# Francesco215/autoregressive_diffusion

Measured on AMD Instinct MI355X. Metric: denoiser-step frames/sec at 1/2/4/8 MI355X; 64-frame Lunar-Lander seq, higher is better.
Workload: dtype bf16; 1 GPU; Lunar-Lander 64-frame seq, gym EDM2 UNet 46.2M (gym_train.py:37-47), 8 seq/GPU (gym_train.py:55 micro_batch_size), step = EDM2Loss fwd + bwd + grad all-reduce + [grad-norm clip +] AdamW + 2 EMA profiles, 3:1 mix of 3-D/2-D steps; global_batch=8, seq_len=64, parallelism=dp1, hip_graph=False

## Files before the change

autoregressive_diffusion_amd/_lib.py:

```python
import ctypes as C
import os

import torch

_HERE = os.path.dirname(os.path.abspath(__file__))
LIB_PATH = os.path.join(_HERE, os.environ.get("ONIRIS_LIB_NAME", "liboniris_hip.so"))

if not os.path.exists(LIB_PATH):
    raise ImportError(f"{LIB_PATH} not found: build the HIP extension first (make -j8 at the repo root); "
                      "there is no CPU/PyTorch fallback for the denoiser kernels")

lib = C.CDLL(LIB_PATH)

c_void_p, c_int, c_float, c_int32, c_int64, c_size_t = C.c_void_p, C.c_int, C.c_float, C.c_int32, C.c_int64, C.c_size_t


class WeightDesc(C.Structure):
    _fields_ = [("w", c_void_p), ("grad", c_void_p), ("wf", c_void_p), ("wb", c_void_p), ("dwp", c_void_p), ("dws", c_void_p),
                ("cout", c_int32), ("cin", c_int32), ("taps", c_int32), ("kt", c_int32),
                ("CoutP", c_int32), ("CinP", c_int32), ("CoutPb", c_int32), ("CinPb", c_int32),
                ("row_start", c_int32), ("perm3", c_int32), ("gain", c_float), ("nsplit_cap", c_int32),
                ("nsplit", c_void_p), ("tile_start", c_int32), ("pad_", c_int32)]


class ConvArgs(C.Structure):
    _fields_ = [("x", c_void_p), ("ctx", c_void_p), ("w_own", c_void_p), ("w_ctx", c_void_p), ("out", c_void_p),
                ("coef_own", c_void_p), ("coef_ctx", c_void_p),
                ("B", c_int32), ("S", c_int32), ("T", c_int32), ("H", c_int32), ("W", c_int32),
                ("Cin", c_int32), ("CinP", c_int32), ("Cout", c_int32), ("CoutP", c_int32), ("taps", c_int32),
                ("ctx_bstride", c_int32), ("ctx_T", c_int32), ("coff0", c_int32), ("coff1", c_int32),
                ("ctx_fill", c_float), ("epi", c_int32),
                ("res", c_void_p), ("escale", c_void_p), ("emb_gain", c_void_p), ("out2", c_void_p),
                ("ta", c_float), ("tb", c_float), ("clip", c_float), ("ctx_out", c_void_p),
                ("big_tile", c_int32), ("escale_pitch", c_int32),
                ("splitk_ws", c_void_p), ("splitk_ws_bytes", C.c_size_t), ("clip_flag", c_void_p),
                ("ctx_prod", c_void_p), ("ctx_prod_mode", c_int32), ("x_split", c_int32), ("x2", c_void_p), ("act_out", c_void_p),
                ("cat_w1", c_float), ("cat_w2", c_float), ("ctx_rows", c_int32),
                ("ab_c1", c_int32), ("ab_da", c_void_p), ("ab_xo", c_void_p), ("ab_dskip", c_void_p), ("ab_dadd", c_void_p),
                ("ab_w1", c_float), ("ab_w2", c_float), ("ab_dxo_scale", c_float)]


class WgradArgs(C.Structure):
    _fields_ = [("x", c_void_p), ("dy", c_void_p), ("dwp", c_void_p), ("scale", c_void_p),
                ("B", c_int32), ("T", c_int32), ("H", c_int32), ("W", c_int32), ("Cin", c_int32), ("CinP", c_int32),
                ("Cout", c_int32), ("CoutP", c_int32), ("taps", c_int32),
                ("xb_stride", c_int32), ("x_T", c_int32), ("coff", c_int32), ("fill", c_float),
                ("nsplit_cap", c_int32), ("taps_total", c_int32), ("tap0", c_int32), ("pad_", c_int32),
                ("nsplit_out", c_void_p)]


class AttnArgs(C.Structure):
    _fields_ = [("q", c_void_p), ("k", c_void_p), ("v", c_void_p), ("qt", c_void_p), ("kt", c_void_p),
                ("vt", c_void_p), ("out", c_void_p), ("lse", c_void_p),
                ("kv_num", c_void_p), ("kv_idx", c_void_p), ("q_num", c_void_p), ("q_idx", c_void_p),
                ("tab_cols", c_int32), ("qtab_cols", c_int32),
                ("B", c_int32), ("heads", c_int32), ("Lq", c_int32), ("Lk", c_int32), ("C", c_int32),
                ("mask_mode", c_int32), ("P", c_int32), ("T", c_int32), ("tab_block", c_int32),
                ("dout", c_void_p), ("doutt", c_void_p), ("delta", c_void_p),
                ("dq", c_void_p), ("dk", c_void_p), ("dv", c_void_p),
                ("dkv_part", c_void_p), ("dkv_chunks", c_int32), ("dkv_item_keys", c_int32),
                ("sched", c_void_p), ("sched_wgs", c_int32), ("sched_slots", c_int32), ("v_bstride", c_int64),
                ("k_bstride", c_int64), ("split_ws", c_void_p), ("kv_splits", c_int32), ("frame_kernel", c_int32)]


class AttnF32Args(C.Structure):
    _fields_ = [("q", c_void_p), ("k", c_void_p), ("v", c_void_p), ("out", c_void_p), ("lse", c_void_p),
                ("dout", c_void_p), ("delta", c_void_p), ("dq", c_void_p), ("dk", c_void_p), ("dv", c_void_p),
                ("BH", c_int32), ("Lq", c_int32), ("Lk", c_int32), ("D", c_int32), ("mask_mode", c_int32), ("P", c_int32),
                ("T", c_int32), ("q_frame_off", c_int32), ("scale", c_float), ("pad_", c_int32)]


EPI_NONE, EPI_EMB_SILU, EPI_MPSUM, EPI_ACT_BWD = 0, 1, 2, 3

_SIGS = {
    "oniris_last_error": (C.c_char_p, []),
    "oniris_abi_version": (c_int, []),
    "oniris_struct_sizes": (c_int, [c_void_p]),
    "oniris_profile_arm": (c_int, [c_void_p, c_void_p]),
    "oniris_profile_disarm": (c_int, []),
    "oniris_set_cu_reserve": (c_int, [c_int]),
    "oniris_set_ew_nt_bytes": (c_int64, [c_int64]),
    "oniris_frame_attn_bwd": (c_int, [c_void_p, c_void_p]),
    "oniris_frame_attn_qkv_fwd": (c_int, [c_void_p, c_void_p, c_void_p, c_int64, c_int, c_int, c_void_p]),
    "oniris_frame_attn_qkv_bwd": (c_int, [c_void_p, c_void_p, c_void_p, c_void_p, c_void_p, c_int64, c_int, c_int, c_void_p]),
    "oniris_conv_f32": (c_int, [c_void_p, c_void_p, c_void_p, c_int64, c_int, c_int, c_int, c_int, c_int, c_void_p]),
    "oniris_wgrad_f32": (c_int, [c_void_p, c_void_p, c_void_p, c_int64, c_int, c_int, c_int, c_int, c_int, c_void_p]),
    "oniris_attn_f32_fwd": (c_int, [c_void_p, c_void_p]),
    "oniris_attn_f32_bwd": (c_int, [c_void_p, c_void_p]),
    "oniris_census": (c_int, [c_int]),
    "oniris_census_read": (c_int64, [C.c_char_p, c_int64]),
    "oniris_train_mask": (c_int, [c_int, c_int, c_void_p, c_void_p, C.POINTER(c_int)]),
    "oniris_infer_mask": (c_int, [c_int, c_int, c_void_p, c_void_p, C.POINTER(c_int)]),
    "oniris_mask_transpose": (c_int, [c_int, c_int, c_void_p, c_void_p, c_void_p, c_void_p]),
    "oniris_attn_schedule": (c_int, [c_int, c_int, c_void_p, c_int, c_void_p, c_int]),
    "oniris_weight_prep": (c_int, [c_void_p, c_int, c_int, c_int, c_int, c_void_p]),
    "oniris_weight_bwd": (c_int, [c_void_p, c_int, c_int, c_void_p]),
    "oniris_adamw": (c_int, [c_void_p, c_void_p, c_void_p, c_void_p, c_size_t, c_float, c_float, c_float, c_float,
                             c_float, c_int, c_float, c_void_p]),
    "oniris_adamw_clip_ema": (c_int, [c_void_p, c_void_p, c_void_p, c_void_p, c_size_t, c_float, c_float, c_float,
                                      c_float, c_float, c_int, c_float, c_void_p, c_float, c_void_p, c_float, c_void_p,
                                      c_float, c_void_p]),
    "oniris_sqnorm": (c_int, [c_void_p, c_size_t, c_void_p, c_void_p]),
    "oniris_dart_input": (c_int, [c_void_p, c_void_p, c_void_p, c_void_p, c_int, c_int, c_int, c_int, c_int, c_int,
                                  c_float, c_void_p, c_int, c_void_p]),
    "oniris_dart_loss": (c_int, [c_void_p, c_void_p, c_void_p, c_void_p, c_void_p, c_void_p, c_int, c_int, c_int, c_int,
                                 c_int, c_int, c_float, c_void_p]),
    "oniris_dart_loss_bwd": (c_int, [c_void_p, c_void_p, c_void_p, c_void_p, c_void_p, c_void_p, c_void_p, c_void_p, c_int,
                                     c_int, c_int, c_int, c_int, c_int, c_float, c_void_p]),
    "oniris_loss_tail": (c_int, [c_void_p, c_void_p, c_void_p, c_void_p, c_void_p, c_void_p, c_void_p, c_void_p, c_void_p, c_int,
                                 c_int, c_int, c_int, c_int, c_int, c_float, c_void_p]),
    "oniris_qkv_norm_hd": (c_int, [c_void_p, c_void_p, c_void_p, c_void_p, c_void_p, c_void_p, c_void_p, c_int64, c_int, c_int,
                                   c_int, c_int, c_int, c_int, c_int, c_void_p]),
    "oniris_qkv_norm_hd_bwd": (c_int, [c_void_p, c_void_p, c_void_p, c_void_p, c_void_p, c_void_p, c_void_p, c_void_p, c_int64,
                                       c_int, c_int, c_int, c_int, c_int, c_int, c_int, c_void_p]),
    "oniris_rope_hd": (c_int, [c_void_p, c_void_p, c_void_p, c_void_p, c_void_p, c_int64, c_int, c_int, c_int, c_int, c_int,
                               c_int, c_int, c_void_p]),
    "oniris_conv_fwd": (c_int, [C.POINTER(ConvArgs), c_void_p]),
    "oniris_conv_wgrad": (c_int, [C.POINTER(WgradArgs), c_void_p]),
    "oniris_conv_wgrad_group": (c_int, [C.POINTER(WgradArgs), c_int, c_void_p]),
    "oniris_gconv_bwd_prep": (c_int, [c_void_p, c_void_p, c_void_p, c_void_p, c_void_p, c_void_p, c_void_p, c_void_p,
                                      c_int, c_int, c_int, c_int64, c_void_p]),
    "oniris_gconv_bwd_fused": (c_int, [c_int, c_void_p, c_void_p, c_void_p, c_void_p, c_void_p, c_void_p, c_void_p, c_void_p,
                                       c_void_p, c_void_p, c_void_p, c_void_p, c_void_p, c_int, c_int, c_int, c_int,
                                       c_float, c_float, c_float, c_int, c_void_p, c_void_p, c_void_p]),
    "oniris_act_fwd": (c_int, [c_void_p, c_void_p, c_void_p, c_void_p, c_void_p, c_int64, c_int, c_int, c_float, c_float,
                               c_int, c_int, c_int, c_int, c_void_p]),
    "oniris_act_bwd": (c_int, [c_void_p, c_void_p, c_void_p, c_void_p, c_void_p, c_void_p, c_void_p, c_int64, c_int, c_int,
                               c_float, c_float, c_int, c_float, c_void_p]),
    "oniris_mpsum_mask": (c_int, [c_void_p, c_void_p, c_int64, c_float, c_void_p, c_void_p]),
    "oniris_emb_silu_bwd": (c_int, [c_void_p, c_void_p, c_void_p, c_void_p, c_void_p, c_int, c_int, c_int, c_int, c_int,
                                    c_void_p]),
    "oniris_mpsum_bwd": (c_int, [c_void_p, c_void_p, c_void_p, c_void_p, c_int64, c_float, c_float, c_float, c_void_p]),
    "oniris_resample": (c_int, [c_void_p, c_void_p, c_void_p, c_int64, c_int, c_int, c_int, c_int, c_float, c_void_p]),
    "oniris_resample_filter": (c_int, [c_void_p, c_void_p, c_void_p, c_int64, c_int, c_int, c_int, c_int, c_void_p, c_int, c_float,
                                       c_void_p]),
    "oniris_qkv_norm": (c_int, [c_void_p, c_void_p, c_void_p, c_void_p, c_int64, c_int, c_int64, c_int64, c_int64, c_void_p]),
    "oniris_qkv_norm_bwd": (c_int, [c_void_p, c_void_p, c_void_p, c_void_p, c_void_p, c_int64, c_int, c_void_p]),
    "oniris_qkv_norm_rope": (c_int, [c_void_p, c_void_p, c_void_p, c_void_p, c_void_p, c_void_p, c_void_p, c_int64, c_int, c_int,
                                     c_int, c_void_p]),
    "oniris_qkv_norm_rope_bwd": (c_int, [c_void_p, c_void_p, c_void_p, c_void_p, c_void_p, c_void_p, c_void_p, c_void_p, c_int64,
                                         c_int, c_int, c_int, c_void_p]),
    "oniris_qkv_eval": (c_int, [c_void_p, c_void_p, c_void_p, c_void_p, c_void_p, c_void_p, c_void_p, c_void_p, c_void_p, c_int64,
                                c_int, c_int, c_int64, c_int64, c_int64, c_int, c_void_p]),
    "oniris_precond_out": (c_int, [c_void_p, c_void_p, c_void_p, c_void_p, c_void_p, c_int, c_int, c_int, c_int, c_float,
                                   c_void_p]),
    "oniris_qkv_eval_pair": (c_int, [c_void_p, c_void_p, c_void_p, c_void_p, c_void_p, c_void_p, c_void_p, c_void_p, c_void_p,
                                     c_int64, c_int64, c_int, c_int, c_int64, c_int64, c_int64, c_int, c_void_p, c_void_p, c_void_p,
                                     c_void_p]),
    "oniris_dart_input_pair": (c_int, [c_void_p, c_void_p, c_void_p, c_int, c_int, c_int, c_int, c_int, c_float, c_void_p, c_int,
                                       c_void_p]),
    "oniris_precond_out_guided": (c_int, [c_void_p, c_void_p, c_void_p, c_void_p, c_void_p, c_int, c_int, c_int, c_int, c_float,
                                          c_float, c_void_p]),
    "oniris_sampler_update": (c_int, [c_int, c_void_p, c_void_p, c_void_p, c_void_p, c_void_p, c_size_t, c_float, c_float,
                                      c_void_p, c_int, c_float, c_void_p]),
    "oniris_embed_eval": (c_int, [c_void_p, c_void_p, c_void_p, c_void_p, c_void_p, c_void_p, c_void_p, c_int, c_int, c_int,
                                  c_int, c_void_p]),
    "oniris_gates": (c_int, [c_void_p, c_void_p, c_void_p, c_void_p, c_void_p, c_int, c_int, c_int, c_void_p]),
    "oniris_gates_bwd": (c_int, [c_void_p, c_void_p, c_void_p, c_void_p, c_void_p, c_void_p, c_int, c_int, c_int, c_void_p]),
    "oniris_emb_scale": (c_int, [c_void_p, c_void_p, c_void_p, c_void_p, c_int, c_int, c_void_p]),
    "oniris_emb_scale_bwd": (c_int, [c_void_p, c_void_p, c_void_p, c_void_p, c_void_p, c_void_p, c_int, c_int, c_int, c_void_p]),
    "oniris_embed_pre": (c_int, [c_void_p, c_void_p, c_void_p, c_void_p, c_void_p, c_void_p, c_int, c_int, c_int, c_int, c_int,
                                 c_void_p]),
    "oniris_embed_post": (c_int, [c_void_p, c_void_p, c_void_p, c_size_t, c_float, c_void_p]),
    "oniris_embed_post_bwd": (c_int, [c_void_p, c_void_p, c_void_p, c_void_p, c_void_p, c_size_t, c_float, c_void_p]),
    "oniris_rope": (c_int, [c_void_p, c_void_p, c_void_p, c_void_p, c_void_p, c_void_p, c_int, c_int, c_int, c_int,
                            c_int, c_int, c_int, c_int64, c_int64, c_void_p]),
    "oniris_qkv_norm_rope_eval": (c_int, [c_void_p, c_void_p, c_void_p, c_void_p, c_void_p, c_void_p, c_void_p, c_void_p,
                                          c_int64, c_int, c_int64, c_int64, c_int64, c_int, c_void_p]),
    "oniris_attn_fwd": (c_int, [C.POINTER(AttnArgs), c_void_p]),
    "oniris_attn_bwd_prep": (c_int, [c_void_p, c_void_p, c_void_p, c_void_p, c_void_p, c_void_p, c_int, c_int, c_int, c_int,
                                     c_void_p]),
    "oniris_attn_bwd_dq": (c_int, [C.POINTER(AttnArgs), c_void_p]),
    "oniris_attn_bwd_dkv": (c_int, [C.POINTER(AttnArgs), c_void_p]),
    "oniris_vae_temb": (c_int, [c_void_p, c_void_p, c_int, c_void_p, c_int, c_void_p, c_void_p]),
    "oniris_vae_up": (c_int, [c_void_p, c_int64, c_int64, c_int64, c_int64, c_int64, c_int, c_int, c_int, c_int, c_int, c_void_p,
                              c_void_p, c_void_p, c_void_p, c_int, c_int, c_void_p, c_void_p]),
    "oniris_vae_res_a": (c_int, [c_void_p, c_void_p, c_void_p, c_void_p, c_void_p, c_void_p, c_int, c_int, c_int, c_int, c_int,
                                 c_int, c_int, c_int, c_void_p, c_void_p]),
    "oniris_vae_res_b": (c_int, [c_void_p, c_void_p, c_void_p, c_void_p, c_int, c_int, c_int, c_int, c_int, c_int, c_void_p,
                                 c_void_p]),
    "oniris_vae_out": (c_int, [c_void_p, c_void_p, c_void_p, c_int, c_int, c_int, c_int, c_int, c_int, c_int, c_void_p, c_void_p,
                               c_void_p, c_int64, c_int64, c_int64, c_int64, c_int64, c_void_p, c_void_p]),
    "oniris_vae_down": (c_int, [c_void_p, c_int, c_int64, c_int64, c_int64, c_int64, c_int64, c_int, c_int, c_int, c_int, c_int,
                                c_int, c_int, c_int, c_void_p, c_void_p, c_int, c_void_p, c_void_p]),
    "oniris_vae_latents": (c_int, [c_void_p, c_int, c_int, c_int, c_int, c_int, c_void_p, c_void_p, c_void_p, c_int64, c_int64,
                                   c_int64, c_int64, c_int64, c_void_p]),
    "oniris_vae_train_res_a": (c_int, [c_void_p, c_void_p, c_void_p, c_void_p, c_int, c_int, c_int, c_int, c_int, c_int, c_int,
                                       c_int, c_void_p, c_void_p]),
    "oniris_vae_train_res_b": (c_int, [c_void_p, c_void_p, c_void_p, c_void_p, c_int, c_int, c_int, c_int, c_int, c_int, c_void_p,
                                       c_void_p]),
    "oniris_vae_res_b_bwd": (c_int, [c_void_p, c_void_p, c_void_p, c_int, c_int, c_int, c_int, c_int, c_int, c_void_p, c_void_p]),
    "oniris_vae_res_a_bwd": (c_int, [c_void_p, c_void_p, c_void_p, c_void_p, c_void_p, c_int, c_int, c_int, c_int, c_int, c_int,
                                     c_int, c_int, c_void_p, c_void_p, c_void_p]),
    "oniris_vae_conv3_wgrad_bwd": (c_int, [c_void_p, c_void_p, c_void_p, c_int, c_int, c_int, c_int, c_int, c_int, c_int, c_void_p,
                                           c_int, c_void_p]),
    "oniris_vae_slab_sum_bwd": (c_int, [c_void_p, c_int, c_int64, c_void_p, c_void_p]),
    "oniris_vae_lin_dx_bwd": (c_int, [c_void_p, c_int, c_int, c_int, c_void_p, c_void_p, c_int, c_int, c_int, c_int, c_int, c_int,
                                      c_int, c_void_p]),
    "oniris_vae_lin_dw_bwd": (c_int, [c_void_p, c_int, c_int, c_int, c_void_p, c_int, c_int, c_int, c_int, c_int, c_int, c_int,
                                      c_void_p, c_int, c_void_p]),
}
# ... 43 lines not shown
```

autoregressive_diffusion_amd/csrc/common.h:

```cpp
#pragma once
#include <hip/hip_runtime.h>
#include <hip/hip_ext.h>
#include <stdint.h>
#include <stdio.h>
#include <string.h>

typedef __bf16 bf16;
typedef __attribute__((ext_vector_type(8))) __bf16 bf16x8;
typedef __attribute__((ext_vector_type(4))) __bf16 bf16x4;
typedef __attribute__((ext_vector_type(2))) __bf16 bf16x2;
typedef __attribute__((ext_vector_type(4))) short s16x4;
typedef __attribute__((ext_vector_type(16))) float f32x16;
typedef __attribute__((ext_vector_type(4))) float f32x4;
typedef __attribute__((ext_vector_type(4))) unsigned int u32x4;

#define ONIRIS_OK 0
#define ONIRIS_EINVAL (-1)
#define ONIRIS_ELAUNCH (-2)
#define ONIRIS_EUNSUPPORTED (-3)

void oniris_set_error(const char* fmt, ...);

#define ONIRIS_CHECK_ARG(cond, ...)                \
  do {                                             \
    if (!(cond)) {                                 \
      oniris_set_error(__VA_ARGS__);               \
      return ONIRIS_EINVAL;                        \
    }                                              \
  } while (0)

#define ONIRIS_LAUNCH_CHECK()                                            \
  do {                                                                   \
    hipError_t e_ = hipGetLastError();                                   \
    if (e_ != hipSuccess) {                                              \
      oniris_set_error("%s:%d launch failed: %s", __FILE__, __LINE__,    \
                       hipGetErrorString(e_));                           \
      return ONIRIS_ELAUNCH;                                             \
    }                                                                    \
  } while (0)

extern thread_local hipEvent_t oniris_prof_ev[2];

extern int oniris_census_on;
void oniris_census_note(const void* kernel_handle, const char* tag);
#define ONIRIS_KLAUNCH(kern, grid, block, shmem, stream, ...)                            \
  do {                                                                                   \
    if (oniris_census_on) oniris_census_note((const void*)(kern), nullptr);              \
    hipLaunchKernelGGL(kern, grid, block, shmem, stream, __VA_ARGS__);                   \
  } while (0)

template <typename K, typename... A>
static inline void oniris_launch_tagged(const char* tag, K kern, dim3 grid, dim3 block, hipStream_t stream, A... args) {
  if (oniris_census_on) oniris_census_note((const void*)kern, tag);
  if (oniris_prof_ev[0]) {
    hipExtLaunchKernelGGL(kern, grid, block, 0, stream, oniris_prof_ev[0], oniris_prof_ev[1], 0, args...);
    oniris_prof_ev[0] = oniris_prof_ev[1] = nullptr;
  } else {
    hipLaunchKernelGGL(kern, grid, block, 0, stream, args...);
  }
}
template <typename K, typename... A>
static inline void oniris_launch(K kern, dim3 grid, dim3 block, hipStream_t stream, A... args) {
  oniris_launch_tagged(nullptr, kern, grid, block, stream, args...);
}

long long oniris_ew_nt_bytes(void);
template <bool NT, typename V>
__device__ __forceinline__ V ldv(const V* p) {
  if constexpr (NT) return __builtin_nontemporal_load(p);
  else return *p;
}
template <bool NT, typename V>
__device__ __forceinline__ void stv(V* p, V v) {
  if constexpr (NT) __builtin_nontemporal_store(v, p);
  else *p = v;
}

extern int oniris_cu_reserve;
int oniris_persistent_wgs(void);

static inline int cdiv(int a, int b) { return (a + b - 1) / b; }
static inline int roundup(int a, int b) { return cdiv(a, b) * b; }

#ifdef __HIPCC__
__device__ __forceinline__ float bf2f(bf16 v) { return (float)v; }
__device__ __forceinline__ bf16 f2bf(float v) { return (bf16)v; }

__device__ __forceinline__ f32x16 mfma32(bf16x8 a, bf16x8 b, f32x16 c) {
  return __builtin_amdgcn_mfma_f32_32x32x16_bf16(a, b, c, 0, 0, 0);
}
__device__ __forceinline__ float sigmoid_fast(float z) {
  return __builtin_amdgcn_rcpf(1.f + __builtin_amdgcn_exp2f(-1.4426950408889634f * z));
}
__device__ __forceinline__ float act_adjoint_da(float da, float xo) {
  const float sg = sigmoid_fast(xo);
  const float one_m = 1.f - sg;
  const float u = __builtin_fmaf(one_m, xo, 1.f);
  float g = sg * u;
  g = g * da;
  return g * (1.0f / 0.596f);
}
__device__ __forceinline__ float act_adjoint_dxo(float g, float dxo_scale, float dxo) { return __builtin_fmaf(dxo_scale, dxo, g); }
__device__ __forceinline__ float act_adjoint_out(float g, float w, bool has_add, float add) {
  return has_add ? __builtin_fmaf(w, g, add) : g * w;
}
__device__ __forceinline__ int mfma_row(int r, int lane) { return (r & 3) + 8 * (r >> 2) + 4 * (lane >> 5); }

__device__ __forceinline__ float wave_sum(float v) {
#pragma unroll
  for (int o = 32; o > 0; o >>= 1) v += __shfl_xor(v, o);
  return v;
}
__device__ __forceinline__ float wave_max(float v) {
#pragma unroll
  for (int o = 32; o > 0; o >>= 1) v = fmaxf(v, __shfl_xor(v, o));
  return v;
}

__device__ __forceinline__ float block_sum(float v, float* red) {
  v = wave_sum(v);
  const int w = threadIdx.x >> 6, nw = blockDim.x >> 6;
  __syncthreads();
  if ((threadIdx.x & 63) == 0) red[w] = v;
  __syncthreads();
  float t = 0.f;
  for (int i = 0; i < nw; ++i) t += red[i];
  return t;
}
#endif
```

autoregressive_diffusion_amd/csrc/conv_api.hip:

```cpp
#include "conv_fwd_common.h"

extern "C" int oniris_conv_fwd(const OnirisConvArgs* args, oniris_stream_t stream_) {
  hipStream_t st = (hipStream_t)stream_;
  ONIRIS_CHECK_ARG(args && args->w_own && ((args->x && args->out) || args->ctx_prod_mode == 3), "conv_fwd: null pointer");
  const OnirisConvArgs& a = *args;
  if (a.ctx_prod_mode != 0 && !(a.S == 1 && a.ctx && a.taps == 9 && a.ctx_prod)) {
    oniris_set_error("conv_fwd: ctx_prod_mode %d is for the one-frame cached evaluation (S == 1, context path, ctx_prod given)", a.ctx_prod_mode);
    return ONIRIS_EUNSUPPORTED;
  }
  if (a.ctx_rows != 0 && !(a.S == 1 && a.T == 1 && a.ctx && a.taps == 9 && a.ctx_rows > 0 && a.B == 2 * a.ctx_rows &&
                           a.ctx_out == nullptr && a.ctx_prod_mode != 3)) {
    oniris_set_error("conv_fwd: ctx_rows %d is for the one-frame cached evaluation of a guided pair (S = T = 1, context path, "
                     "B = 2 * ctx_rows (got B = %d), no ctx_out, ctx_prod_mode != 3)", a.ctx_rows, a.B);
    return ONIRIS_EUNSUPPORTED;
  }
  ONIRIS_CHECK_ARG(a.taps == 9 || a.taps == 1, "conv_fwd: taps must be 1 or 9 (got %d)", a.taps);
  ONIRIS_CHECK_ARG(a.B > 0 && a.T > 0 && a.H > 0 && a.W > 0 && (a.S == 1 || a.S == 2), "conv_fwd: bad sizes");
  ONIRIS_CHECK_ARG(a.Cin % 8 == 0 && a.Cout % 8 == 0, "conv_fwd: Cin, Cout must be multiples of 8 (%d,%d)", a.Cin, a.Cout);
  ONIRIS_CHECK_ARG(a.CoutP % 32 == 0 && a.CinP % 64 == 0 && a.CoutP >= a.Cout && a.CinP >= a.Cin,
                   "conv_fwd: bad padded sizes CoutP=%d CinP=%d", a.CoutP, a.CinP);
  ONIRIS_CHECK_ARG(a.epi != ONIRIS_EPI_MPSUM || a.res, "conv_fwd: EPI_MPSUM needs res");
  ONIRIS_CHECK_ARG(a.epi != ONIRIS_EPI_EMB_SILU || (a.escale && a.out2), "conv_fwd: EPI_EMB_SILU needs escale/out2");
  ONIRIS_CHECK_ARG(a.epi != ONIRIS_EPI_ACT_BWD ||
                       (a.taps == 1 && a.S == 1 && !a.ctx && !a.x2 && !a.out2 && !a.ctx_out && !a.coef_own && !a.coef_ctx && a.ab_da && a.ab_xo &&
                        a.ab_dskip && a.ab_c1 > 0 && a.ab_c1 < a.Cout && a.ab_c1 % 8 == 0 && a.ctx_prod_mode == 0 && a.ctx_rows == 0),
                   "conv_fwd: EPI_ACT_BWD is a plain 1x1 launch (S == 1) with ab_da / ab_xo / ab_dskip and 0 < ab_c1 < Cout, ab_c1 %% 8 == 0");
  ONIRIS_CHECK_ARG(a.x2 == nullptr || (a.taps == 1 && a.ctx == nullptr), "conv_fwd: x2 (concatenated input) is a 1x1, context-free option");
  const bool has_ctx = a.ctx != nullptr;
  ONIRIS_CHECK_ARG(!has_ctx || (a.w_ctx && a.taps == 9), "conv_fwd: context path needs w_ctx and taps == 9");
  if (a.clip_flag && (a.taps == 1 || (a.S == 1 && has_ctx))) {
    const hipError_t e = hipMemsetD32Async((hipDeviceptr_t)a.clip_flag, 1, 1, st);
    if (e != hipSuccess) { oniris_set_error("conv: clip_flag fill failed: %s", hipGetErrorString(e)); return ONIRIS_ELAUNCH; }
  }
  if (a.taps == 1) {
    ONIRIS_CHECK_ARG(a.S == 1, "conv_fwd: 1x1 variant expects S == 1 (fold slots into T)");
    return conv_dispatch_1x1(a, st);
  }
  if (a.S == 2) {
    ONIRIS_CHECK_ARG(has_ctx, "conv_fwd: S == 2 is the DART training layout and needs the context path");
    return conv_dispatch_s2ctx(a, st);
  }
  return has_ctx ? conv_dispatch_s1ctx(a, st) : conv_dispatch_s1(a, st);
}
```

autoregressive_diffusion_amd/csrc/conv_fwd_s2ctx.hip:

```cpp
#include "conv_fwd_common.h"
#include "conv_glds.h"
#include "conv_stream.h"

template <int NT>
static int glds_pick(const OnirisConvArgs& a, hipStream_t st) {
  if constexpr (NT == 1)
    if (a.Cin == 32 && a.big_tile != 7) return launch_conv_glds<1, 16, 8, 1, 1, true, true>(a, st);
  return launch_conv_glds<NT, 16, 8, 1>(a, st);
}

int conv_dispatch_s2ctx(const OnirisConvArgs& a, hipStream_t st) {
  if (a.big_tile >= 4 && conv_stream_ok(a)) return launch_conv_stream(a, st);
  if (a.big_tile >= 3 && conv_glds_ok(a, 16, 16, (a.CoutP % 64 == 0) ? 64 : 32))
    return (a.CoutP % 64 == 0) ? glds_pick<2>(a, st) : glds_pick<1>(a, st);
  if (a.big_tile >= 3 && a.W == 8 && a.H == 8 && a.CoutP % 64 == 0 && conv_glds_ok(a, 8, 8, 64))
    return launch_conv_glds<1, 8, 8, 1, 2>(a, st);
  if (a.clip_flag) {
    const hipError_t e = hipMemsetD32Async((hipDeviceptr_t)a.clip_flag, 1, 1, st);
    if (e != hipSuccess) { oniris_set_error("conv: clip_flag fill failed: %s", hipGetErrorString(e)); return ONIRIS_ELAUNCH; }
  }
  return conv3x3_pick<2, true>(a, st);
}
```

autoregressive_diffusion_amd/csrc/conv_stream.h:

```cpp
#pragma once
#include "conv_kernels.h"
#include "lds_dma.h"

#ifdef CONV_STAMP
#define SSTAMP_DECL unsigned long long st_t = __builtin_amdgcn_s_memtime(), st_acc[8] = {0, 0, 0, 0, 0, 0, 0, 0};
#define SSTAMP(i) { const unsigned long long n_ = __builtin_amdgcn_s_memtime(); st_acc[i] += n_ - st_t; st_t = n_; }
#else
#define SSTAMP_DECL
#define SSTAMP(i)
#endif

struct ConvStreamDev {
  OnirisConvArgs a;
  int ntx, nty, nseg, seglen;
  int dir;
  int nt;
};

template <bool ALIAS>
__global__ __launch_bounds__(256, 2) void conv_stream_kernel(const ConvStreamDev d) {
#if defined(__HIP_DEVICE_COMPILE__)
  constexpr int TAPS = 9, KS = 2, NST = TAPS * KS, HW_ = 18, HALO = 6 * 18, HBUF = 7168;
  constexpr int NXS0 = ALIAS ? 4 : 2, NCTX = ALIAS ? 0 : 3;
  constexpr int EROW = 80, STGB = 32 * EROW;
  constexpr int XS0 = 0, XS1 = NXS0 * HBUF, CTXR = XS1 + 2 * HBUF, EXCH = CTXR + NCTX * HBUF;
  constexpr int STG = ALIAS ? EXCH + 6 * 4096 : EXCH, ESC = EXCH + 6 * 4096 + (ALIAS ? 4 * STGB : 0);
  constexpr int LDS_BYTES = ESC + 512;
  static_assert(2 * LDS_BYTES <= 160 * 1024, "two workgroups per CU");
  __shared__ __attribute__((aligned(16))) unsigned char smem[LDS_BYTES];

  const OnirisConvArgs& a = d.a;
  const int tid = threadIdx.x, lane = tid & 63, wave = tid >> 6, r = lane & 31, h = lane >> 5;
  const int uw = __builtin_amdgcn_readfirstlane(wave);
  const bool ctxw = uw >= 2;
  const int sl = uw >> 1, pt = uw & 1;
  const int H = a.H, W = a.W, T = a.T, HWp = H * W, Cout = a.Cout;
  constexpr int Cin = 32;
  const int frame_elems = HWp * Cin;

  int u;
  {
    const int n = gridDim.x, xcd = blockIdx.x & 7, q = n >> 3, rr = n & 7;
    u = ((xcd < rr) ? xcd * (q + 1) : rr * (q + 1) + (xcd - rr) * q) + (blockIdx.x >> 3);
  }
  const int seg = u % d.nseg; u /= d.nseg;
  const int x0 = (u % d.ntx) * 16; u /= d.ntx;
  const int y0 = (u % d.nty) * 4;
  const int b = u / d.nty;
  const int t_lo = seg * d.seglen, t_hi = min(T, t_lo + d.seglen), nfr = t_hi - t_lo;
  const int dir = d.dir, ts = (dir > 0) ? t_lo : t_hi - 1;

  int pr;
  {
    const bool ga = (r < 4) || (r >= 12 && r < 16) || (r >= 20 && r < 28);
    const int k = ga ? ((r < 4) ? r : (r < 16) ? r - 8 : r - 12) : ((r < 12) ? r - 4 : (r < 20) ? r - 8 : r - 16);
    pr = (ga ? 0 : 16) + k;
  }
  int xaddrA[TAPS], xaddrB[TAPS];
#pragma unroll
  for (int tap = 0; tap < TAPS; ++tap) {
    const int tA = ctxw ? 0 : pt, tB = ctxw ? 1 : pt;
    const int RA = (2 * tA + (pr >> 4) + tap / 3) * HW_ + (pr & 15) + tap % 3;
    const int RB = (2 * tB + (pr >> 4) + tap / 3) * HW_ + (pr & 15) + tap % 3;
    xaddrA[tap] = RA * 64 + ((h ^ ((RA >> 2) & 3)) << 4);
    xaddrB[tap] = RB * 64 + ((h ^ ((RB >> 2) & 3)) << 4);
  }

  constexpr int OOB = (int)0x80000000;
  int hv[2];
#pragma unroll
  for (int i = 0; i < 2; ++i) {
    const int e = i * 256 + tid, row = e >> 2, gp = (e & 3) ^ ((row >> 2) & 3);
    const int y = y0 + row / HW_ - 1, x = x0 + row % HW_ - 1;
    hv[i] = (e < HALO * 4 && (unsigned)y < (unsigned)H && (unsigned)x < (unsigned)W) ? ((y * W + x) * Cin + gp * 8) * 2 : OOB;
  }
  const i32x4 rs_x = make_rsrc((const bf16*)a.x + (size_t)b * 2 * T * frame_elems, 2 * T * frame_elems * 2);
  const i32x4 rs_c = make_rsrc((const bf16*)a.ctx + (size_t)b * a.ctx_bstride * frame_elems, a.ctx_T * frame_elems * 2);
  const i32x4 rs_f = make_rsrc(oniris_fill_rows, 128);
  const int fillsel = (a.ctx_fill != 0.f) ? 64 : 0;
  const unsigned lds0 = (unsigned)(size_t)(lds_void_t*)smem, wdst = lds0 + wave * 1024;
  auto halo = [&](const i32x4& rs, int so, unsigned dst) __attribute__((always_inline)) {
    dma16(rs, hv[0], so, dst + wdst);
    if (256 + tid < HALO * 4) dma16(rs, hv[1], so, dst + wdst + 4096);
  };
  auto halo_fill = [&](unsigned dst) __attribute__((always_inline)) {
    dma16(rs_f, (hv[0] < 0) ? OOB : fillsel, 0, dst + wdst);
    if (256 + tid < HALO * 4) dma16(rs_f, (hv[1] < 0) ? OOB : fillsel, 0, dst + wdst + 4096);
  };
  auto ctx_slot = [&](int f) __attribute__((always_inline)) {
    return ALIAS ? XS0 + (f & 3) * HBUF : CTXR + ((f + 3) % 3) * HBUF;
  };
  auto issue_ctx = [&](int f) __attribute__((always_inline)) {
    if (f >= 0 && f < a.ctx_T) halo(rs_c, f * frame_elems * 2, ctx_slot(f));
    else halo_fill(ctx_slot(f));
  };
  auto issue_x = [&](int f) __attribute__((always_inline)) {
    halo(rs_x, f * frame_elems * 2, XS0 + (ALIAS ? (f & 3) : (f & 1)) * HBUF);
    halo(rs_x, (T + f) * frame_elems * 2, XS1 + (f & 1) * HBUF);
  };

  bf16x8 wreg[NST];
  {
    const bf16* wsrc = ctxw ? (const bf16*)a.w_ctx + (size_t)(uw - 2) * TAPS * a.CoutP * a.CinP : (const bf16*)a.w_own;
#pragma unroll
    for (int i = 0; i < NST; ++i)
      wreg[i] = *(const bf16x8*)(wsrc + ((size_t)(i / KS) * a.CoutP + r) * a.CinP + (i % KS) * 16 + h * 8);
  }
#pragma unroll
  for (int i = 0; i < NST; ++i) asm volatile("" : "+v"(wreg[i]));

  const int ppy = 2 * pt + (pr >> 4), ppx = pr & 15;
  const int pix = (y0 + ppy) * W + x0 + ppx;
  const int uslot = sl;
  const bool emb = a.epi == ONIRIS_EPI_EMB_SILU, mps = a.epi == ONIRIS_EPI_MPSUM;
  const int epitch = a.escale_pitch ? a.escale_pitch : Cout;
  const i32x4 rs_e = make_rsrc(a.escale ? a.escale : (const void*)oniris_fill_rows, emb ? (int)(((size_t)a.B * 2 * T - 1) * epitch + Cout) * 4 : 0);
  const i32x4 rs_r = make_rsrc(mps ? (const bf16*)a.res + (size_t)b * 2 * T * HWp * Cout : (const bf16*)oniris_fill_rows,
                               mps ? 2 * T * HWp * Cout * 2 : 0);
  const int evoff = (lane < 16 && (lane & 7) * 4 < Cout) ? ((lane >> 3) * T * epitch) * 4 + (lane & 7) * 16 : OOB;
  auto issue_esc = [&](int f) __attribute__((always_inline)) {
    if (lane < 16) dma16(rs_e, evoff, ((b * 2 * T + f) * epitch) * 4, lds0 + ESC + (f & 1) * 256);
  };
  typedef __attribute__((ext_vector_type(2))) unsigned int u32x2;
  u32x2 resq[4];
#pragma unroll
  for (int g = 0; g < 4; ++g) { resq[g][0] = 0u; resq[g][1] = 0u; }
  int rvoff[4];
#pragma unroll
  for (int g = 0; g < 4; ++g) rvoff[g] = (8 * g + 4 * h < Cout) ? (pix * Cout + 8 * g + 4 * h) * 2 : OOB;
  auto load_res = [&](int f) __attribute__((always_inline)) {
    const int so = __builtin_amdgcn_readfirstlane(((uslot * T + f) * HWp * Cout) * 2);
#pragma unroll
    for (int g = 0; g < 4; ++g)
      asm volatile("buffer_load_dwordx2 %0, %1, %2, %3 offen" : "=v"(resq[g]) : "v"(rvoff[g]), "s"(rs_r), "s"(so) : "memory");
  };
  auto wait_vm = [&](int n) __attribute__((always_inline)) {
    switch (n) {
      case 0: asm volatile("s_waitcnt vmcnt(0)" ::: "memory"); break;
      case 1: asm volatile("s_waitcnt vmcnt(1)" ::: "memory"); break;
      case 2: asm volatile("s_waitcnt vmcnt(2)" ::: "memory"); break;
      case 3: asm volatile("s_waitcnt vmcnt(3)" ::: "memory"); break;
      case 4: asm volatile("s_waitcnt vmcnt(4)" ::: "memory"); break;
      case 5: asm volatile("s_waitcnt vmcnt(5)" ::: "memory"); break;
      case 6: asm volatile("s_waitcnt vmcnt(6)" ::: "memory"); break;
      case 7: asm volatile("s_waitcnt vmcnt(7)" ::: "memory"); break;
      case 8: asm volatile("s_waitcnt vmcnt(8)" ::: "memory"); break;
      default: asm volatile("s_waitcnt vmcnt(9)" ::: "memory"); break;
    }
  };
  const int per_halo = (uw < 3) ? 2 : 1;
  const int n_dma = (ALIAS ? 2 : 3) * per_halo + ((emb && uw == 0) ? 1 : 0);
  const int n_st = (a.ctx_out ? 1 : 0) + 2 * (mps ? ((a.out2 ? 1 : 0) + 1) : emb ? 2 : 1);
  if (nfr <= 0) return;
  issue_ctx(ts + a.coff0);
  issue_ctx(ts + a.coff1);
  issue_x(ts);
  if (emb && uw == 0) issue_esc(ts);

  float* const E = (float*)(smem + EXCH);
  unsigned char* const ep = smem + STG + wave * (ALIAS ? STGB : 4096);

  SSTAMP_DECL
#pragma unroll 1
  for (int i = 0; i < nfr; ++i) {
    const int t = ts + i * dir, tn = t + dir;
    SSTAMP(7)
    wait_vm(i ? n_st : 0);
    SSTAMP(0)
    __syncthreads();
    SSTAMP(1)
    const bool has_next = i + 1 < nfr;
    const int nfrm = __builtin_amdgcn_readfirstlane((b * 2 + uslot) * T + t);
    typedef const __attribute__((address_space(4))) float cfloat_t;
    const float cown = a.coef_own ? ((cfloat_t*)(size_t)a.coef_own)[nfrm] : 1.f;
    const float cctx = a.coef_ctx ? ((cfloat_t*)(size_t)a.coef_ctx)[nfrm] : 1.f;
    if (mps) load_res(t);
    if (has_next) {
      issue_x(tn);
      if (!ALIAS) issue_ctx(tn + a.coff1);
      if (emb && uw == 0) issue_esc(tn);
    }

    SSTAMP(2)
    f32x16 acc0, acc1;
#pragma unroll
    for (int k = 0; k < 16; ++k) { acc0[k] = 0.f; acc1[k] = 0.f; }
    {
      const unsigned char* bA = smem + (ctxw ? ctx_slot(t + (uw == 2 ? a.coff0 : a.coff1)) : XS0 + (ALIAS ? (t & 3) : (t & 1)) * HBUF);
      const unsigned char* bB = ctxw ? bA : smem + XS1 + (t & 1) * HBUF;
      bf16x8 xf[2][2];
      xf[0][0] = *(const bf16x8*)(bA + xaddrA[0]);
      xf[0][1] = *(const bf16x8*)(bB + xaddrB[0]);
#pragma unroll
      for (int st = 0; st < NST; ++st) {
        if (st + 1 < NST) {
          const int tap = (st + 1) / KS, ks = (st + 1) % KS;
          xf[(st + 1) & 1][0] = *(const bf16x8*)(bA + (xaddrA[tap] ^ (ks * 32)));
          xf[(st + 1) & 1][1] = *(const bf16x8*)(bB + (xaddrB[tap] ^ (ks * 32)));
        }
        acc0 = mfma32(wreg[st], xf[st & 1][0], acc0);
        acc1 = mfma32(wreg[st], xf[st & 1][1], acc1);
        if (st + 1 < NST) __builtin_amdgcn_sched_group_barrier(0x100, 2, 0);
        __builtin_amdgcn_sched_group_barrier(0x008, 2, 0);
      }
    }
#ifdef CONV_STAMP
    asm volatile("" ::"v"(acc0), "v"(acc1));
#endif
    SSTAMP(3)
    if (!ctxw) {
#pragma unroll
      for (int k = 0; k < 16; ++k) E[(pt * 16 + k) * 64 + lane] = acc1[k];
    } else {
      const int e0 = (uw == 2) ? 2 : 4;
#pragma unroll
      for (int k = 0; k < 16; ++k) {
        E[((e0 + 0) * 16 + k) * 64 + lane] = acc0[k];
        E[((e0 + 1) * 16 + k) * 64 + lane] = acc1[k];
      }
    }
    SSTAMP(4)
    __syncthreads();
    SSTAMP(5)
    float v[16], cx[16];
    if (!ctxw) {
#pragma unroll
      for (int k = 0; k < 16; ++k) {
        cx[k] = E[((2 + pt) * 16 + k) * 64 + lane] + E[((4 + pt) * 16 + k) * 64 + lane];
        v[k] = __builtin_fmaf(cctx, cx[k], cown * acc0[k]);
      }
    } else {
      const float* Eo = E + ((((uw == 2) ? 4 : 2) + pt) * 16) * 64 + lane;
      const float* Ew = E + (pt * 16) * 64 + lane;
#pragma unroll
      for (int k = 0; k < 16; ++k) {
        const float mine = pt ? acc1[k] : acc0[k], other = Eo[k * 64];
        cx[k] = (uw == 2) ? mine + other : other + mine;
        v[k] = __builtin_fmaf(cctx, cx[k], cown * Ew[k * 64]);
      }
    }
    if (!ALIAS) __syncthreads();
    const size_t blk = ((size_t)(b * 2 + sl) * T + t) * HWp;
    auto put = [&](const float (&vv)[16]) __attribute__((always_inline)) {
#pragma unroll
      for (int g = 0; g < 4; ++g) {
        bf16x4 o;
#pragma unroll
        for (int k = 0; k < 4; ++k) o[k] = f2bf(vv[4 * g + k]);
        *(bf16x4*)(ep + pr * EROW + (8 * g + 4 * h) * 2) = o;
      }
    };
    auto flush_row = [&](bf16* dst, size_t fblk, int it) __attribute__((always_inline)) {
      const int id = it * 64 + lane, row = id >> 2, part = id & 3;
      const size_t px_ = (size_t)(y0 + 2 * pt + (row >> 4)) * W + x0 + (row & 15);
      if (part * 8 < Cout) {
        const u32x4 v_ = *(const u32x4*)(ep + row * EROW + part * 16);
        u32x4* o_ = (u32x4*)(dst + (fblk + px_) * Cout + part * 8);
        if (d.nt) __builtin_nontemporal_store(v_, o_); else *o_ = v_;
      }
    };
    auto flush = [&](bf16* dst, size_t fblk) __attribute__((always_inline)) {
      flush_row(dst, fblk, 0);
      flush_row(dst, fblk, 1);
    };
    auto store_y3 = [&]() __attribute__((always_inline)) {
      put(cx);
      flush_row((bf16*)a.ctx_out, ((size_t)b * T + t) * HWp, sl);
    };
    if (mps) {
      wait_vm(has_next ? n_dma : 0);
#pragma unroll
      for (int g = 0; g < 4; ++g) asm volatile("" : "+v"(resq[g]));
      float o[16];
      bool clip_hit = false;
#pragma unroll
      for (int g = 0; g < 4; ++g) {
        const bf16x4 rv = __builtin_bit_cast(bf16x4, resq[g]);
#pragma unroll
        for (int k = 0; k < 4; ++k) {
          float q = a.ta * bf2f(rv[k]) + a.tb * v[4 * g + k];
          if (a.clip > 0.f) {
            q = fminf(fmaxf(q, -a.clip), a.clip);
            clip_hit |= !(fabsf(bf2f(f2bf(q))) < a.clip);
          }
          o[4 * g + k] = q;
        }
      }
      if (a.ctx_out) store_y3();
      if (a.out2) { put(v); flush((bf16*)a.out2, blk); }
      put(o);
      flush((bf16*)a.out, blk);
      if (a.clip_flag && __builtin_amdgcn_ballot_w64(clip_hit) != 0ull) {
        if (lane == 0) atomicOr(a.clip_flag, 1);
        asm volatile("s_waitcnt vmcnt(0)" ::: "memory");
      }
      SSTAMP(6)
      continue;
    }
    if (a.ctx_out) store_y3();
    {
      put(v);
      flush((bf16*)a.out, blk);
      if (a.epi == ONIRIS_EPI_EMB_SILU) {
#pragma unroll
        for (int g = 0; g < 4; ++g) {
          const float4 ev = *(const float4*)(smem + ESC + (t & 1) * 256 + (sl * 32 + 8 * g + 4 * h) * 4);
          const float cvv[4] = {ev.x, ev.y, ev.z, ev.w};
#pragma unroll
          for (int k = 0; k < 4; ++k) {
            const float z = bf2f(f2bf(v[4 * g + k])) * cvv[k];
            v[4 * g + k] = z * sigmoid_fast(z) * (1.f / 0.596f);
          }
        }
        put(v);
        flush((bf16*)a.out2, blk);
      }
    }
    SSTAMP(6)
  }
#ifdef CONV_STAMP
  if (blockIdx.x == 0 && lane == 0 && a.splitk_ws) {
    unsigned long long* dst = (unsigned long long*)a.splitk_ws + wave * 8;
    for (int i = 0; i < 8; ++i) dst[i] = st_acc[i];
  }
#endif
#endif
}

static inline bool conv_stream_ok(const OnirisConvArgs& a) {
  if (!(a.S == 2 && a.ctx && a.taps == 9 && a.Cin == 32 && a.CinP == 64 && a.CoutP == 32 && a.W % 16 == 0 && a.H % 4 == 0))
    return false;
  if (!(a.ctx_fill == 0.f || a.ctx_fill == 1.f) || a.ctx_T != a.T) return false;
  if (!((a.coff0 == -2 && a.coff1 == -1) || (a.coff0 == 2 && a.coff1 == 1))) return false;
  if (2LL * a.T * a.H * a.W * 32 * 2 >= (1LL << 31)) return false;
  return true;
}

static int launch_conv_stream(const OnirisConvArgs& a, hipStream_t stream) {
  ConvStreamDev d;
  d.a = a;
  d.ntx = a.W / 16; d.nty = a.H / 4;
  d.dir = (a.coff0 < 0) ? 1 : -1;
  const int units = a.B * d.ntx * d.nty;
  int nseg = 512 / units;
  if (nseg > a.T / 8) nseg = a.T / 8;
  if (nseg < 1) nseg = 1;
  d.nt = 2LL * a.B * a.T * a.H * a.W * a.Cout * 2 >= oniris_ew_nt_bytes();
  d.seglen = cdiv(a.T, nseg);
  d.nseg = cdiv(a.T, d.seglen);
  const bool alias = a.ctx == a.x && a.ctx_bstride == 2 * a.T && d.dir == 1;
  if (alias) oniris_launch_tagged(d.nt ? "nt-stores" : nullptr, conv_stream_kernel<true>, dim3(units * d.nseg), dim3(256), stream, d);
  else oniris_launch_tagged(d.nt ? "nt-stores" : nullptr, conv_stream_kernel<false>, dim3(units * d.nseg), dim3(256), stream, d);
  ONIRIS_LAUNCH_CHECK();
  return ONIRIS_OK;
}
```

autoregressive_diffusion_amd/csrc/conv_wgrad.hip:

```cpp
#include "conv_kernels.h"

#define WGRAD_MAXG 3
struct WgradDev {
  OnirisWgradArgs a[WGRAD_MAXG];
  int ntiles[WGRAD_MAXG], ntt[WGRAD_MAXG], gstart[WGRAD_MAXG + 1];
  int ntx, nty, ncib;
};

__device__ __forceinline__ bf16x8 tr_frag(const unsigned char* base0, const unsigned char* base1) {
  typedef __attribute__((address_space(3))) s16x4 lds_s16x4;
  const s16x4 lo = __builtin_amdgcn_ds_read_tr16_b64_v4i16((lds_s16x4*)base0);
  const s16x4 hi = __builtin_amdgcn_ds_read_tr16_b64_v4i16((lds_s16x4*)base1);
  typedef __attribute__((ext_vector_type(8))) short s16x8;
  s16x8 v;
  v[0] = lo[0]; v[1] = lo[1]; v[2] = lo[2]; v[3] = lo[3];
  v[4] = hi[0]; v[5] = hi[1]; v[6] = hi[2]; v[7] = hi[3];
  return __builtin_bit_cast(bf16x8, v);
}

#include "conv_wgrad_glds.h"
#include "conv_wgrad_stream.h"
#include "wgrad1x1_glds.h"

template <int TAPS, int PW, int CT, int IT>
// ... 122 lines not shown
#pragma unroll 1
  for (int tile = bx; tile < g_ntiles; tile += gxg) {
    store_tile();
    __syncthreads();
    if (tile + gxg < g_ntiles) load_tile(tile + gxg);
    {
      constexpr int NK = 8 / NKS, NSTEP = NK * TAPS;
      bf16x8 af[4], bfm[4];
      auto ld_a = [&](int kb, int ksi) __attribute__((always_inline)) {
        const int ks = ksi * NKS + my_ks;
        const int p0 = ks * 16 + 8 * hh + q, p1 = p0 + 4;
        af[kb] = tr_frag(dy_lds + p0 * DY_ROWB + (ct * 32 + pcol) * 2, dy_lds + p1 * DY_ROWB + (ct * 32 + pcol) * 2);
      };
      auto ld_b = [&](int fb, int st) __attribute__((always_inline)) {
        const int ksi = st / TAPS, tap = st % TAPS;
        const int ks = ksi * NKS + my_ks;
        const int p0 = ks * 16 + 8 * hh + q, p1 = p0 + 4;
        int r0 = p0, r1 = p1;
        if constexpr (TAPS == 9) {
          r0 = ((p0 / (P::PH * P::PW)) * P::HH + (p0 / P::PW) % P::PH) * P::HW + p0 % P::PW;
          r1 = ((p1 / (P::PH * P::PW)) * P::HH + (p1 / P::PW) % P::PH) * P::HW + p1 % P::PW;
        }
        const int off = (TAPS == 9) ? ((tap / 3) * P::HW + (tap % 3)) : 0;
        bfm[fb] = tr_frag(x_lds + (r0 + off) * X_ROWB + (it * 32 + pcol) * 2, x_lds + (r1 + off) * X_ROWB + (it * 32 + pcol) * 2);
      };
      constexpr int LA = (NSTEP > 3) ? 3 : 1;
      constexpr int NA0 = (LA + TAPS - 1) / TAPS;
#pragma unroll
      for (int j = 0; j < LA; ++j) {
        if (j % TAPS == 0) ld_a((j / TAPS) & 3, j / TAPS);
        ld_b(j, j);
      }
      __builtin_amdgcn_sched_group_barrier(0x100, 2 * NA0 + 2 * LA, 0);
#pragma unroll
      for (int st = 0; st < NSTEP; ++st) {
        const int ksi = st / TAPS, tap = st % TAPS;
        const int nx = st + LA;
        if (nx < NSTEP) {
          if (nx % TAPS == 0) ld_a((nx / TAPS) & 3, nx / TAPS);
          ld_b(nx & 3, nx);
        }
        acc[tap] = mfma32(af[ksi & 3], bfm[st & 3], acc[tap]);
        if (nx < NSTEP) {
          if (nx % TAPS == 0) __builtin_amdgcn_sched_group_barrier(0x100, 4, 0);
          else __builtin_amdgcn_sched_group_barrier(0x100, 2, 0);
        }
        __builtin_amdgcn_sched_group_barrier(0x008, 1, 0);
      }
    }
    __syncthreads();
  }

  if (bx == 0 && blockIdx.y == 0 && tid == 0 && a.nsplit_out) *a.nsplit_out = gxg;
  const int cj = ci0 + it * 32 + (lane & 31);
  if constexpr (NKS > 1) {
    float* red = (float*)smem;
#pragma unroll
    for (int tap = 0; tap < TAPS; ++tap) {
      __syncthreads();
      if (my_ks > 0) {
#pragma unroll
        for (int rr = 0; rr < 16; ++rr) red[((my_ks - 1) * 16 + rr) * 64 + lane] = acc[tap][rr];
      }
      __syncthreads();
      if (my_ks == 0) {
#pragma unroll
        for (int rr = 0; rr < 16; ++rr) {
          float v = acc[tap][rr];
#pragma unroll
          for (int w = 0; w < NKS - 1; ++w) v += red[(w * 16 + rr) * 64 + lane];
          acc[tap][rr] = v;
        }
      }
    }
    if (my_ks != 0) return;
  }
  bf16* slab = (bf16*)a.dwp + (size_t)bx * a.taps_total * a.CoutP * a.CinP;
#pragma unroll
  for (int tap = 0; tap < TAPS; ++tap) {
    bf16* base = slab + (size_t)(a.tap0 + tap) * a.CinP;
#pragma unroll
    for (int rr = 0; rr < 16; ++rr) {
      const int co = co0 + ct * 32 + mfma_row(rr, lane);
      if (co < a.CoutP && cj < a.CinP) base[(size_t)co * a.taps_total * a.CinP + cj] = f2bf(acc[tap][rr]);
    }
  }
}

template <int TAPS, int PW, int CT, int IT>
static int launch_wgrad(const OnirisWgradArgs* args, int ng, hipStream_t stream) {
  using P = Patch<PW>;
  const OnirisWgradArgs& a = args[0];
  WgradDev d;
  memset(&d, 0, sizeof(d));
  if (TAPS == 9) { d.ntx = a.W / P::PW; d.nty = a.H / P::PH; } else { d.ntx = 1; d.nty = 1; }
  d.ncib = cdiv(a.Cin, 32 * IT);
  const int ncob = cdiv(a.Cout, 32 * CT);
  const int gy = d.ncib * ncob;
  long long tot = 0;
  bool use_glds = false;
  if constexpr (TAPS == 9 && (PW == 16 || PW == 8)) use_glds = a.pad_ >= 0 && wgrad_glds_ok(args, ng);
  const int ft = (use_glds && PW == 8) ? 1 : P::FT;
  for (int g = 0; g < ng; ++g) {
    d.a[g] = args[g];
    d.ntt[g] = (TAPS == 9) ? cdiv(args[g].T, ft) : cdiv(args[g].T * a.H * a.W, 128);
    d.ntiles[g] = d.ntx * d.nty * d.ntt[g] * args[g].B;
    tot += d.ntiles[g];
  }
#ifndef WGRAD_NG
#define WGRAD_NG 1
#endif
  const int gx_budget = (CT * IT == 4) ? ((use_glds && WGRAD_NG == 1) ? 512 : 256) : 512;
  const int gx_all = gx_budget / gy > ng ? gx_budget / gy : ng;
  int gx_tot = 0;
  for (int g = 0; g < ng; ++g) {
    int gx = (int)((long long)gx_all * d.ntiles[g] / (tot > 0 ? tot : 1));
    if (gx > args[g].nsplit_cap) gx = args[g].nsplit_cap;
    if (gx > d.ntiles[g]) gx = d.ntiles[g];
    if (gx < 1) gx = 1;
    d.gstart[g] = gx_tot;
    gx_tot += gx;
  }
  for (int g = ng; g <= WGRAD_MAXG; ++g) d.gstart[g] = gx_tot;
  if constexpr (TAPS == 9 && (PW == 16 || PW == 8)) {
    if (use_glds) {
#ifndef WGRAD_NG1
#define WGRAD_NG1 1
#endif
      constexpr int NG = (CT * IT == 4) ? WGRAD_NG : WGRAD_NG1;
      auto kern = conv_wgrad_glds_kernel<CT, IT, NG, PW>;
      oniris_launch(kern, dim3(gx_tot, gy), dim3(256 * NG), stream, d);
      ONIRIS_LAUNCH_CHECK();
      return ONIRIS_OK;
    }
  }
  auto kern = conv_wgrad_kernel<TAPS, PW, CT, IT>;
  oniris_launch(kern, dim3(gx_tot, gy), dim3(256), stream, d);
  ONIRIS_LAUNCH_CHECK();
  return ONIRIS_OK;
}

template <int TAPS, int PW>
static int wgrad_pick_tile(const OnirisWgradArgs* a, int ng, hipStream_t stream) {
  if (a[0].Cin > 32 && a[0].Cout > 32) return launch_wgrad<TAPS, PW, 2, 2>(a, ng, stream);
  return launch_wgrad<TAPS, PW, 1, 1>(a, ng, stream);
}

extern "C" int oniris_conv_wgrad_group(const OnirisWgradArgs* args, int ngroups, oniris_stream_t stream_) {
  hipStream_t stream = (hipStream_t)stream_;
  ONIRIS_CHECK_ARG(args && ngroups >= 1 && ngroups <= WGRAD_MAXG, "conv_wgrad: 1..%d groups", WGRAD_MAXG);
  const OnirisWgradArgs& a = args[0];
  for (int g = 0; g < ngroups; ++g) {
    const OnirisWgradArgs& b = args[g];
    ONIRIS_CHECK_ARG(b.x && b.dy && b.dwp, "conv_wgrad: null pointer (group %d)", g);
    ONIRIS_CHECK_ARG(b.nsplit_cap >= 1 && b.taps_total >= b.taps + b.tap0 && b.tap0 >= 0,
                     "conv_wgrad: bad slab description (group %d)", g);
    ONIRIS_CHECK_ARG(b.B > 0 && b.T > 0, "conv_wgrad: empty group %d", g);
    ONIRIS_CHECK_ARG(b.H == a.H && b.W == a.W && b.Cin == a.Cin && b.CinP == a.CinP && b.Cout == a.Cout &&
                     b.CoutP == a.CoutP && b.taps == a.taps, "conv_wgrad: groups must share H, W, channels and taps");
  }
  ONIRIS_CHECK_ARG(a.taps == 9 || a.taps == 1, "conv_wgrad: taps must be 1 or 9 (got %d)", a.taps);
  ONIRIS_CHECK_ARG(a.Cin % 8 == 0 && a.Cout % 8 == 0, "conv_wgrad: Cin/Cout must be multiples of 8");
  ONIRIS_CHECK_ARG(a.CoutP % 32 == 0 && a.CinP % 64 == 0 && a.CoutP >= a.Cout && a.CinP >= a.Cin,
                   "conv_wgrad: bad padded sizes");
  if (a.taps == 1) {
    if (ngroups == 1 && a.pad_ >= 0 && wgrad1x1_glds_ok(a)) return launch_wgrad1x1_glds(a, stream);
    return wgrad_pick_tile<1, 16>(args, ngroups, stream);
  }
  const int W = a.W, H = a.H;
  if (wgrad_stream_ok(args, ngroups)) {
    const int rc = launch_wgrad_stream(args, stream);
    if (rc != 1) return rc;
  }
  if (W >= 16 && W % 16 == 0 && H % 8 == 0) return wgrad_pick_tile<9, 16>(args, ngroups, stream);
  if (W == 8 && H % 8 == 0) return wgrad_pick_tile<9, 8>(args, ngroups, stream);
  if (W == 4 && H % 4 == 0) return wgrad_pick_tile<9, 4>(args, ngroups, stream);
  if (W == 2 && H % 2 == 0) return wgrad_pick_tile<9, 2>(args, ngroups, stream);
  oniris_set_error("conv_wgrad: unsupported image size %dx%d", H, W);
  return ONIRIS_EUNSUPPORTED;
}

extern "C" int oniris_conv_wgrad(const OnirisWgradArgs* args, oniris_stream_t stream) {
  return oniris_conv_wgrad_group(args, 1, stream);
}
```

autoregressive_diffusion_amd/csrc/conv_wgrad_stream.h:

```cpp
#pragma once
#include "lds_dma.h"

struct WgradStreamDev {
  const void* x;
  const void* dout;
  const void* dy3;
  const float* scale;
  void* dwp2;
  void* dwp3;
  int32_t* nsplit2;
  int32_t* nsplit3;
  int B, T, H, W, Cin, CinP, Cout, CoutP;
  int ntx, nty, nseg, seglen, ncib;
  float fill;
};

template <int PH>
__global__ __launch_bounds__(64 * PH, 2) void conv_wgrad_stream_kernel(const WgradStreamDev d) {
#if defined(__HIP_DEVICE_COMPILE__)
  static_assert(PH == 8 || PH == 4, "tile heights");
  constexpr int NTHR = 64 * PH, NPOS = PH * 16;
  constexpr int TAPS = 9, HW_ = 18, HALO = (PH + 2) * HW_, XB = HALO * 64, DB = NPOS * 64;
  constexpr int XS0 = 0, XS1 = 4 * XB, DY0 = 6 * XB;
  constexpr int LDS_BYTES = 6 * XB + 6 * DB;
  static_assert(LDS_BYTES <= 160 * 1024 && 5 * 3 * 16 * 64 * 4 <= LDS_BYTES, "LDS budget");
  __shared__ __attribute__((aligned(16))) unsigned char smem[LDS_BYTES];

  const int tid = threadIdx.x, lane = tid & 63, wave = tid >> 6;
  const int H = d.H, W = d.W, T = d.T, HWp = H * W, Cin = d.Cin, Cout = d.Cout;
  const int cib = blockIdx.y % d.ncib, cob = blockIdx.y / d.ncib;
  const int co0 = cob * 32, ci0 = cib * 32;
  int u = blockIdx.x;
  const int seg = u % d.nseg; u /= d.nseg;
  const int x0 = (u % d.ntx) * 16; u /= d.ntx;
  const int y0 = (u % d.nty) * PH;
  const int b = u / d.nty;
  const int t0 = seg * d.seglen, t1 = min(T, t0 + d.seglen);

  const int role = (PH == 8) ? ((wave < 4) ? 0 : (wave < 6 ? 1 : 2)) : ((wave < 2) ? 0 : wave - 1);
  const int slot = (PH == 8) ? ((wave < 4) ? (wave >> 1) : 0) : ((wave < 2) ? wave : 0), half = (PH == 8) ? (wave & 1) : 0;

  f32x16 acc[TAPS];
#pragma unroll
  for (int t = 0; t < TAPS; ++t)
#pragma unroll
    for (int i = 0; i < 16; ++i) acc[t][i] = 0.f;

  constexpr int OOB = (int)0x80000000;
  int dvoff;
  {
    const int row = tid >> 2, gp = tid & 3, co = co0 + gp * 8;
    dvoff = (co < Cout) ? (((row >> 4) * W + (row & 15)) * Cout + co) * 2 : OOB;
  }
  int xvoff[2];
  bool xok[2];
#pragma unroll
  for (int i = 0; i < 2; ++i) {
    const int e = i * NTHR + tid, row = e >> 2, gp = e & 3, ci = ci0 + gp * 8;
    const int hy = row / HW_, hx = row % HW_;
    xok[i] = e < HALO * 4 && ci < Cin && (unsigned)(y0 + hy - 1) < (unsigned)H && (unsigned)(x0 + hx - 1) < (unsigned)W;
    xvoff[i] = xok[i] ? (((y0 + hy - 1) * W + (x0 + hx - 1)) * Cin + ci) * 2 : OOB;
  }
  const i32x4 rs_do = make_rsrc(d.dout, d.B * 2 * T * HWp * Cout * 2);
  const i32x4 rs_d3 = make_rsrc(d.dy3, d.B * T * HWp * Cout * 2);
  const i32x4 rs_x = make_rsrc(d.x, d.B * 2 * T * HWp * Cin * 2);
  const i32x4 rs_f = make_rsrc(oniris_fill_rows, 128);
  const int fillsel = (d.fill != 0.f) ? 64 : 0;
  const unsigned lds0 = (unsigned)(size_t)(lds_void_t*)smem;
  const unsigned wdst = lds0 + wave * 1024;
  const int dy_origin = (y0 * W + x0) * Cout * 2;

  auto issue_halo = [&](int s, int f, unsigned dst) __attribute__((always_inline)) {
    if (f >= 0) {
      const int so = (((b * 2 + s) * T + f) * HWp * Cin) * 2;
      dma16(rs_x, xvoff[0], so, dst + wdst);
      if (wave < (HALO * 4 - NTHR + 63) / 64) { if (NTHR + tid < HALO * 4) dma16(rs_x, xvoff[1], so, dst + wdst + NTHR * 16); }
    } else {
      dma16(rs_f, xok[0] ? fillsel : OOB, 0, dst + wdst);
      if (wave < (HALO * 4 - NTHR + 63) / 64) { if (NTHR + tid < HALO * 4) dma16(rs_f, xok[1] ? fillsel : OOB, 0, dst + wdst + NTHR * 16); }
    }
  };
  auto issue_frame = [&](int f) __attribute__((always_inline)) {
    issue_halo(0, f, XS0 + (f & 3) * XB);
    issue_halo(1, f, XS1 + (f & 1) * XB);
    const unsigned dyb = DY0 + (f & 1) * 3 * DB;
    dma16(rs_do, dvoff, (((b * 2 + 0) * T + f) * HWp * Cout) * 2 + dy_origin, dyb + wdst);
    dma16(rs_do, dvoff, (((b * 2 + 1) * T + f) * HWp * Cout) * 2 + dy_origin, dyb + DB + wdst);
    dma16(rs_d3, dvoff, ((b * T + f) * HWp * Cout) * 2 + dy_origin, dyb + 2 * DB + wdst);
  };

  const int hh = lane >> 5, q = (lane & 15) >> 2;
  const int cslot = (lane & 3) * 8 + 32 * ((lane >> 4) & 1);
  const int dya = (half * 64 + 8 * hh + q) * 64 + cslot;
  int xa[3];
#pragma unroll
  for (int kx = 0; kx < 3; ++kx) xa[kx] = (half * 4 * HW_ + 8 * hh + q + kx) * 64 + cslot;

  typedef __attribute__((address_space(3))) s16x4 lds_s16x4;
  typedef __attribute__((ext_vector_type(8))) short s16x8;
  auto trf = [&](const unsigned char* p0) __attribute__((always_inline)) {
    const s16x4 lo = __builtin_amdgcn_ds_read_tr16_b64_v4i16((lds_s16x4*)p0);
    const s16x4 hi = __builtin_amdgcn_ds_read_tr16_b64_v4i16((lds_s16x4*)(p0 + 256));
    s16x8 v;
    v[0] = lo[0]; v[1] = lo[1]; v[2] = lo[2]; v[3] = lo[3];
    v[4] = hi[0]; v[5] = hi[1]; v[6] = hi[2]; v[7] = hi[3];
    return __builtin_bit_cast(bf16x8, v);
  };

  const bool scaled = role == 0 && d.scale != nullptr;
  float sc_next = 1.f;
  if (t0 < t1) {
    if (scaled) sc_next = d.scale[(b * 2 + slot) * T + t0];
    asm volatile("" : "+v"(sc_next));
    issue_halo(0, t0 - 2, XS0 + ((t0 - 2) & 3) * XB);
    issue_halo(0, t0 - 1, XS0 + ((t0 - 1) & 3) * XB);
    issue_frame(t0);
  }
#pragma unroll 1
  for (int t = t0; t < t1; ++t) {
    dma_wait();
    __syncthreads();
    float sc = sc_next;
    asm volatile("" : "+v"(sc));
    if (t + 1 < t1) {
      if (scaled) sc_next = d.scale[(b * 2 + slot) * T + t + 1];
      asm volatile("" : "+v"(sc_next));
      issue_frame(t + 1);
    }
    const unsigned char* abuf = smem + DY0 + (t & 1) * 3 * DB + ((role == 0) ? slot * DB : 2 * DB);
    const unsigned char* bbuf = smem + ((role == 0) ? (slot ? XS1 + (t & 1) * XB : XS0 + (t & 3) * XB)
                                                    : XS0 + ((t - 3 + role) & 3) * XB);
    constexpr int NK = 4, NSTEP = NK * TAPS, LA = 3;
    bf16x8 af[2], bfm[4];
    auto ld_a = [&](int kb, int j) __attribute__((always_inline)) {
      bf16x8 v = trf(abuf + dya + j * 16 * 64);
      if (scaled) {
#pragma unroll
        for (int k = 0; k < 8; ++k) v[k] = f2bf(bf2f(v[k]) * sc);
      }
      af[kb] = v;
    };
    auto ld_b = [&](int fb, int st) __attribute__((always_inline)) {
      const int j = st / TAPS, tap = st % TAPS, ky = tap / 3, kx = tap % 3;
      bfm[fb] = trf(bbuf + xa[kx] + (j + ky) * HW_ * 64);
    };
#ifndef WGRAD_STREAM_ROWORDER
#define WGRAD_STREAM_ROWORDER 1
#endif
    if constexpr (WGRAD_STREAM_ROWORDER != 0) {
      constexpr int NU = NK + 2, NB = NU * 3;
      bf16x8 aw[4];
      auto ld_aw = [&](int j) __attribute__((always_inline)) { ld_a(0, j); aw[j & 3] = af[0]; };
      auto ld_bu = [&](int fb, int i) __attribute__((always_inline)) { bfm[fb] = trf(bbuf + xa[i % 3] + (i / 3) * HW_ * 64); };
      ld_aw(0);
#pragma unroll
      for (int i = 0; i < LA; ++i) ld_bu(i, i);
      __builtin_amdgcn_sched_group_barrier(0x100, 2 + 2 * LA, 0);
#pragma unroll
      for (int i = 0; i < NB; ++i) {
        const int u = i / 3, kx = i % 3;
        int nrd = 0, nmf = 0;
        if (i + LA < NB) { ld_bu((i + LA) & 3, i + LA); nrd += 2; }
        if (kx == 0 && u + 1 < NK) { ld_aw(u + 1); nrd += 2; }
#pragma unroll
        for (int ky = 0; ky < 3; ++ky) {
          const int j = u - ky;
          if (j >= 0 && j < NK) { acc[ky * 3 + kx] = mfma32(aw[j & 3], bfm[i & 3], acc[ky * 3 + kx]); ++nmf; }
        }
        if (nrd == 2) __builtin_amdgcn_sched_group_barrier(0x100, 2, 0);
        else if (nrd == 4) __builtin_amdgcn_sched_group_barrier(0x100, 4, 0);
        if (nmf == 1) __builtin_amdgcn_sched_group_barrier(0x008, 1, 0);
        else if (nmf == 2) __builtin_amdgcn_sched_group_barrier(0x008, 2, 0);
        else __builtin_amdgcn_sched_group_barrier(0x008, 3, 0);
      }
    } else {
    ld_a(0, 0);
#pragma unroll
    for (int j = 0; j < LA; ++j) ld_b(j, j);
    __builtin_amdgcn_sched_group_barrier(0x100, 2 + 2 * LA, 0);
#pragma unroll
    for (int st = 0; st < NSTEP; ++st) {
      const int ks = st / TAPS, tap = st % TAPS;
      const int nxs = st + LA;
      if (nxs < NSTEP) {
        if (nxs % TAPS == 0) ld_a((nxs / TAPS) & 1, nxs / TAPS);
        ld_b(nxs & 3, nxs);
      }
      acc[tap] = mfma32(af[ks & 1], bfm[st & 3], acc[tap]);
      if (nxs < NSTEP) {
        if (nxs % TAPS == 0) __builtin_amdgcn_sched_group_barrier(0x100, 4, 0);
        else __builtin_amdgcn_sched_group_barrier(0x100, 2, 0);
      }
      __builtin_amdgcn_sched_group_barrier(0x008, 1, 0);
    }
    }
  }

  if (blockIdx.x == 0 && blockIdx.y == 0 && tid == 0) {
    if (d.nsplit2) *d.nsplit2 = gridDim.x;
    if (d.nsplit3) *d.nsplit3 = gridDim.x;
  }
  const int nl = (PH == 8) ? ((wave == 1) ? 0 : (wave == 2) ? 1 : (wave == 3) ? 2 : (wave == 5) ? 3 : (wave == 7) ? 4 : -1)
                           : ((wave == 1) ? 0 : -1);
  float* red = (float*)smem;
#pragma unroll
  for (int r3 = 0; r3 < 3; ++r3) {
    __syncthreads();
    if (nl >= 0) {
#pragma unroll
      for (int k = 0; k < 3; ++k)
#pragma unroll
        for (int rr = 0; rr < 16; ++rr) red[((nl * 3 + k) * 16 + rr) * 64 + lane] = acc[r3 * 3 + k][rr];
    }
    __syncthreads();
    if (nl < 0) {
      const int first = (PH == 8) ? ((wave == 0) ? 0 : (wave == 4) ? 3 : 4) : 0;
      const int cnt = (PH == 8) ? ((wave == 0) ? 3 : 1) : ((wave == 0) ? 1 : 0);
#pragma unroll
      for (int k = 0; k < 3; ++k)
#pragma unroll
        for (int rr = 0; rr < 16; ++rr) {
          float v = acc[r3 * 3 + k][rr];
          for (int w = 0; w < cnt; ++w) v += red[(((first + w) * 3 + k) * 16 + rr) * 64 + lane];
          acc[r3 * 3 + k][rr] = v;
        }
    }
  }
  if (nl >= 0) return;
  const int taps_total = (role == 0) ? 9 : 18, tap0 = (role == 2) ? 9 : 0;
  const int cj = ci0 + (lane & 31);
  bf16* slab = (bf16*)((role == 0) ? d.dwp2 : d.dwp3) + (size_t)blockIdx.x * taps_total * d.CoutP * d.CinP;
#pragma unroll
  for (int tap = 0; tap < TAPS; ++tap) {
    bf16* base = slab + (size_t)(tap0 + tap) * d.CinP;
#pragma unroll
    for (int rr = 0; rr < 16; ++rr) {
      const int co = co0 + mfma_row(rr, lane);
      if (co < d.CoutP && cj < d.CinP) base[(size_t)co * taps_total * d.CinP + cj] = f2bf(acc[tap][rr]);
    }
  }
#endif
}

static inline bool wgrad_stream_ok(const OnirisWgradArgs* a, int ng) {
  if (ng != 3 || a[0].pad_ < 0 || (a[0].pad_ & 2)) return false;
  const OnirisWgradArgs &o = a[0], &c0 = a[1], &c1 = a[2];
  if (o.taps != 9 || o.W % 16 != 0 || o.H % 8 != 0) return false;
  if (o.Cin > 32 && o.Cout > 32) return false;
  if (o.B != 1 || o.coff != 0 || o.tap0 != 0 || o.taps_total != 9 || o.xb_stride != o.T || o.x_T != o.T) return false;
  if (c0.x != o.x || c1.x != o.x || c0.dy != c1.dy || c0.dwp != c1.dwp || c0.scale || c1.scale) return false;
  if (c0.B != c1.B || c0.T != c1.T || o.T != 2 * c0.B * c0.T) return false;
  if (c0.xb_stride != 2 * c0.T || c1.xb_stride != 2 * c0.T || c0.x_T != c0.T || c1.x_T != c0.T) return false;
  if (c0.coff != -2 || c1.coff != -1 || c0.tap0 != 0 || c1.tap0 != 9 || c0.taps_total != 18 || c1.taps_total != 18) return false;
  if (c0.fill != c1.fill || !(c0.fill == 0.f || c0.fill == 1.f)) return false;
  if ((long long)o.T * o.H * o.W * (o.Cout > o.Cin ? o.Cout : o.Cin) * 2 >= (1LL << 31)) return false;
  return true;
}

static int launch_wgrad_stream(const OnirisWgradArgs* a, hipStream_t stream) {
  const OnirisWgradArgs &o = a[0], &c0 = a[1];
  WgradStreamDev d;
  memset(&d, 0, sizeof(d));
  d.x = o.x; d.dout = o.dy; d.dy3 = c0.dy; d.scale = o.scale;
  d.dwp2 = o.dwp; d.dwp3 = c0.dwp; d.nsplit2 = o.nsplit_out; d.nsplit3 = c0.nsplit_out;
  d.B = c0.B; d.T = c0.T; d.H = o.H; d.W = o.W; d.Cin = o.Cin; d.CinP = o.CinP; d.Cout = o.Cout; d.CoutP = o.CoutP;
#ifndef WGRAD_STREAM_PH
#define WGRAD_STREAM_PH 4
#endif
  d.ntx = o.W / 16; d.ncib = cdiv(o.Cin, 32);
  d.fill = c0.fill;
  const int ncob = cdiv(o.Cout, 32), gy = d.ncib * ncob;
  const int cap = o.nsplit_cap < c0.nsplit_cap ? o.nsplit_cap : c0.nsplit_cap;
  int ph = (WGRAD_STREAM_PH == 4 && d.B * d.ntx * (o.H / 4) <= cap) ? 4 : 8;
  d.nty = o.H / ph;
  const int units = d.B * d.ntx * d.nty;
  if (units > cap) return 1;
  int nseg = ((ph == 4 ? 512 : 256) / gy) / units;
  if (nseg > d.T / 8) nseg = d.T / 8;
  if (nseg * units > cap) nseg = cap / units;
  if (nseg < 1) nseg = 1;
  d.seglen = cdiv(d.T, nseg);
  d.nseg = cdiv(d.T, d.seglen);
  if (ph == 4) oniris_launch(conv_wgrad_stream_kernel<4>, dim3(units * d.nseg, gy), dim3(256), stream, d);
  else oniris_launch(conv_wgrad_stream_kernel<8>, dim3(units * d.nseg, gy), dim3(512), stream, d);
  ONIRIS_LAUNCH_CHECK();
  return ONIRIS_OK;
}
```

autoregressive_diffusion_amd/csrc/weights.hip:

```cpp
#include <cstdlib>
#include "common.h"
#include "../../include/oniris.h"

#define W_EPS 1e-4f

__device__ __forceinline__ const OnirisWeightDesc* find_desc(const OnirisWeightDesc* d, int n, int row) {
  int lo = 0, hi = n - 1;
  while (lo < hi) {
    int mid = (lo + hi + 1) >> 1;
    if (d[mid].row_start <= row) lo = mid; else hi = mid - 1;
  }
  return d + lo;
}

__device__ __forceinline__ int perm_row(const OnirisWeightDesc* d, int co) {
  if (!d->perm3) return co;
  const int C = d->cout / 3;
  return (co % 3) * C + co / 3;
}

__device__ __forceinline__ const OnirisWeightDesc* find_desc_tile(const OnirisWeightDesc* d, int n, int tile) {
  int lo = 0, hi = n - 1;
  while (lo < hi) {
    int mid = (lo + hi + 1) >> 1;
// ... 215 lines not shown
  return ONIRIS_OK;
}

__global__ void adamw_kernel(float* __restrict__ p, const float* __restrict__ g, float* __restrict__ m,
                             float* __restrict__ v, size_t n, float lr, float b1, float b2, float eps, float wd,
                             float bc1, float bc2, float gscale, const float* __restrict__ gnorm_sq, float max_norm,
                             float* __restrict__ ema0, float w0, float* __restrict__ ema1, float w1) {
  if (bc1 == 0.f) {
    size_t i = ((size_t)blockIdx.x * blockDim.x + threadIdx.x) * 4;
    const size_t stride = (size_t)gridDim.x * blockDim.x * 4;
    for (; i < n; i += stride)
      for (size_t k = i; k < n && k < i + 4; ++k) {
        if (ema0) ema0[k] += w0 * (p[k] - ema0[k]);
        if (ema1) ema1[k] += w1 * (p[k] - ema1[k]);
      }
    return;
  }
  if (gnorm_sq) {
    const float coef = max_norm / (sqrtf(*gnorm_sq) * fabsf(gscale) + 1e-6f);
    if (coef < 1.f) gscale *= coef;
  }
  size_t i = ((size_t)blockIdx.x * blockDim.x + threadIdx.x) * 4;
  const size_t stride = (size_t)gridDim.x * blockDim.x * 4;
  for (; i + 3 < n; i += stride) {
    float4 P = *(float4*)(p + i), G = *(const float4*)(g + i), M = *(float4*)(m + i), V = *(float4*)(v + i);
    float* pp = (float*)&P; float* gg = (float*)&G; float* mm = (float*)&M; float* vv = (float*)&V;
#pragma unroll
    for (int k = 0; k < 4; ++k) {
      const float gr = gg[k] * gscale;
      mm[k] = b1 * mm[k] + (1.f - b1) * gr;
      vv[k] = b2 * vv[k] + (1.f - b2) * gr * gr;
      const float mh = mm[k] / bc1, vh = vv[k] / bc2;
      pp[k] = pp[k] * (1.f - lr * wd) - lr * mh / (sqrtf(vh) + eps);
    }
    *(float4*)(p + i) = P; *(float4*)(m + i) = M; *(float4*)(v + i) = V;
    if (ema0) {
      float4 E = *(float4*)(ema0 + i);
      E.x += w0 * (P.x - E.x); E.y += w0 * (P.y - E.y); E.z += w0 * (P.z - E.z); E.w += w0 * (P.w - E.w);
      *(float4*)(ema0 + i) = E;
    }
    if (ema1) {
      float4 E = *(float4*)(ema1 + i);
      E.x += w1 * (P.x - E.x); E.y += w1 * (P.y - E.y); E.z += w1 * (P.z - E.z); E.w += w1 * (P.w - E.w);
      *(float4*)(ema1 + i) = E;
    }
  }
  if (i < n && i + 3 >= n) {
    for (size_t k = i; k < n; ++k) {
      const float gr = g[k] * gscale;
      m[k] = b1 * m[k] + (1.f - b1) * gr;
      v[k] = b2 * v[k] + (1.f - b2) * gr * gr;
      p[k] = p[k] * (1.f - lr * wd) - lr * (m[k] / bc1) / (sqrtf(v[k] / bc2) + eps);
      if (ema0) ema0[k] += w0 * (p[k] - ema0[k]);
      if (ema1) ema1[k] += w1 * (p[k] - ema1[k]);
    }
  }
}

static int launch_adamw(float* p, const float* g, float* m, float* v, size_t n, float lr, float beta1, float beta2,
                        float eps, float weight_decay, int step, float grad_scale, const float* gnorm_sq, float max_norm,
                        float* ema0, float w0, float* ema1, float w1, hipStream_t stream) {
  ONIRIS_CHECK_ARG(p && g && m && v && step >= 0, "adamw: bad arguments");
  ONIRIS_CHECK_ARG(!gnorm_sq || max_norm > 0.f, "adamw: clipping needs max_norm > 0");
  if (n == 0) return ONIRIS_OK;
  const float bc1 = step ? 1.f - powf(beta1, (float)step) : 0.f, bc2 = step ? 1.f - powf(beta2, (float)step) : 0.f;
  if (step == 0 && !ema0 && !ema1) return ONIRIS_OK;
  size_t nb = (n / 4 + 255) / 256;
  if (nb > 4096) nb = 4096;
  if (nb == 0) nb = 1;
  ONIRIS_KLAUNCH(adamw_kernel, dim3((unsigned)nb), dim3(256), 0, stream, p, g, m, v, n, lr, beta1, beta2, eps,
                     weight_decay, bc1, bc2, grad_scale, gnorm_sq, max_norm, ema0, w0, ema1, w1);
  ONIRIS_LAUNCH_CHECK();
  return ONIRIS_OK;
}

extern "C" int oniris_adamw(float* p, const float* g, float* m, float* v, size_t n, float lr, float beta1, float beta2,
                            float eps, float weight_decay, int step, float grad_scale, oniris_stream_t stream_) {
  return launch_adamw(p, g, m, v, n, lr, beta1, beta2, eps, weight_decay, step, grad_scale, nullptr, 0.f, nullptr, 0.f,
                      nullptr, 0.f, (hipStream_t)stream_);
}

extern "C" int oniris_adamw_clip_ema(float* p, const float* g, float* m, float* v, size_t n, float lr, float beta1,
                                     float beta2, float eps, float weight_decay, int step, float grad_scale,
                                     const float* gnorm_sq, float max_norm, float* ema0, float ema_w0, float* ema1,
                                     float ema_w1, oniris_stream_t stream_) {
  return launch_adamw(p, g, m, v, n, lr, beta1, beta2, eps, weight_decay, step, grad_scale, gnorm_sq, max_norm, ema0,
                      ema_w0, ema1, ema_w1, (hipStream_t)stream_);
}

__global__ __launch_bounds__(256) void sqnorm_partial_kernel(const float* __restrict__ g, size_t n, float* __restrict__ part) {
  __shared__ float red[16];
  float acc = 0.f;
  size_t i = ((size_t)blockIdx.x * 256 + threadIdx.x) * 4;
  const size_t stride = (size_t)gridDim.x * 256 * 4;
  for (; i + 3 < n; i += stride) {
    const float4 G = *(const float4*)(g + i);
    acc += G.x * G.x + G.y * G.y + G.z * G.z + G.w * G.w;
  }
  if (i < n && i + 3 >= n)
    for (size_t k = i; k < n; ++k) acc += g[k] * g[k];
  acc = block_sum(acc, red);
  if (threadIdx.x == 0) part[blockIdx.x] = acc;
}
__global__ __launch_bounds__(256) void sqnorm_final_kernel(const float* __restrict__ part, int nb, float* __restrict__ out) {
  __shared__ float red[16];
  float acc = 0.f;
  for (int i = threadIdx.x; i < nb; i += 256) acc += part[i];
  acc = block_sum(acc, red);
  if (threadIdx.x == 0) out[0] = acc;
}

extern "C" int oniris_sqnorm(const float* g, size_t n, float* out, oniris_stream_t stream_) {
  hipStream_t stream = (hipStream_t)stream_;
  ONIRIS_CHECK_ARG(g && out, "sqnorm: null pointer");
  size_t nb = (n / 4 + 255) / 256;
  if (nb > ONIRIS_SQNORM_WS) nb = ONIRIS_SQNORM_WS;
  if (nb == 0) nb = 1;
  ONIRIS_KLAUNCH(sqnorm_partial_kernel, dim3((unsigned)nb), dim3(256), 0, stream, g, n, out + 1);
  ONIRIS_LAUNCH_CHECK();
  ONIRIS_KLAUNCH(sqnorm_final_kernel, dim3(1), dim3(256), 0, stream, (const float*)(out + 1), (int)nb, out);
  ONIRIS_LAUNCH_CHECK();
  return ONIRIS_OK;
}

__global__ __launch_bounds__(256) void gconv_bwd_prep_kernel(const bf16* __restrict__ dout, const bf16* __restrict__ out,
                                                             const bf16* __restrict__ y3, const float* __restrict__ ca,
                                                             const float* __restrict__ cb,
                                                             float* __restrict__ S1, float* __restrict__ S2,
                                                             bf16* __restrict__ dy3, int S, int T, size_t PC) {
  __shared__ float red[16];
  const int bt = blockIdx.x, b = bt / T, t = bt % T;
  const bf16* y3f = y3 + (size_t)bt * PC;
  bf16* dy3f = dy3 + (size_t)bt * PC;
  float s1[2] = {0.f, 0.f}, s2[2] = {0.f, 0.f};
  float c[2];
  const bf16* df[2];
  const bf16* of[2];
  for (int s = 0; s < S; ++s) {
    const size_t n = (size_t)(b * S + s) * T + t;
    c[s] = cb[n]; df[s] = dout + n * PC; of[s] = out + n * PC;
  }
  const size_t per = ((PC / 8 + gridDim.y - 1) / gridDim.y) * 8, e_lo = blockIdx.y * per, e_hi = (e_lo + per < PC) ? e_lo + per : PC;
  for (size_t e = e_lo + (size_t)threadIdx.x * 8; e < e_hi; e += 256 * 8) {
    const bf16x8 yv = *(const bf16x8*)(y3f + e);
    float acc[8];
#pragma unroll
    for (int i = 0; i < 8; ++i) acc[i] = 0.f;
    for (int s = 0; s < S; ++s) {
      const bf16x8 dv = *(const bf16x8*)(df[s] + e);
      const bf16x8 ov = *(const bf16x8*)(of[s] + e);
#pragma unroll
      for (int i = 0; i < 8; ++i) {
        const float dd = bf2f(dv[i]);
        s1[s] += dd * bf2f(ov[i]); s2[s] += dd * bf2f(yv[i]); acc[i] += c[s] * dd;
      }
    }
    bf16x8 o;
#pragma unroll
    for (int i = 0; i < 8; ++i) o[i] = f2bf(acc[i]);
    *(bf16x8*)(dy3f + e) = o;
  }
  for (int s = 0; s < S; ++s) {
    const float a = block_sum(s1[s], red), bsum = block_sum(s2[s], red);
    if (threadIdx.x == 0) { const size_t n = (size_t)(b * S + s) * T + t; atomicAdd(S1 + n, (a - cb[n] * bsum) / ca[n]); atomicAdd(S2 + n, bsum); }
  }
}

template <int MODE, bool NT>
__global__ __launch_bounds__(1024) void gconv_bwd_fused_kernel(const bf16* g, const bf16* __restrict__ raw,
                                                              const bf16* __restrict__ y3, const float* __restrict__ ca,
                                                              const float* __restrict__ cb, const float* __restrict__ cs,
                                                              const bf16* __restrict__ xo, bf16* dout,
                                                              bf16* __restrict__ dres, bf16* __restrict__ dy3,
                                                              float* __restrict__ dca, float* __restrict__ dcb,
                                                              float* __restrict__ dcs, int T, int P, int C, float ta,
                                                              float tb, float clip, int pix_per_block, int cs_pitch,
                                                              const int* __restrict__ clip_flag, float* __restrict__ ca_scaled) {
  const bool alias = MODE == 2 && ca_scaled != nullptr;
  const bool masked = MODE == 2 && clip > 0.f && (!alias || *clip_flag != 0);
  __shared__ float red[16];
  __shared__ float accs[2][512];
  const int bt = blockIdx.x, b = bt / T, t = bt % T;
  const size_t PC = (size_t)P * C;
  const int G8 = C >> 3;
  const int NTH = blockDim.x;
  const int cg = threadIdx.x % G8, pl = threadIdx.x / G8, npl = NTH / G8;
  if (MODE == 1)
    for (int i = threadIdx.x; i < 2 * 512; i += NTH) (&accs[0][0])[i] = 0.f;
  __syncthreads();
  float s1[2] = {0.f, 0.f}, s2[2] = {0.f, 0.f};
  float part[2][8];
#pragma unroll
  for (int s = 0; s < 2; ++s)
#pragma unroll
    for (int i = 0; i < 8; ++i) part[s][i] = 0.f;
  size_t nn[2];
  float cbv[2], cv[2][8];
#pragma unroll
  for (int s = 0; s < 2; ++s) {
    nn[s] = (size_t)(b * 2 + s) * T + t;
    cbv[s] = cb[nn[s]];
#pragma unroll
    for (int i = 0; i < 8; ++i) cv[s][i] = 1.f;
    if (MODE == 1 && pl < npl) {
      const float4 c0 = *(const float4*)(cs + nn[s] * cs_pitch + cg * 8), c1 = *(const float4*)(cs + nn[s] * cs_pitch + cg * 8 + 4);
      cv[s][0] = c0.x; cv[s][1] = c0.y; cv[s][2] = c0.z; cv[s][3] = c0.w;
      cv[s][4] = c1.x; cv[s][5] = c1.y; cv[s][6] = c1.z; cv[s][7] = c1.w;
    }
  }
  if (pl < npl) {
    const int p0 = blockIdx.y * pix_per_block, p1 = min(P, p0 + pix_per_block);
    for (int p = p0 + pl; p < p1; p += npl) {
      const size_t off = (size_t)p * C + cg * 8;
      const bf16x8 yv3 = ldv<NT>((const bf16x8*)(y3 + (size_t)bt * PC + off));
      float acc3[8];
#pragma unroll
      for (int i = 0; i < 8; ++i) acc3[i] = 0.f;
#pragma unroll
      for (int s = 0; s < 2; ++s) {
        const size_t o = nn[s] * PC + off;
        const bf16x8 gv = ldv<NT>((const bf16x8*)(g + o));
        const bf16x8 rv = ldv<NT>((const bf16x8*)(raw + o));
        bf16x8 dv, drv;
        bf16x8 xv;
        if (masked) xv = ldv<NT>((const bf16x8*)(xo + o));
#pragma unroll
        for (int i = 0; i < 8; ++i) {
          const float r_ = bf2f(rv[i]);
          float d;
          if (MODE == 1) {
            const float z = r_ * cv[s][i];
            const float sg = sigmoid_fast(z);
            const float dz = bf2f(gv[i]) * (sg * (1.f + z * (1.f - sg))) * (1.0f / 0.596f);
            part[s][i] += dz * r_;
            d = dz * cv[s][i];
          } else {
            float gg = bf2f(gv[i]);
            if (masked && !(fabsf(bf2f(xv[i])) < clip)) gg = 0.f;
            drv[i] = f2bf(gg * ta);
            d = gg * tb;
            if (alias) dv[i] = f2bf(gg);
          }
          float dr = d;
          if (!alias) { dv[i] = f2bf(d); dr = bf2f(dv[i]); }
          s1[s] += dr * r_; s2[s] += dr * bf2f(yv3[i]); acc3[i] += cbv[s] * dr;
        }
        if (!alias || masked) stv<NT>((bf16x8*)(dout + o), dv);
        if (MODE == 2 && dres) stv<NT>((bf16x8*)(dres + o), drv);
      }
      bf16x8 o3;
#pragma unroll
      for (int i = 0; i < 8; ++i) o3[i] = f2bf(acc3[i]);
      stv<NT>((bf16x8*)(dy3 + (size_t)bt * PC + off), o3);
    }
  }
  if (MODE == 1 && (G8 & (G8 - 1)) == 0) {
#pragma unroll
    for (int s = 0; s < 2; ++s)
#pragma unroll
      for (int i = 0; i < 8; ++i)
        for (int o = G8; o < 64; o <<= 1) part[s][i] += __shfl_xor(part[s][i], o);
    for (int q = 0; q < NTH / 64; ++q) {
      if ((int)(threadIdx.x >> 6) == q && (int)(threadIdx.x & 63) < G8)
#pragma unroll
        for (int s = 0; s < 2; ++s)
#pragma unroll
          for (int i = 0; i < 8; ++i) accs[s][cg * 8 + i] += part[s][i];
      __syncthreads();
    }
  } else if (MODE == 1) {
    for (int q = 0; q < npl; ++q) {
      if (pl == q)
#pragma unroll
        for (int s = 0; s < 2; ++s)
#pragma unroll
          for (int i = 0; i < 8; ++i) accs[s][cg * 8 + i] += part[s][i];
      __syncthreads();
    }
  }
#pragma unroll
  for (int s = 0; s < 2; ++s) {
    const float a_ = block_sum(s1[s], red), b_ = block_sum(s2[s], red);
    if (threadIdx.x == 0) {
      atomicAdd(dca + nn[s], (a_ - cbv[s] * b_) / ca[nn[s]]); atomicAdd(dcb + nn[s], b_);
      if (alias && blockIdx.y == 0) ca_scaled[nn[s]] = tb * ca[nn[s]];
    }
  }
  if (MODE == 1) {
    __syncthreads();
    for (int i = threadIdx.x; i < C; i += NTH) {
      atomicAdd(dcs + nn[0] * C + i, accs[0][i]); atomicAdd(dcs + nn[1] * C + i, accs[1][i]);
    }
  }
}

extern "C" int oniris_gconv_bwd_fused(int mode, const void* g, const void* raw, const void* y3, const float* coef_own,
                                      const float* coef_ctx, const float* cscale, const void* xo, void* dout, void* dres,
                                      void* dy3, float* d_coef_own, float* d_coef_ctx, float* d_cscale, int B, int T,
                                      int P, int C, float ta, float tb, float clip, int cscale_pitch,
                                      const int32_t* clip_flag, float* coef_own_scaled, oniris_stream_t stream_) {
  hipStream_t stream = (hipStream_t)stream_;
  ONIRIS_CHECK_ARG((mode == 1 || mode == 2) && g && raw && y3 && coef_own && coef_ctx && dout && dy3 && d_coef_own &&
                   d_coef_ctx && B > 0 && T > 0 && P > 0 && C % 8 == 0 && C <= 512, "gconv_bwd_fused: bad arguments");
  ONIRIS_CHECK_ARG(mode != 1 || (cscale && d_cscale), "gconv_bwd_fused: mode 1 needs cscale / d_cscale");
  ONIRIS_CHECK_ARG(mode != 2 || ((dres || coef_own_scaled) && (clip <= 0.f || xo)),
                   "gconv_bwd_fused: mode 2 needs dres (optional under the aliasing protocol) and xo when clipping");
  ONIRIS_CHECK_ARG((mode == 2 || (!clip_flag && !coef_own_scaled)) && (!clip_flag || coef_own_scaled) &&
                   (!coef_own_scaled || clip <= 0.f || clip_flag),
                   "gconv_bwd_fused: coef_own_scaled selects the aliasing protocol (mode 2); with clip > 0 it needs clip_flag");
  ONIRIS_CHECK_ARG(!coef_own_scaled || dout == g, "gconv_bwd_fused: the aliasing protocol masks g in place (pass dout = g)");
  int slices = 1;
  static int nth1 = -1;
  if (nth1 < 0) { const char* e = getenv("ONIRIS_GCONV_BWD_THREADS"); nth1 = e ? atoi(e) : 256; }
  const int nth = (mode == 1 && (long long)P * (C / 8) >= 4096) ? nth1 : 256;
  const int npl = nth / (C / 8) > 0 ? nth / (C / 8) : 1;
  static int tgt1 = -1;
  if (tgt1 < 0) { const char* e = getenv("ONIRIS_GCONV_BWD_BLOCKS"); tgt1 = e ? atoi(e) : 512; }
  const int tgt = (mode == 1) ? tgt1 : 2048;
  while (slices < 2 && P / (slices * 2) >= npl * 2 && (long long)B * T * slices < tgt) slices *= 2;
  const int ppb = cdiv(P, slices);
  const int csp = cscale_pitch > 0 ? cscale_pitch : C;
  ONIRIS_CHECK_ARG(csp >= C && csp % 4 == 0, "gconv_bwd_fused: cscale_pitch must be a multiple of 4 and >= C");
  const bool nt = 2LL * B * T * P * C * 2 >= oniris_ew_nt_bytes();
#define GCONV_BWD_LAUNCH(MODE_, NT_, NTH_, FLAG_, CAS_) ONIRIS_KLAUNCH((gconv_bwd_fused_kernel<MODE_, NT_>), dim3(B * T, slices), dim3(NTH_), 0, stream, (const bf16*)g, \
                       (const bf16*)raw, (const bf16*)y3, coef_own, coef_ctx, cscale, (const bf16*)xo, (bf16*)dout, \
                       (bf16*)dres, (bf16*)dy3, d_coef_own, d_coef_ctx, d_cscale, T, P, C, ta, tb, clip, ppb, csp, FLAG_, CAS_)
  if (mode == 1) { if (nt) GCONV_BWD_LAUNCH(1, true, nth, nullptr, nullptr); else GCONV_BWD_LAUNCH(1, false, nth, nullptr, nullptr); }
  else { if (nt) GCONV_BWD_LAUNCH(2, true, 256, (const int*)clip_flag, coef_own_scaled); else GCONV_BWD_LAUNCH(2, false, 256, (const int*)clip_flag, coef_own_scaled); }
#undef GCONV_BWD_LAUNCH
  ONIRIS_LAUNCH_CHECK();
  return ONIRIS_OK;
}

extern "C" int oniris_gconv_bwd_prep(const void* dout, const void* out, const void* y3, const float* coef_own,
                                     const float* coef_ctx, float* S1, float* S2, void* dy3, int B, int S, int T,
                                     int64_t frame_elems,
                                     oniris_stream_t stream_) {
  hipStream_t stream = (hipStream_t)stream_;
  ONIRIS_CHECK_ARG(dout && out && y3 && coef_own && coef_ctx && S1 && S2 && dy3 && B > 0 && T > 0 && (S == 1 || S == 2) &&
                   frame_elems > 0 && frame_elems % 8 == 0, "gconv_bwd_prep: bad arguments");
  int slices = 1;
  while (slices < 2 && (long long)B * T * slices < 1024 && frame_elems / (slices * 2) >= 256 * 8 * 2) slices *= 2;
  ONIRIS_KLAUNCH(gconv_bwd_prep_kernel, dim3(B * T, slices), dim3(256), 0, stream, (const bf16*)dout, (const bf16*)out,
                     (const bf16*)y3, coef_own, coef_ctx, S1, S2, (bf16*)dy3, S, T, (size_t)frame_elems);
  ONIRIS_LAUNCH_CHECK();
  return ONIRIS_OK;
}
```

autoregressive_diffusion_amd/ops.py:

```python
import ctypes
import math
import numpy as np
import torch

from . import _lib
from ._lib import lib, check, OnirisError

BF16 = torch.bfloat16


_raw_stream = getattr(torch._C, "_cuda_getCurrentRawStream", None)


def _stream():
    if _raw_stream is not None:
        return ctypes.c_void_p(_raw_stream(torch.cuda.current_device()))
    return ctypes.c_void_p(torch.cuda.current_stream().cuda_stream)


def _p(t):
    return None if t is None else t.data_ptr()


def _need_gpu(*ts):
# ... 379 lines not shown
                                     _stream()),
              "weight_prep")
        self._packed_sig = None if training else (_weights_epoch, tuple(w.param._version for w, _ in self.items))

    def take_flag(self, device):
        if self._flags is None or self._flags.device != device or self._flag_off >= self._flags.numel():
            self._flags, self._flag_off = torch.zeros(256, dtype=torch.int32, device=device), 0
        f = self._flags[self._flag_off:self._flag_off + 1]
        self._flag_off += 1
        return f

    def packed_valid(self):
        sig = getattr(self, "_packed_sig", None)
        return sig is not None and sig == (_weights_epoch, tuple(w.param._version for w, _ in self.items))

    def backward(self):
        self._ensure()
        check(lib.oniris_weight_bwd(_p(self._dev_table), len(self.items), self.total_rows, _stream()), "weight_bwd")
        self.nsplit_all.zero_()

    def request_finish(self):
        if not self._finish_queued:
            self._finish_queued = True
            torch.autograd.Variable._execution_engine.queue_callback(self._finish)

    def _finish(self):
        if not self._finish_queued:
            return
        self._finish_queued = False
        self.backward()
        for w, _ in self.items:
            if w.fresh:
                if not w.hit:
                    w.param.grad = None
                w.fresh = False
            w.hit = False
        for h in self.post_backward_hooks:
            h()
        GradSlot.check_all_taken()



import os as _os
import sys as _sys
FUSED_ROPE = int(_os.environ.get("ONIRIS_FUSED_ROPE", "1"))
ATTN_DKV_CHUNKS = int(_os.environ.get("ONIRIS_DKV_CHUNKS", "4"))
ATTN_DKV_MIN_L = 2048
ATTN_DKV_PERSISTENT = int(_os.environ.get("ONIRIS_DKV_PERSISTENT", "1"))
ATTN_DQ_PERSISTENT = int(_os.environ.get("ONIRIS_DQ_PERSISTENT", "1"))
WGRAD_VARIANT = int(_os.environ.get("ONIRIS_WGRAD", "0"))
BIG_TILE = int(_os.environ.get("ONIRIS_BIG_TILE", "4"))
GRAD_POOL = int(_os.environ.get("ONIRIS_GRAD_POOL", "1"))
GRAD_SLOTS = int(_os.environ.get("ONIRIS_GRAD_SLOTS", "1"))


class KernelProfile:
    enabled = False
    records = []

    @classmethod
    def start(cls):
        cls.records, cls.enabled = [], True

    @classmethod
    def stop(cls):
        cls.enabled = False
        torch.cuda.synchronize()
        agg = {}
        for key, flops, e0, e1, *rest in cls.records:
            a = agg.setdefault(key, dict(launches=0, flops=0.0, ms=0.0, bytes=0.0, t_min=0.0))
            a["launches"] += 1
            a["flops"] += flops
            a["ms"] += e0.elapsed_time(e1)
            a["bytes"] += rest[0] if rest else 0.0
            a["t_min"] += max(flops / 2.5e15, (rest[0] if rest else 0.0) / 6.3e12)
        cls.records = []
        return agg


def _timed_launch(fn):
    e0, e1 = torch.cuda.Event(enable_timing=True), torch.cuda.Event(enable_timing=True)
    e0.record()
    e1.record()
    check(lib.oniris_profile_arm(e0.cuda_event, e1.cuda_event), "profile_arm")
    try:
        fn()
    finally:
        if lib.oniris_profile_disarm():
            e1.record()
    return e0, e1


def _profiled(key, flops, fn, nbytes=None):
    if not KernelProfile.enabled:
        return fn()
    e0, e1 = _timed_launch(fn)
    KernelProfile.records.append((key, flops, e0, e1) if nbytes is None else (key, flops, e0, e1, float(nbytes)))


def train_frame_pairs(T, P):
    fpb = max(1, 128 // P)
    return T * (T + 1) // 2 + sum(1 + fpb * (f // fpb) for f in range(T))


def _attn_flops(kind, B, T, heads, L, P):
    pairs = (train_frame_pairs(T, P) * P * P * B) if kind == "video" else (B * L * L)
    return 4.0 * 64 * heads * pairs


def _patch_w(W):
    return 16 if W >= 16 else W


def conv3x3_size_ok(H, W):
    H, W = int(H), int(W)
    if H <= 0 or W <= 0:
        return False
    if W % 16 == 0:
        return H % 8 == 0
    return W in (8, 4, 2) and H % W == 0


def _conv3x3_check(H, W, forward_only_ok, wants_grad):
    if conv3x3_size_ok(H, W):
        return
    if not forward_only_ok:
        raise OnirisError(f"conv: unsupported image size {H}x{W} (H x W) for a 3x3 kernel: served are W % 16 == 0 with H % 8 == 0, "
                          f"and W in (8, 4, 2) with H % W == 0")
    if wants_grad:
        raise OnirisError(f"conv: image size {H}x{W} (H x W) is served forward-only (streaming kernel, H % 4 == 0): the weight "
                          f"gradient needs H % 8 == 0 -- run it under torch.no_grad() or pad the image")


def _s2ctx_family(T, H, W, Cin, CinP, CoutP, ctx_T, coff, ctx_fill):
    ok = ctx_fill in (0.0, 1.0)
    if (BIG_TILE >= 4 and ok and Cin == 32 and CinP == 64 and CoutP == 32 and W % 16 == 0 and H % 4 == 0 and ctx_T == T
            and tuple(coff) in ((-2, -1), (2, 1))):
        return "stream"
    if BIG_TILE >= 3 and ok and Cin % 32 == 0 and H % 16 == 0 and W % 16 == 0:
        return "glds16"
    if BIG_TILE >= 3 and ok and Cin % 32 == 0 and H == 8 and W == 8 and CoutP % 64 == 0:
        return "glds8"
    return "staged"


PROFILE_SHAPES = int(_os.environ.get("ONIRIS_PROFILE_SHAPES", "0"))
ALIAS2 = int(_os.environ.get("ONIRIS_ALIAS2", "1"))
CLIP_FLAG = int(_os.environ.get("ONIRIS_CLIP_FLAG", "1"))


def _conv_launch(x, ctx, w_own, w_ctx, out, coef_own, coef_ctx, B, S, T, H, W, Cin, CinP, Cout, CoutP, taps,
                 ctx_bstride=0, ctx_T=0, coff=(0, 0), ctx_fill=0.0, epi=0, res=None, escale=None, emb_gain=None,
                 out2=None, ta=0.0, tb=0.0, clip=0.0, ctx_out=None, clip_flag=None, ctx_prod=None, ctx_prod_mode=0,
                 x2=None, act_out=None, x_split=0, cat_w=(1.0, 1.0), ctx_rows=0, act_bwd=None):
    if KernelProfile.enabled:
        flops = 2.0 * B * S * T * H * W * Cout * Cin * taps
        if ctx is not None:
            flops += 2.0 * B * T * H * W * Cout * Cin * 2 * taps
        nt = 2 if CoutP % 64 == 0 else 1
        if (BIG_TILE >= 4 and S == 2 and ctx is not None and taps == 9 and Cin == 32 and CinP == 64 and CoutP == 32 and W % 16 == 0
                and H % 4 == 0 and ctx_fill in (0.0, 1.0) and ctx_T == T and tuple(coff) in ((-2, -1), (2, 1))):
            key = f"conv_stream_kernel<ALIAS={int(ctx.data_ptr() == x.data_ptr() and ctx_bstride == 2 * T and coff[0] < 0)}>"
        elif (BIG_TILE >= 3 and S == 2 and ctx is not None and taps == 9 and Cin % 32 == 0 and H % 16 == 0 and W % 16 == 0
                and ctx_fill in (0.0, 1.0)):
            key = f"conv_glds_kernel<NT={nt},PW=16,NW=8,MT=1,WC=1,CTX=1>"
        elif (BIG_TILE >= 3 and S == 2 and ctx is not None and taps == 9 and Cin % 32 == 0 and H == 8 and W == 8
              and CoutP % 64 == 0 and ctx_fill in (0.0, 1.0)):
            key = "conv_glds_kernel<NT=1,PW=8,NW=8,MT=1,WC=2,CTX=1>"
        elif (BIG_TILE >= 4 and not (BIG_TILE & 128) and S == 1 and ctx is None and taps == 9 and Cin == 32 and CinP == 64 and CoutP == 32
              and W % 16 == 0 and H % 8 == 0 and x2 is None and B * T * (H // 8) * (W // 16) >= 512):
            key = "conv_plain_stream_kernel"
        elif (BIG_TILE >= 3 and S == 1 and ctx is None and taps == 9 and Cin % 32 == 0 and T % 2 == 0
              and ((H % 16 == 0 and W % 16 == 0) or (H == 8 and W == 8 and CoutP % 64 == 0))):
            key = (f"conv_glds_kernel<NT={nt},PW=16,NW=8,MT=1,WC=1,CTX=0>" if H % 16 == 0 else
                   "conv_glds_kernel<NT=1,PW=8,NW=8,MT=1,WC=2,CTX=0>")
        elif (BIG_TILE >= 3 and taps == 1 and ctx is None and Cin % 64 == 0 and CinP == Cin
              and epi in (0, _lib.EPI_MPSUM, _lib.EPI_ACT_BWD) and B * S * T * H * W >= 8192):
            key = "conv1x1_glds_kernel<ACTB>" if epi == _lib.EPI_ACT_BWD else "conv1x1_glds_kernel"
        elif epi == _lib.EPI_ACT_BWD:
            key = f"conv_fwd_kernel<S=1,TAPS=1,CK=64,NT={2 if CoutP % 64 == 0 else 3},CTX=0,PW={_patch_w(W)},ACTB>"
        else:
            key = f"conv_fwd_kernel<S={S},TAPS={taps},CK={32 if taps == 9 else 64},NT={nt},CTX={int(ctx is not None)},PW={_patch_w(W)}>"
        if PROFILE_SHAPES:
            key += f" [{H}x{W} {Cin}->{Cout} epi={epi}{' act_bwd' if act_bwd is not None else ''}{' dadd' if act_bwd is not None and act_bwd[3] is not None else ''}{' res' if res is not None else ''}{' out2' if out2 is not None else ''}{' y3' if ctx_out is not None else ''}{' dgrad' if coff[0] > 0 else ''}]"
        KernelProfile.enabled = False
        try:
            e0, e1 = _timed_launch(lambda: _conv_launch(x, ctx, w_own, w_ctx, out, coef_own, coef_ctx, B, S, T, H, W, Cin, CinP,
                                                        Cout, CoutP, taps, ctx_bstride, ctx_T, coff, ctx_fill, epi, res, escale,
                                                        emb_gain, out2, ta, tb, clip, ctx_out, clip_flag, ctx_prod, ctx_prod_mode,
                                                        ctx_rows=ctx_rows, act_bwd=act_bwd))
        finally:
            KernelProfile.enabled = True
        px = B * T * H * W
        nbytes = 2.0 * (S * px * Cin + S * px * Cout * (1 + (out2 is not None) + (res is not None))
                        + (px * Cout if ctx_out is not None else 0)
                        + taps * CoutP * CinP * (3 if ctx is not None else 1))
        if ctx is not None and ctx.data_ptr() != x.data_ptr():
            nbytes += 2.0 * B * ctx_T * H * W * Cin
        if act_bwd is not None:
            nbytes += 2.0 * px * (2 * Cout + (act_bwd[4] if act_bwd[3] is not None else 0))
        KernelProfile.records.append((key, flops, e0, e1, nbytes))
        return
    a = _lib.ConvArgs()
    a.x, a.ctx, a.w_own, a.w_ctx, a.out = _p(x), _p(ctx), _p(w_own), _p(w_ctx), _p(out)
    a.coef_own, a.coef_ctx = _p(coef_own), _p(coef_ctx)
    a.B, a.S, a.T, a.H, a.W = B, S, T, H, W
    a.Cin, a.CinP, a.Cout, a.CoutP, a.taps = Cin, CinP, Cout, CoutP, taps
    a.ctx_bstride, a.ctx_T, a.coff0, a.coff1, a.ctx_fill = ctx_bstride, ctx_T, coff[0], coff[1], ctx_fill
    a.epi, a.res, a.escale, a.emb_gain, a.out2 = epi, _p(res), _p(escale), _p(emb_gain), _p(out2)
    if escale is not None:
        a.escale_pitch = escale.stride(0)
    a.ta, a.tb, a.clip, a.ctx_out = ta, tb, clip, _p(ctx_out)
    a.clip_flag = _p(clip_flag)
    a.ctx_prod, a.ctx_prod_mode = _p(ctx_prod), ctx_prod_mode
    if x2 is not None:
        a.x2, a.act_out, a.x_split, a.cat_w1, a.cat_w2 = _p(x2), _p(act_out), x_split, cat_w[0], cat_w[1]
    a.big_tile = BIG_TILE
    a.ctx_rows = ctx_rows
    if act_bwd is not None:
        da, xo, dskip, dadd, a.ab_c1, a.ab_w1, a.ab_w2, a.ab_dxo_scale = act_bwd
        a.ab_da, a.ab_xo, a.ab_dskip, a.ab_dadd = _p(da), _p(xo), _p(dskip), _p(dadd)
    if SPLITK and B * S * T * H * W <= 64 * 256 and ctx_prod_mode == 0 and ctx_rows == 0:
        ws = _splitk_workspace(x.device)
        a.splitk_ws, a.splitk_ws_bytes = _p(ws), ws.numel() * 4
    check(lib.oniris_conv_fwd(ctypes.byref(a), _stream()), "conv_fwd")


SPLITK = int(_os.environ.get("ONIRIS_SPLITK", "1"))
_splitk_cache = {}


def _splitk_workspace(device):
    key = str(device)
    if key not in _splitk_cache:
        _splitk_cache[key] = torch.empty(8 << 20, dtype=torch.float32, device=device)
    return _splitk_cache[key]


def _wgrad_args(x, dy, pw, scale, B, T, H, W, Cin, CinP, Cout, CoutP, taps, xb_stride, x_T, coff, fill, tap0=0):
    a = _lib.WgradArgs()
    pw.touched = pw.hit = True
    if pw.members is not None:
        for m_ in pw.members:
            m_.touched = m_.hit = True
    a.x, a.dy, a.dwp, a.scale = _p(x), _p(dy), _p(pw.dwp), _p(scale)
    a.nsplit_cap, a.taps_total, a.tap0, a.nsplit_out = pw.nsplit_cap, pw.taps, tap0, _p(pw.nsplit)
    a.B, a.T, a.H, a.W, a.Cin, a.CinP, a.Cout, a.CoutP, a.taps = B, T, H, W, Cin, CinP, Cout, CoutP, taps
    a.xb_stride, a.x_T, a.coff, a.fill = xb_stride, x_T, coff, fill
    a.pad_ = WGRAD_VARIANT
    return a


def _wgrad_launch_group(arglist):
    if KernelProfile.enabled:
        a0 = arglist[0]
        tile = 2 if (a0.Cin > 32 and a0.Cout > 32) else 1
        if (WGRAD_VARIANT >= 0 and not (WGRAD_VARIANT & 2) and len(arglist) == 3 and tile == 1 and a0.taps == 9 and a0.W % 16 == 0
                and a0.H % 8 == 0 and arglist[1].B * (a0.W // 16) * (a0.H // 8) <= min(a0.nsplit_cap, arglist[1].nsplit_cap)):
            key = "conv_wgrad_stream_kernel"
        elif WGRAD_VARIANT >= 0 and all(a.taps == 9 and ((a.W % 16 == 0 and a.H % 8 == 0) or (a.W == 8 and a.H == 8))
                                      and a.fill in (0.0, 1.0) for a in arglist):
            key = f"conv_wgrad_glds_kernel<CT={tile},IT={tile},NG=1,PW={_patch_w(a0.W)}>"
        elif (WGRAD_VARIANT >= 0 and len(arglist) == 1 and a0.taps == 1 and a0.Cin >= 64 and a0.Cout >= 64 and not a0.scale
              and a0.coff == 0):
            key = "wgrad1x1_glds_kernel<NG=2>"
        else:
            key = f"conv_wgrad_kernel<TAPS={a0.taps},PW={_patch_w(a0.W)},CT={tile},IT={tile}>"
        flops = sum(2.0 * a.B * a.T * a.H * a.W * a.Cout * a.Cin * a.taps for a in arglist)
        seen, nbytes = set(), 0.0
        for a in arglist:
            for ptr, n in ((a.x, a.B * a.xb_stride * a.H * a.W * a.Cin), (a.dy, a.B * a.T * a.H * a.W * a.Cout)):
                if ptr not in seen:
                    seen.add(ptr)
                    nbytes += 2.0 * n
        KernelProfile.enabled = False
        try:
            e0, e1 = _timed_launch(lambda: _wgrad_launch_group(arglist))
        finally:
            KernelProfile.enabled = True
        KernelProfile.records.append((key, flops, e0, e1, nbytes))
        return
    arr = (_lib.WgradArgs * len(arglist))(*arglist)
    check(lib.oniris_conv_wgrad_group(arr, len(arglist), _stream()), "conv_wgrad")


def _wgrad_launch(x, dy, pw, scale, B, T, H, W, Cin, CinP, Cout, CoutP, taps, xb_stride, x_T, coff, fill, tap0=0):
    _wgrad_launch_group([_wgrad_args(x, dy, pw, scale, B, T, H, W, Cin, CinP, Cout, CoutP, taps, xb_stride, x_T, coff,
                                     fill, tap0)])


class ConvCfg:
    __slots__ = ("pw2", "pw3", "B", "T", "epi", "ta", "tb", "clip", "need_grad", "in_slot", "res_slot", "grad_private", "res_alias",
                 "dgrad_slot")

    def __init__(self, pw2, pw3=None, B=1, T=1, epi="none", ta=0.0, tb=0.0, clip=0.0, need_grad=True, in_slot=None,
                 res_slot=None, grad_private=False, res_alias=False, dgrad_slot=None):
        self.pw2, self.pw3, self.B, self.T = pw2, pw3, B, T
        self.dgrad_slot = dgrad_slot
        self.grad_private = bool(grad_private)
        self.res_alias = bool(res_alias) and res_slot is not None
        self.epi, self.ta, self.tb, self.clip, self.need_grad = epi, ta, tb, clip, need_grad
        self.in_slot = in_slot
        self.res_slot = res_slot


def _rows_f32(t):
    t = t.detach()
    if t.dtype != torch.float32:
        t = t.float()
    if t.dim() != 2 or t.stride(1) != 1 or t.stride(0) % 4 != 0 or t.stride(0) < t.shape[1] or t.data_ptr() % 16 != 0:
        t = t.contiguous()
    return t


def _wants_wgrad(pw):
    members = getattr(pw, "members", None)
    if members:
        return any(m.param.requires_grad for m in members)
    return pw.param.requires_grad


class _ConvOp(torch.autograd.Function):

    @staticmethod
    def forward(ctx, x, w2param, w3param, ca, cb, cscale, res, cfg):
        _need_gpu(x)
        pw2, pw3 = cfg.pw2, cfg.pw3
        gated = pw3 is not None
        N, H, W, Cin = x.shape
        if pw2.taps == 9 and not conv3x3_size_ok(H, W):
            _conv3x3_check(H, W, gated and _s2ctx_family(cfg.T, H, W, Cin, pw2.CinP, pw2.CoutP, cfg.T, (-2, -1), 1.0) == "stream",
                           cfg.need_grad and any(ctx.needs_input_grad))
        Co = roundup(pw2.cout, 8)
        dev = x.device
        kw = {}
        raw = torch.empty((N, H, W, Co), dtype=BF16, device=dev)
        ret = raw
        clip_flag = None
        if cfg.epi == "emb_silu":
            cs = _rows_f32(cscale)
            assert tuple(cs.shape) == (N, Co), (cs.shape, N, Co)
            ret = torch.empty_like(raw)
            kw = dict(epi=_lib.EPI_EMB_SILU, escale=cs, out2=ret)
        elif cfg.epi == "mpsum":
            keep_raw = gated and cfg.need_grad
            ret = torch.empty_like(raw)
            kw = dict(epi=_lib.EPI_MPSUM, res=res, ta=cfg.ta, tb=cfg.tb, clip=cfg.clip, out2=raw if keep_raw else None)
            if not keep_raw:
                raw = None
            if (CLIP_FLAG and keep_raw and cfg.grad_private and Co <= 512 and cfg.clip > 0 and
                    _s2ctx_family(cfg.T, H, W, Cin, pw2.CinP, pw2.CoutP, cfg.T, (-2, -1), 1.0) != "staged"):
                clip_flag = pw2.bank.take_flag(dev)
                kw["clip_flag"] = clip_flag
            if (CLIP_FLAG and ALIAS2 and not gated and cfg.need_grad and cfg.grad_private and pw2.taps == 9 and cfg.clip > 0 and
                    Cin % 32 == 0 and (H % 16 == 0 and W % 16 == 0 or H == 8 and W == 8 and pw2.CoutP % 64 == 0) and N % 2 == 0):
                clip_flag = pw2.bank.take_flag(dev)
                kw["clip_flag"] = clip_flag
        y3 = ca32 = cb32 = None
        ctx.clip_flag = kw.get("clip_flag")
        first_out = ret if cfg.epi == "mpsum" else (raw if raw is not None else ret)
        if gated:
            B, T = cfg.B, cfg.T
            assert N == B * 2 * T
            y3 = torch.empty((B * T, H, W, Co), dtype=BF16, device=dev) if cfg.need_grad else None
            ca32, cb32 = ca.detach().float().contiguous(), cb.detach().float().contiguous()
            _conv_launch(x, x, pw2.wf, pw3.wf, first_out, ca32, cb32, B, 2, T, H, W, Cin, pw2.CinP, Co, pw2.CoutP, 9,
                         ctx_bstride=2 * T, ctx_T=T, coff=(-2, -1), ctx_fill=1.0, ctx_out=y3, **kw)
        else:
            _conv_launch(x, None, pw2.wf, None, first_out, None, None, 1, 1, N, H, W, Cin, pw2.CinP, Co, pw2.CoutP,
                         pw2.taps, **kw)
        ctx.cfg = cfg
        ctx.save_for_backward(x, raw, y3, ca32, cb32, kw["escale"] if cfg.epi == "emb_silu" else None,
                              ret if (cfg.epi == "mpsum" and cfg.clip > 0) else None)
        return ret

    @staticmethod
    def backward(ctx, g):
        x, raw, y3, ca, cb, cs, xo = ctx.saved_tensors
        cfg = ctx.cfg
        pw2, pw3 = cfg.pw2, cfg.pw3
        gated = pw3 is not None
        N, H, W, Cin = x.shape
        g = g.contiguous()
        Co = g.shape[-1]
        dev = x.device
        dcs = dres = None
        dx = dca = dcb = None
        plain_coef = None
        fused = gated and cfg.epi in ("emb_silu", "mpsum") and Co <= 512
        ca_own = ca
        if fused:
            B, T = cfg.B, cfg.T
            flag = getattr(ctx, "clip_flag", None) if cfg.epi == "mpsum" else None
            alias = cfg.epi == "mpsum" and cfg.grad_private and CLIP_FLAG and (flag is not None or (cfg.clip <= 0 and ALIAS2))
            if alias:
                dout = g
                ca_own = torch.empty_like(ca)
            else:
                dout = torch.empty_like(g)
            dy3 = torch.empty_like(y3)
            acc = pw2.bank.zero_arena.take(N * (2 + (Co if cfg.epi == "emb_silu" else 0)), dev)
            dca, dcb = acc[:N], acc[N:2 * N]
            res_alias = alias and cfg.res_alias
            if cfg.epi == "emb_silu":
                dcs = acc[2 * N:2 * N + N * Co].view(N, Co)
            elif not res_alias:
                dres = torch.empty_like(g)
            check(lib.oniris_gconv_bwd_fused(1 if cfg.epi == "emb_silu" else 2, _p(g), _p(raw), _p(y3), _p(ca), _p(cb),
                                             _p(cs), _p(xo), _p(dout), _p(dres), _p(dy3), _p(dca), _p(dcb), _p(dcs), B, T,
                                             H * W, Co, cfg.ta, cfg.tb, cfg.clip, cs.stride(0) if cs is not None else 0,
                                             _p(flag) if alias else None, _p(ca_own) if alias else None, _stream()), "gconv_bwd_fused")
            if res_alias:
                cfg.res_slot.put(g, cfg.ta)
                cfg = _no_res_slot(cfg)
        elif cfg.epi == "emb_silu":
            dout = torch.empty_like(g)
            dcs = pw2.bank.zero_arena.take(N * Co, dev)[:N * Co].view(N, Co)
            check(lib.oniris_emb_silu_bwd(_p(g), _p(raw), _p(cs), _p(dout), _p(dcs), N, H * W, Co, cs.stride(0), 1, _stream()),
                  "emb_silu_bwd")
        elif cfg.epi == "mpsum" and not gated and cfg.grad_private and CLIP_FLAG and ALIAS2 and pw2.taps == 9 and (
                getattr(ctx, "clip_flag", None) is not None or cfg.clip <= 0):
            flag = getattr(ctx, "clip_flag", None)
            if flag is not None:
                check(lib.oniris_mpsum_mask(_p(g), _p(xo), g.numel(), cfg.clip, _p(flag), _stream()), "mpsum_mask")
            dout, plain_coef = g, _const_vec(N, cfg.tb, dev)
            if cfg.res_alias:
                cfg.res_slot.put(g, cfg.ta)
                cfg = _no_res_slot(cfg)
            else:
                dres = torch.empty_like(g)
                check(lib.oniris_mpsum_bwd(_p(g), None, _p(dres), None, g.numel(), cfg.ta, cfg.tb, 0.0, _stream()), "mpsum_bwd")
        elif cfg.epi == "mpsum":
            dres, dout = torch.empty_like(g), torch.empty_like(g)
            check(lib.oniris_mpsum_bwd(_p(g), _p(xo), _p(dres), _p(dout), g.numel(), cfg.ta, cfg.tb, cfg.clip, _stream()),
                  "mpsum_bwd")
        else:
            dout = g
        if gated:
            B, T = cfg.B, cfg.T
            if not fused:
                acc = pw2.bank.zero_arena.take(2 * N, dev)
                dca, dcb = acc[:N], acc[N:2 * N]
                dy3 = torch.empty_like(y3)
                check(lib.oniris_gconv_bwd_prep(_p(dout), _p(raw), _p(y3), _p(ca), _p(cb), _p(dca), _p(dcb), _p(dy3), B, 2,
                                                T, H * W * Co, _stream()), "gconv_bwd_prep")
            if ctx.needs_input_grad[0]:
                dx = torch.empty_like(x)
                sel = _clean_selector(B, T, dev)
                _conv_launch(dout, dy3, pw2.wb, pw3.wb, dx, ca_own, sel, B, 2, T, H, W, Co, pw2.CinPb, Cin, pw2.CoutPb, 9,
                             ctx_bstride=T, ctx_T=T, coff=(2, 1), ctx_fill=0.0)
            grp = []
            if _wants_wgrad(pw2):
                grp.append(_wgrad_args(x, dout, pw2, ca_own, 1, N, H, W, Cin, pw2.CinP, Co, pw2.CoutP, 9, N, N, 0, 0.0))
            if _wants_wgrad(pw3):
                for j, coff in enumerate((-2, -1)):
                    grp.append(_wgrad_args(x, dy3, pw3, None, B, T, H, W, Cin, pw3.CinP, Co, pw3.CoutP, 9, 2 * T, T, coff,
                                           1.0, tap0=9 * j))
            if grp:
                _wgrad_launch_group(grp)
        else:
            if ctx.needs_input_grad[0] and cfg.dgrad_slot is not None:
                cfg.dgrad_slot.put((dout, pw2, (N, H, W, Cin, Co)))
            elif ctx.needs_input_grad[0]:
                dx = torch.empty_like(x)
                dadd = cfg.in_slot.take() if cfg.in_slot is not None else None
                if dadd is not None:
                    _conv_launch(dout, None, pw2.wb, None, dx, plain_coef, None, 1, 1, N, H, W, Co, pw2.CinPb, Cin, pw2.CoutPb,
                                 pw2.taps, epi=_lib.EPI_MPSUM, res=dadd.contiguous(), ta=1.0, tb=1.0, clip=0.0)
                else:
                    _conv_launch(dout, None, pw2.wb, None, dx, plain_coef, None, 1, 1, N, H, W, Co, pw2.CinPb, Cin, pw2.CoutPb,
                                 pw2.taps)
            if _wants_wgrad(pw2):
                _wgrad_launch(x, dout, pw2, plain_coef, 1, N, H, W, Cin, pw2.CinP, Co, pw2.CoutP, pw2.taps, N, N, 0, 0.0)
        if _wants_wgrad(pw2) or (gated and _wants_wgrad(pw3)):
            pw2.bank.request_finish()
        if cfg.res_slot is not None and dres is not None:
            cfg.res_slot.put(dres)
            dres = None
        return dx, None, None, dca, dcb, dcs, dres, None


_const_cache = {}


def _const_vec(n, value, dev):
    key = (n, float(value), str(dev))
    if key not in _const_cache:
        if len(_const_cache) > 64:
            _const_cache.clear()
        _const_cache[key] = torch.full((n,), float(value), dtype=torch.float32, device=dev)
    return _const_cache[key]


def _no_res_slot(cfg):
    c = ConvCfg(cfg.pw2, cfg.pw3, cfg.B, cfg.T, cfg.epi, cfg.ta, cfg.tb, cfg.clip, cfg.need_grad, cfg.in_slot, None,
                cfg.grad_private)
    return c


_sel_cache = {}


def _clean_selector(B, T, dev):
    key = (B, T, str(dev))
    if key not in _sel_cache:
        sel = torch.zeros(B, 2, T, dtype=torch.float32, device=dev)
        sel[:, 0] = 1.0
        _sel_cache[key] = sel.reshape(-1)
    return _sel_cache[key]


def gate_coefs(gate):
    den = torch.rsqrt((1 - gate) ** 2 + gate ** 2)
    return (1 - gate) * den, gate * den


def conv(x, pw, res=None, ta=0.0, tb=0.0, clip=0.0, cscale=None, in_slot=None, res_slot=None, grad_private=False,
         res_alias=False, dgrad_slot=None):
    epi = "mpsum" if res is not None else ("emb_silu" if cscale is not None else "none")
    assert dgrad_slot is None or (epi == "none" and in_slot is None and pw.taps == 1)
    cfg = ConvCfg(pw, None, epi=epi, ta=ta, tb=tb, clip=clip, need_grad=torch.is_grad_enabled(), in_slot=in_slot,
                  res_slot=res_slot, grad_private=grad_private, res_alias=res_alias, dgrad_slot=dgrad_slot)
    sched = pw.param
    if getattr(pw, "members", None) and not sched.requires_grad:
        sched = next((m.param for m in pw.members if m.param.requires_grad), sched)
    return _ConvOp.apply(x, sched, None, None, None, cscale, res, cfg)


def gated_conv_train(x, gate, pw2, pw3, B, T, coefs=None, res=None, ta=0.0, tb=0.0, clip=0.0, cscale=None, grad_private=False,
                     res_slot=None, res_alias=False):
    ca, cb = coefs if coefs is not None else gate_coefs(gate)
    epi = "mpsum" if res is not None else ("emb_silu" if cscale is not None else "none")
    cfg = ConvCfg(pw2, pw3, B, T, epi, ta, tb, clip, torch.is_grad_enabled(), grad_private=grad_private, res_slot=res_slot,
                  res_alias=res_alias)
    return _ConvOp.apply(x, pw2.param, pw3.param, ca, cb, cscale, res, cfg)


CAT_ACT_FUSED = int(_os.environ.get("ONIRIS_CAT_ACT_FUSED", "1"))


def conv_cat_act_ok(x, skip, pw):
    N, H, W, C1 = x.shape
    Cin = C1 + skip.shape[-1]
    glds = BIG_TILE >= 3 and Cin % 64 == 0 and pw.CinP == Cin and Cin <= 1024 and N * H * W >= 8192
    return bool(CAT_ACT_FUSED and x.is_cuda and not torch.is_grad_enabled() and pw.taps == 1 and pw.cin == Cin and C1 % 8 == 0
                and Cin % 8 == 0 and not glds and x.is_contiguous() and skip.is_contiguous())


@torch.no_grad()
def conv_cat_act(x, skip, w1, w2, pw):
    N, H, W, C1 = x.shape
    Cin = C1 + skip.shape[-1]
    Co = roundup(pw.cout, 8)
    out = torch.empty((N, H, W, Co), dtype=BF16, device=x.device)
    a = torch.empty((N, H, W, Cin), dtype=BF16, device=x.device)
    _conv_launch(x, None, pw.wf, None, out, None, None, 1, 1, N, H, W, Cin, pw.CinP, Co, pw.CoutP, 1,
                 x2=skip, act_out=a, x_split=C1, cat_w=(float(w1), float(w2)))
    return out, a


KEEP_CTX_PRODUCT = int(_os.environ.get("ONIRIS_KEEP_CTX_PRODUCT", "1"))


def ctx_product_ok(H, W, Cin, Cout):
    return bool(KEEP_CTX_PRODUCT and BIG_TILE >= 3 and not (BIG_TILE & 16) and Cin % 32 == 0 and Cin >= 32 and H % 8 == 0
                and W % 8 == 0 and Cout % 8 == 0 and 2 * H * W * Cin * 2 < (1 << 31))


@torch.no_grad()
def gated_conv_ctx_product(pair, pw2, pw3, B, out=None):
    _, two, H, W, Cin = pair.shape
    assert two == 2 and pair.is_contiguous() and pair.dtype == BF16
    Co = roundup(pw2.cout, 8)
    y3 = out if out is not None else torch.empty((B, H, W, Co), dtype=torch.float32, device=pair.device)
    _conv_launch(None, pair, pw2.wf, pw3.wf, None, None, None, B, 1, 1, H, W, Cin, pw2.CinP, Co, pw2.CoutP, 9,
                 ctx_bstride=2, ctx_T=2, coff=(0, 1), ctx_fill=0.0, ctx_prod=y3, ctx_prod_mode=3)
    return y3


def pair_conv_ok(x, pw2):
    N, H, W, Cin = x.shape
    Co = roundup(pw2.cout, 8)
    return bool(BIG_TILE >= 3 and not (BIG_TILE & 16) and Cin % 32 == 0 and Cin >= 32 and H % 8 == 0 and W % 8 == 0
                and Co % 8 == 0 and 2 * H * W * Cin * 2 < (1 << 31) and (H // 8) * N <= 65535 and W // 8 <= 65535)


@torch.no_grad()
def gated_conv_eval(x, gate, pw2, pw3, B, t, ctx_frames, coefs=None, res=None, ta=0.0, tb=0.0, clip=0.0, cscale=None,
                    ctx_T=None, ctx_prod=None, ctx_prod_mode=0, ctx_rows=0):
    if ctx_rows:
        return _gated_conv_eval_pair(x, gate, pw2, pw3, B, ctx_frames, coefs, res, ta, tb, clip, cscale, ctx_T, ctx_prod,
                                     ctx_prod_mode, ctx_rows)
    ctx_T = t + 2 if ctx_T is None else ctx_T
    assert ctx_frames.shape[1] == ctx_T and (ctx_T == t + 2 or t == 1)
    N, H, W, Cin = x.shape
    Co = roundup(pw2.cout, 8)
    out = torch.empty((N, H, W, Co), dtype=BF16, device=x.device)
    ca, cb = coefs if coefs is not None else gate_coefs(gate)
    ca, cb = ca.float().contiguous(), cb.float().contiguous()
    kw, ret = {}, out
    if res is not None:
        kw = dict(epi=_lib.EPI_MPSUM, res=res, ta=ta, tb=tb, clip=clip)
    elif cscale is not None:
        ret = torch.empty_like(out)
        kw = dict(epi=_lib.EPI_EMB_SILU, escale=_rows_f32(cscale), out2=ret)
    if ctx_prod_mode:
        assert t == 1 and ctx_prod.dtype == torch.float32 and tuple(ctx_prod.shape) == (B, H, W, Co) and ctx_prod.is_contiguous()
        kw.update(ctx_prod=ctx_prod, ctx_prod_mode=ctx_prod_mode)
    _conv_launch(x, ctx_frames, pw2.wf, pw3.wf, out, ca, cb, B, 1, t, H, W, Cin, pw2.CinP, Co, pw2.CoutP, 9,
                 ctx_bstride=ctx_T, ctx_T=ctx_T, coff=(0, 1), ctx_fill=0.0, **kw)
    return ret


def _gated_conv_eval_pair(x, gate, pw2, pw3, B, ctx_frames, coefs, res, ta, tb, clip, cscale, ctx_T, ctx_prod, ctx_prod_mode,
                          ctx_rows):
    ctx_T = 2 if ctx_T is None else ctx_T
    N, H, W, Cin = x.shape
    R = ctx_rows
    assert N == B == 2 * R and ctx_T == 2 and ctx_frames.shape[:2] == (R, 2), (x.shape, B, R, ctx_frames.shape)
    Co = roundup(pw2.cout, 8)
    out = torch.empty((N, H, W, Co), dtype=BF16, device=x.device)
    ca, cb = coefs if coefs is not None else gate_coefs(gate)
    ca, cb = ca.float().contiguous(), cb.float().contiguous()
    assert ca.numel() == R and cb.numel() == R
    ret, cs = out, None
    if res is None and cscale is not None:
        ret = torch.empty_like(out)
        cs = _rows_f32(cscale)
        assert tuple(cs.shape) == (R, Co), (cs.shape, R, Co)
    if ctx_prod_mode:
        assert ctx_prod.dtype == torch.float32 and tuple(ctx_prod.shape) == (R, H, W, Co) and ctx_prod.is_contiguous()

# ... 1233 lines not shown
```

include/oniris.h:

```cpp
#ifndef ONIRIS_H
#define ONIRIS_H
#include <stddef.h>
#include <stdint.h>

#ifdef __cplusplus
extern "C" {
#endif

typedef void* oniris_stream_t;

const char* oniris_last_error(void);
int oniris_abi_version(void);
int oniris_profile_arm(void* start_event, void* stop_event);
int oniris_profile_disarm(void);
int oniris_set_cu_reserve(int k);
long long oniris_set_ew_nt_bytes(long long bytes);
int oniris_census(int on);
long long oniris_census_read(char* buf , long long cap);
int oniris_struct_sizes(int32_t* out4 );

int oniris_train_mask(int n_frames, int image_size, int32_t* kv_num_blocks, int32_t* kv_indices, int* block_size);
int oniris_infer_mask(int n_frames, int image_size, int32_t* kv_num_blocks, int32_t* kv_indices, int* block_size);
int oniris_mask_transpose(int n_rows, int n_cols, const int32_t* kv_num_blocks, const int32_t* kv_indices,
                          int32_t* q_num_blocks, int32_t* q_indices);

typedef struct OnirisWeightDesc {
  float* w;
  float* grad;
  void* wf;
  void* wb;
  void* dwp;
  float* dws;
  int32_t cout, cin, taps, kt;
  int32_t CoutP, CinP;
  int32_t CoutPb, CinPb;
  int32_t row_start;
  int32_t perm3;
  float gain;
  int32_t nsplit_cap;
  int32_t* nsplit;
  int32_t tile_start;
  int32_t pad_;
} OnirisWeightDesc;

int oniris_weight_prep(const OnirisWeightDesc* descs, int ndesc, int total_rows, int total_tiles, int training,
                       oniris_stream_t stream);
int oniris_weight_bwd(const OnirisWeightDesc* descs, int ndesc, int total_rows, oniris_stream_t stream);

int oniris_dart_input(const float* images, const float* noise, const float* sigma, void* xcl, int B, int S, int T, int C,
                      int H, int W, float sigma_data, float* c_noise_out, int cpad ,
                      oniris_stream_t stream);
int oniris_dart_loss(const void* F, const float* images, const float* noise, const float* sigma, const float* out_gain,
                     float* losses, int B, int S, int T, int C, int H, int W, float sigma_data, oniris_stream_t stream);
int oniris_dart_loss_bwd(const void* F, const float* images, const float* noise, const float* sigma,
                         const float* out_gain, const float* dlosses, void* dF, float* dgain_part, int B, int S, int T,
                         int C, int H, int W, float sigma_data, oniris_stream_t stream);

int oniris_loss_tail(const float* mse, const float* sigma, const float* coef, float* out, float* dcoef, float* ring_sigma,
                     float* ring_loss, int* ring_pos, long long* count, int cap, int B, int T, int sig_pitch, int sig_off,
                     int nterms, float sigma_data, oniris_stream_t stream);

int oniris_precond_out(const void* F, const float* x, const float* sigma, const float* out_gain, float* D, int N, int C,
                       int H, int W, float sigma_data, oniris_stream_t stream);
int oniris_dart_input_pair(const float* x, const float* sigma, void* xcl, int B, int T, int C, int H, int W, float sigma_data,
                           float* c_noise_out, int cpad, oniris_stream_t stream);
int oniris_precond_out_guided(const void* F, const float* x, const float* sigma, const float* out_gain, float* D, int N, int C,
                              int H, int W, float sigma_data, float guidance, oniris_stream_t stream);
int oniris_sampler_update(int mode, float* x_hat, const float* x_pred, float* d_io, const float* x_aux, float* x_out, size_t n,
                          float t_a, float dt, float* sigma_buf, int nsig, float sigma_next, oniris_stream_t stream);
int oniris_embed_eval(const float* c_noise, const int64_t* labels, const float* freqs, const float* phases,
                      const float* w_noise, const float* w_label, void* emb, int N, int cnoise, int cemb, int label_dim,
                      oniris_stream_t stream);
int oniris_gates(const float* c_noise, const float* params, const int32_t* nctx, float* ca, float* cb, int L, int N, int T,
                 oniris_stream_t stream);

int oniris_gates_bwd(const float* c_noise, const float* params, const int32_t* nctx, const float* dca, const float* dcb,
                     float* dparams, int L, int N, int T, oniris_stream_t stream);
int oniris_emb_scale(const void* c_all, const float* gain, const int32_t* seg, float* c, int N, int Ctot,
                     oniris_stream_t stream);
#define ONIRIS_EMB_BWD_CHUNKS 16
int oniris_emb_scale_bwd(const float* dc, const void* c_all, const float* gain, const int32_t* start, void* dc_all,
                         float* dgain_part, int N, int Ctot, int K, oniris_stream_t stream);
int oniris_embed_pre(const float* c_noise, const int64_t* labels, const float* freqs, const float* phases, void* four,
                     void* onehot, int N, int cnoise, int cnoiseP, int label_dim, int labelP, oniris_stream_t stream);
int oniris_embed_post(const void* e1, const void* e2, void* emb, size_t n, float t, oniris_stream_t stream);
int oniris_embed_post_bwd(const void* demb, const void* e1, const void* e2, void* de1, void* de2, size_t n, float t,
                          oniris_stream_t stream);

int oniris_adamw(float* p, const float* g, float* m, float* v, size_t n, float lr, float beta1, float beta2,
                 float eps, float weight_decay, int step, float grad_scale, oniris_stream_t stream);
int oniris_adamw_clip_ema(float* p, const float* g, float* m, float* v, size_t n, float lr, float beta1, float beta2,
                          float eps, float weight_decay, int step, float grad_scale, const float* gnorm_sq,
                          float max_norm, float* ema0, float ema_w0, float* ema1, float ema_w1, oniris_stream_t stream);
#define ONIRIS_SQNORM_WS 1024
int oniris_sqnorm(const float* g, size_t n, float* out, oniris_stream_t stream);

enum { ONIRIS_EPI_NONE = 0, ONIRIS_EPI_EMB_SILU = 1, ONIRIS_EPI_MPSUM = 2, ONIRIS_EPI_ACT_BWD = 3 };

typedef struct OnirisConvArgs {
  const void* x;
  const void* ctx;
  const void* w_own;
  const void* w_ctx;
  void* out;
  const float* coef_own;
  const float* coef_ctx;
  int32_t B, S, T, H, W;
  int32_t Cin, CinP, Cout, CoutP;
  int32_t taps;
  int32_t ctx_bstride, ctx_T, coff0, coff1;
  float ctx_fill;
  int32_t epi;
  const void* res;
  const void* escale;
  const float* emb_gain;
  void* out2;
  float ta, tb, clip;
  void* ctx_out;
  int32_t big_tile;
  int32_t escale_pitch;
  float* splitk_ws;
  size_t splitk_ws_bytes;
  int32_t* clip_flag;
  float* ctx_prod;
  int32_t ctx_prod_mode;
  int32_t x_split;
  const void* x2;
  void* act_out;
  float cat_w1, cat_w2;
  int32_t ctx_rows;
  int32_t ab_c1;
  const void* ab_da;
  const void* ab_xo;
  void* ab_dskip;
  const void* ab_dadd;
  float ab_w1, ab_w2, ab_dxo_scale;
} OnirisConvArgs;

int oniris_conv_fwd(const OnirisConvArgs* args , oniris_stream_t stream);

typedef struct OnirisWgradArgs {
  const void* x;
  const void* dy;
  void* dwp;
  const float* scale;
  int32_t B, T, H, W, Cin, CinP, Cout, CoutP, taps;
  int32_t xb_stride, x_T, coff;
  float fill;
  int32_t nsplit_cap, taps_total, tap0;
  int32_t pad_;
  int32_t* nsplit_out;
} OnirisWgradArgs;

int oniris_conv_wgrad(const OnirisWgradArgs* args , oniris_stream_t stream);
int oniris_conv_wgrad_group(const OnirisWgradArgs* args , int ngroups,
                            oniris_stream_t stream);

int oniris_gconv_bwd_prep(const void* dout, const void* out, const void* y3, const float* coef_own,
                          const float* coef_ctx, float* d_coef_own, float* d_coef_ctx, void* dy3, int B, int S, int T,
                          int64_t frame_elems, oniris_stream_t stream);

int oniris_gconv_bwd_fused(int mode, const void* g, const void* raw, const void* y3, const float* coef_own,
                           const float* coef_ctx, const float* cscale, const void* xo, void* dout, void* dres, void* dy3,
                           float* d_coef_own, float* d_coef_ctx, float* d_cscale, int B, int T, int P, int C, float ta,
                           float tb, float clip,
                           int cscale_pitch ,
                           const int32_t* clip_flag, float* coef_own_scaled, oniris_stream_t stream);

int oniris_act_fwd(const void* x, const void* skip, void* xo, void* a, float* sden, int64_t npix, int C1, int C2,
                   float w1, float w2, int norm, int resample, int Ho, int Wo, oniris_stream_t stream);
int oniris_act_bwd(const void* da, const void* dxo, const void* xo, const float* sden, void* dx, void* dskip,
                   const void* dadd, int64_t npix, int C1, int C2, float w1, float w2, int norm,
                   float dxo_scale ,
                   oniris_stream_t stream);
int oniris_emb_silu_bwd(const void* du, const void* y, const float* c, void* dy, float* dc, int N, int P, int C,
                        int c_pitch ,
                        int dc_is_zero ,
                        oniris_stream_t stream);
int oniris_mpsum_bwd(const void* g, const void* out, void* dres, void* dv ,
                     int64_t numel, float ta, float tb, float clip, oniris_stream_t stream);
int oniris_mpsum_mask(void* g, const void* out, int64_t numel, float clip, const int32_t* clip_flag, oniris_stream_t stream);
int oniris_resample(const void* in, void* out, const void* add, int64_t N, int H, int W, int C, int mode, float scale,
                    oniris_stream_t stream);
int oniris_resample_filter(const void* in, void* out, const void* add, int64_t N, int H, int W, int C, int mode,
                           const float* taps , int ntaps, float scale, oniris_stream_t stream);

int oniris_qkv_norm(const void* qkv, void* q, void* k, void* v, int64_t n_tokens, int C, int64_t kv_tokens_per_batch,
                    int64_t kv_batch_stride, int64_t kv_token_offset, oniris_stream_t stream);
int oniris_qkv_norm_bwd(const void* qkv, const void* dq, const void* dk, const void* dv, void* dqkv,
                        int64_t n_tokens, int C, oniris_stream_t stream);
int oniris_qkv_norm_rope(const void* qkv, void* q, void* k, void* v, const float* cos_t, const float* sin_t,
                         const float* scale_t, int64_t n_tokens, int C, int P, int pos_mod, oniris_stream_t stream);
int oniris_qkv_norm_rope_bwd(const void* qkv, const void* dq, const void* dk, const void* dv, void* dqkv,
                             const float* cos_t, const float* sin_t, const float* scale_t, int64_t n_tokens, int C, int P,
                             int pos_mod, oniris_stream_t stream);
int oniris_rope(const void* x, void* xr, void* xt, const float* cos_t, const float* sin_t, const float* scale_t,
                int mode, int B, int frames, int P, int C, int pos_offset, int pos_mod,
                int64_t x_batch_stride ,
                int64_t xr_batch_stride , oniris_stream_t stream);
int oniris_qkv_norm_hd(const void* qkv, void* q, void* k, void* v, const float* cos_t, const float* sin_t,
                       const float* scale_t, int64_t n_tokens, int heads, int head_dim, int P, int pos_mod, int pos_off,
                       int rope, int seq_frames, oniris_stream_t stream);
int oniris_qkv_norm_hd_bwd(const void* qkv, const void* dq, const void* dk, const void* dv, void* dqkv, const float* cos_t,
                           const float* sin_t, const float* scale_t, int64_t n_tokens, int heads, int head_dim, int P,
                           int pos_mod, int pos_off, int rope, int seq_frames, oniris_stream_t stream);
int oniris_rope_hd(const void* x, void* out, const float* cos_t, const float* sin_t, const float* scale_t, int64_t n_tokens,
                   int heads, int head_dim, int P, int pos_mod, int pos_off, int mode, int seq_frames, oniris_stream_t stream);
int oniris_qkv_norm_rope_eval(const void* qkv, void* q, void* k, void* v, void* kr, const float* cos_t, const float* sin_t,
                              const float* scale_t, int64_t n_tokens, int C, int64_t kv_tokens_per_batch,
                              int64_t kv_batch_stride, int64_t kv_token_offset, int pos, oniris_stream_t stream);

int oniris_qkv_eval(const void* x, const void* w, void* q, void* k, void* v, void* kr, const float* cos_t, const float* sin_t,
                    const float* scale_t, int64_t n_tokens, int C, int CinP, int64_t kv_tokens_per_batch,
                    int64_t kv_batch_stride, int64_t kv_token_offset, int pos, oniris_stream_t stream);
int oniris_qkv_eval_pair(const void* x, const void* w, void* q, void* k, void* v, void* kr, const float* cos_t, const float* sin_t,
                         const float* scale_t, int64_t n_tokens, int64_t split, int C, int CinP, int64_t kv_tokens_per_batch,
                         int64_t kv_batch_stride, int64_t kv_token_offset, int pos, void* q2, void* k2, void* v2,
                         oniris_stream_t stream);

typedef struct OnirisAttnArgs {
  const void *q, *k, *v, *qt, *kt, *vt;
  void* out;
  float* lse;
  const int32_t *kv_num, *kv_idx;
  const int32_t *q_num, *q_idx;
  int32_t tab_cols, qtab_cols;
  int32_t B, heads, Lq, Lk, C;
  int32_t mask_mode, P, T;
  int32_t tab_block;
  const void *dout, *doutt;
  const float* delta;
  void *dq, *dk, *dv;
  float* dkv_part;
  int32_t dkv_chunks, dkv_item_keys;
  const int32_t* sched;
  int32_t sched_wgs, sched_slots;
  int64_t v_bstride;
  int64_t k_bstride;
  float* split_ws;
  int32_t kv_splits, frame_kernel;
} OnirisAttnArgs;

int oniris_frame_attn_bwd(const OnirisAttnArgs* args, oniris_stream_t stream);
int oniris_frame_attn_qkv_fwd(const void* qkv, void* out, float* lse, int64_t n_frames, int P, int heads, oniris_stream_t stream);
int oniris_frame_attn_qkv_bwd(const void* qkv, const void* out, const float* lse, const void* dout, void* dqkv, int64_t n_frames,
                              int P, int heads, oniris_stream_t stream);

int oniris_attn_schedule(int n_pairs, int n_blocks, const int32_t* weight, int n_wg, int32_t* sched, int n_slots);

int oniris_attn_fwd(const OnirisAttnArgs* args , oniris_stream_t stream);
int oniris_attn_bwd_prep(const void* dout, const void* out, float* delta, void* doutt, const float* lse, float* neg, int B,
                         int heads, int L, int C, oniris_stream_t stream);
int oniris_attn_bwd_dq(const OnirisAttnArgs* args , oniris_stream_t stream);
int oniris_attn_bwd_dkv(const OnirisAttnArgs* args , oniris_stream_t stream);


int oniris_conv_f32(const float* x, const float* w, float* out, int64_t N, int H, int W, int Cin, int Cout, int taps,
                    oniris_stream_t stream);
int oniris_wgrad_f32(const float* x, const float* dy, float* dw, int64_t N, int H, int W, int Cin, int Cout, int taps,
                     oniris_stream_t stream);
typedef struct OnirisAttnF32Args {
  const float* q; const float* k; const float* v; float* out; float* lse;
  const float* dout; const float* delta; float* dq; float* dk; float* dv;
  int32_t BH, Lq, Lk, D, mask_mode, P, T, q_frame_off;
  float scale; int32_t pad_;
} OnirisAttnF32Args;
int oniris_attn_f32_fwd(const OnirisAttnF32Args* args, oniris_stream_t stream);
int oniris_attn_f32_bwd(const OnirisAttnF32Args* args, oniris_stream_t stream);

int oniris_vae_temb(const float* params, const int32_t* table, int n_res_blocks, const float* t, int B, float* emb,
                    oniris_stream_t stream);
int oniris_vae_up(const float* x, int64_t sb, int64_t st, int64_t sh, int64_t sw, int64_t sc, int B, int T, int H, int W, int C,
                  const float* in_scale, const float* in_shift, const float* w, const float* bias, int tcomp, int scomp, float* out,
                  oniris_stream_t stream);
int oniris_vae_res_a(const float* x, const float* cache_in, float* cache_out, const float* emb, const float* w, const float* bias,
                     int B, int T, int H, int W, int C, int g, int nch, int gpt, float* out, oniris_stream_t stream);
int oniris_vae_res_b(const float* u, const float* res, const float* w, const float* bias, int B, int T, int H, int W, int C,
                     int nch, float* out, oniris_stream_t stream);
int oniris_vae_out(const float* x, const float* w, const float* bias, int B, int T, int H, int W, int Cin, int Cout, int split,
                   const float* logvar_mult, float* out, float* out2, int64_t sb, int64_t st, int64_t sh, int64_t sw, int64_t sc,
                   uint8_t* frames, oniris_stream_t stream);

int oniris_vae_down(const void* x, int x_is_u8, int64_t sb, int64_t st, int64_t sh, int64_t sw, int64_t sc, int B, int To, int Ho,
                    int Wo, int Cin, int tcomp, int scomp, int normalize, const float* w, const float* bias, int Cout, float* out,
                    oniris_stream_t stream);
int oniris_vae_latents(const float* x, int B, int T, int H, int W, int C, const float* mean, const float* std, float* out,
                       int64_t sb, int64_t st, int64_t sh, int64_t sw, int64_t sc, oniris_stream_t stream);

int oniris_vae_train_res_a(const float* x, const float* emb, const float* w, const float* bias, int B, int T, int H, int W, int C,
                           int g, int nch, int gpt, float* a_out, oniris_stream_t stream);
int oniris_vae_train_res_b(const float* a_in, const float* res, const float* w, const float* bias, int B, int T, int H, int W,
                           int C, int nch, float* out, oniris_stream_t stream);
int oniris_vae_res_b_bwd(const float* dout, const float* a_in, const float* wd, int B, int T, int H, int W, int C, int nch,
                         float* da, oniris_stream_t stream);
int oniris_vae_res_a_bwd(const float* da, const float* x, const float* emb, const float* dout, const float* wd, int B, int T,
                         int H, int W, int C, int g, int nch, int gpt, float* dx, float* emb_part, oniris_stream_t stream);
int oniris_vae_conv3_wgrad_bwd(const float* xin, const float* emb, const float* dA, int B, int T, int H, int W, int C, int g,
                               int causal, float* slab, int nslab, oniris_stream_t stream);
int oniris_vae_slab_sum_bwd(const float* slab, int nslab, int64_t n, float* out, oniris_stream_t stream);
int oniris_vae_lin_dx_bwd(const float* dy, int Cy, int tcy, int scy, const float* wc, float* dx, int Cx, int tcx, int scx, int B,
                          int T, int H, int W, oniris_stream_t stream);
int oniris_vae_lin_dw_bwd(const float* x, int Cx, int tcx, int scx, const float* dy, int Cy, int tcy, int scy, int B, int T, int H,
                          int W, float* slab, int nslab, oniris_stream_t stream);

// ... 6 lines not shown
```

Before: 8810 latent-frames/s.

## Compute dy3 on the fly inside dgrad and wgrad streaming kernels

Instead of materialising the dy3 gradient tensor (a per-frame weighted combination of the two dout slots) in HBM, the streaming dgrad conv kernel and the streaming wgrad kernel rebuild it in LDS/registers from the already-loaded dout halos using the per-frame cb coefficients. This removes the dy3 write, its re-reads, and the third DMA stream in those kernels, and in the wgrad kernel it reduces LDS use. The cost is extra ALU work per tile and extra synchronisation in the dgrad prologue. It is gated by an env flag that defaults on and only applies to shapes handled by the streaming kernels.

```diff
diff --git a/autoregressive_diffusion_amd/_lib.py b/autoregressive_diffusion_amd/_lib.py
--- a/autoregressive_diffusion_amd/_lib.py
+++ b/autoregressive_diffusion_amd/_lib.py
@@ -37,7 +37,8 @@
                 ("ctx_prod", c_void_p), ("ctx_prod_mode", c_int32), ("x_split", c_int32), ("x2", c_void_p), ("act_out", c_void_p),
                 ("cat_w1", c_float), ("cat_w2", c_float), ("ctx_rows", c_int32),
                 ("ab_c1", c_int32), ("ab_da", c_void_p), ("ab_xo", c_void_p), ("ab_dskip", c_void_p), ("ab_dadd", c_void_p),
-                ("ab_w1", c_float), ("ab_w2", c_float), ("ab_dxo_scale", c_float)]
+                ("ab_w1", c_float), ("ab_w2", c_float), ("ab_dxo_scale", c_float),
+                ("dy3_cb", c_void_p), ("dy3_tb", c_float)]
 
 
 class WgradArgs(C.Structure):
@@ -46,7 +47,7 @@
                 ("Cout", c_int32), ("CoutP", c_int32), ("taps", c_int32),
                 ("xb_stride", c_int32), ("x_T", c_int32), ("coff", c_int32), ("fill", c_float),
                 ("nsplit_cap", c_int32), ("taps_total", c_int32), ("tap0", c_int32), ("pad_", c_int32),
-                ("nsplit_out", c_void_p)]
+                ("nsplit_out", c_void_p), ("dy3_cb", c_void_p), ("dy3_tb", c_float)]
 
 
 class AttnArgs(C.Structure):
diff --git a/autoregressive_diffusion_amd/csrc/common.h b/autoregressive_diffusion_amd/csrc/common.h
--- a/autoregressive_diffusion_amd/csrc/common.h
+++ b/autoregressive_diffusion_amd/csrc/common.h
@@ -104,6 +104,17 @@
 __device__ __forceinline__ float act_adjoint_out(float g, float w, bool has_add, float add) {
   return has_add ? __builtin_fmaf(w, g, add) : g * w;
 }
+__device__ __forceinline__ float dy3_term(float dout, float tb) { return dout * tb; }
+__device__ __forceinline__ float dy3_accum(float acc, float cb, float dr) { return __builtin_fmaf(cb, dr, acc); }
+__device__ __forceinline__ float dy3_combine(float cb0, float dr0, float cb1, float dr1) {
+  return dy3_accum(dy3_accum(0.f, cb0, dr0), cb1, dr1);
+}
+__device__ __forceinline__ bf16x8 dy3_combine8(bf16x8 d0, bf16x8 d1, float cb0, float cb1, float tb) {
+  bf16x8 o;
+#pragma unroll
+  for (int k = 0; k < 8; ++k) o[k] = f2bf(dy3_combine(cb0, dy3_term(bf2f(d0[k]), tb), cb1, dy3_term(bf2f(d1[k]), tb)));
+  return o;
+}
 __device__ __forceinline__ int mfma_row(int r, int lane) { return (r & 3) + 8 * (r >> 2) + 4 * (lane >> 5); }
 
 __device__ __forceinline__ float wave_sum(float v) {
diff --git a/autoregressive_diffusion_amd/csrc/conv_api.hip b/autoregressive_diffusion_amd/csrc/conv_api.hip
--- a/autoregressive_diffusion_amd/csrc/conv_api.hip
+++ b/autoregressive_diffusion_amd/csrc/conv_api.hip
@@ -26,7 +26,12 @@
                         a.ab_dskip && a.ab_c1 > 0 && a.ab_c1 < a.Cout && a.ab_c1 % 8 == 0 && a.ctx_prod_mode == 0 && a.ctx_rows == 0),
                    "conv_fwd: EPI_ACT_BWD is a plain 1x1 launch (S == 1) with ab_da / ab_xo / ab_dskip and 0 < ab_c1 < Cout, ab_c1 %% 8 == 0");
   ONIRIS_CHECK_ARG(a.x2 == nullptr || (a.taps == 1 && a.ctx == nullptr), "conv_fwd: x2 (concatenated input) is a 1x1, context-free option");
-  const bool has_ctx = a.ctx != nullptr;
+  const bool fly = a.ctx == nullptr && a.dy3_cb != nullptr;
+  if (fly && !(a.S == 2 && a.taps == 9 && a.w_ctx)) {
+    oniris_set_error("conv_fwd: ctx == NULL with dy3_cb needs the streaming kernel (S == 2, 32 -> <= 32 channels, coff = (2, 1), ctx_fill = 0)");
+    return ONIRIS_EUNSUPPORTED;
+  }
+  const bool has_ctx = a.ctx != nullptr || fly;
   ONIRIS_CHECK_ARG(!has_ctx || (a.w_ctx && a.taps == 9), "conv_fwd: context path needs w_ctx and taps == 9");
   if (a.clip_flag && (a.taps == 1 || (a.S == 1 && has_ctx))) {
     const hipError_t e = hipMemsetD32Async((hipDeviceptr_t)a.clip_flag, 1, 1, st);
diff --git a/autoregressive_diffusion_amd/csrc/conv_fwd_s2ctx.hip b/autoregressive_diffusion_amd/csrc/conv_fwd_s2ctx.hip
--- a/autoregressive_diffusion_amd/csrc/conv_fwd_s2ctx.hip
+++ b/autoregressive_diffusion_amd/csrc/conv_fwd_s2ctx.hip
@@ -11,6 +11,10 @@
 
 int conv_dispatch_s2ctx(const OnirisConvArgs& a, hipStream_t st) {
   if (a.big_tile >= 4 && conv_stream_ok(a)) return launch_conv_stream(a, st);
+  if (!a.ctx) {
+    oniris_set_error("conv_fwd: ctx == NULL with dy3_cb needs the streaming kernel (32 -> <= 32 channels, coff = (2, 1), ctx_fill = 0)");
+    return ONIRIS_EUNSUPPORTED;
+  }
   if (a.big_tile >= 3 && conv_glds_ok(a, 16, 16, (a.CoutP % 64 == 0) ? 64 : 32))
     return (a.CoutP % 64 == 0) ? glds_pick<2>(a, st) : glds_pick<1>(a, st);
   if (a.big_tile >= 3 && a.W == 8 && a.H == 8 && a.CoutP % 64 == 0 && conv_glds_ok(a, 8, 8, 64))
diff --git a/autoregressive_diffusion_amd/csrc/conv_stream.h b/autoregressive_diffusion_amd/csrc/conv_stream.h
--- a/autoregressive_diffusion_amd/csrc/conv_stream.h
+++ b/autoregressive_diffusion_amd/csrc/conv_stream.h
@@ -17,9 +17,10 @@
   int nt;
 };
 
-template <bool ALIAS>
+template <bool ALIAS, bool FLY = false>
 __global__ __launch_bounds__(256, 2) void conv_stream_kernel(const ConvStreamDev d) {
 #if defined(__HIP_DEVICE_COMPILE__)
+  static_assert(!(ALIAS && FLY), "FLY is a form of the dgrad kernel");
   constexpr int TAPS = 9, KS = 2, NST = TAPS * KS, HW_ = 18, HALO = 6 * 18, HBUF = 7168;
   constexpr int NXS0 = ALIAS ? 4 : 2, NCTX = ALIAS ? 0 : 3;
   constexpr int EROW = 80, STGB = 32 * EROW;
@@ -75,7 +76,7 @@
     hv[i] = (e < HALO * 4 && (unsigned)y < (unsigned)H && (unsigned)x < (unsigned)W) ? ((y * W + x) * Cin + gp * 8) * 2 : OOB;
   }
   const i32x4 rs_x = make_rsrc((const bf16*)a.x + (size_t)b * 2 * T * frame_elems, 2 * T * frame_elems * 2);
-  const i32x4 rs_c = make_rsrc((const bf16*)a.ctx + (size_t)b * a.ctx_bstride * frame_elems, a.ctx_T * frame_elems * 2);
+  const i32x4 rs_c = make_rsrc(FLY ? (const bf16*)a.x : (const bf16*)a.ctx + (size_t)b * a.ctx_bstride * frame_elems, FLY ? 0 : a.ctx_T * frame_elems * 2);
   const i32x4 rs_f = make_rsrc(oniris_fill_rows, 128);
   const int fillsel = (a.ctx_fill != 0.f) ? 64 : 0;
   const unsigned lds0 = (unsigned)(size_t)(lds_void_t*)smem, wdst = lds0 + wave * 1024;
@@ -97,6 +98,20 @@
   auto issue_x = [&](int f) __attribute__((always_inline)) {
     halo(rs_x, f * frame_elems * 2, XS0 + (ALIAS ? (f & 3) : (f & 1)) * HBUF);
     halo(rs_x, (T + f) * frame_elems * 2, XS1 + (f & 1) * HBUF);
+  };
+  typedef const __attribute__((address_space(4))) float cfloat_t;
+  auto combine_ctx = [&](int f) __attribute__((always_inline)) {
+    const int n0 = __builtin_amdgcn_readfirstlane((b * 2 + 0) * T + f), n1 = __builtin_amdgcn_readfirstlane((b * 2 + 1) * T + f);
+    const float c0 = ((cfloat_t*)(size_t)a.dy3_cb)[n0], c1 = ((cfloat_t*)(size_t)a.dy3_cb)[n1];
+    const unsigned char* s0 = smem + XS0 + (f & 1) * HBUF;
+    const unsigned char* s1 = smem + XS1 + (f & 1) * HBUF;
+    unsigned char* dst = smem + ctx_slot(f);
+#pragma unroll
+    for (int i = 0; i < 2; ++i) {
+      const int e = i * 256 + tid;
+      if (e < HALO * 4)
+        *(bf16x8*)(dst + e * 16) = dy3_combine8(*(const bf16x8*)(s0 + e * 16), *(const bf16x8*)(s1 + e * 16), c0, c1, a.dy3_tb);
+    }
   };
 
   bf16x8 wreg[NST];
@@ -149,11 +164,24 @@
     }
   };
   const int per_halo = (uw < 3) ? 2 : 1;
-  const int n_dma = (ALIAS ? 2 : 3) * per_halo + ((emb && uw == 0) ? 1 : 0);
+  const int n_dma = ((ALIAS || FLY) ? 2 : 3) * per_halo + ((emb && uw == 0) ? 1 : 0);
   const int n_st = (a.ctx_out ? 1 : 0) + 2 * (mps ? ((a.out2 ? 1 : 0) + 1) : emb ? 2 : 1);
   if (nfr <= 0) return;
-  issue_ctx(ts + a.coff0);
-  issue_ctx(ts + a.coff1);
+  if constexpr (FLY) {
+    const int f0 = ts + a.coff0, f1 = ts + a.coff1;
+    if (f0 < T) issue_x(f0); else halo_fill(ctx_slot(f0));
+    if (f1 < T) issue_x(f1); else halo_fill(ctx_slot(f1));
+    if (f1 < T) {
+      asm volatile("s_waitcnt vmcnt(0)" ::: "memory");
+      __syncthreads();
+      if (f0 < T) combine_ctx(f0);
+      combine_ctx(f1);
+      __syncthreads();
+    }
+  } else {
+    issue_ctx(ts + a.coff0);
+    issue_ctx(ts + a.coff1);
+  }
   issue_x(ts);
   if (emb && uw == 0) issue_esc(ts);
 
@@ -171,16 +199,16 @@
     SSTAMP(1)
     const bool has_next = i + 1 < nfr;
     const int nfrm = __builtin_amdgcn_readfirstlane((b * 2 + uslot) * T + t);
-    typedef const __attribute__((address_space(4))) float cfloat_t;
     const float cown = a.coef_own ? ((cfloat_t*)(size_t)a.coef_own)[nfrm] : 1.f;
     const float cctx = a.coef_ctx ? ((cfloat_t*)(size_t)a.coef_ctx)[nfrm] : 1.f;
     if (mps) load_res(t);
     if (has_next) {
       issue_x(tn);
-      if (!ALIAS) issue_ctx(tn + a.coff1);
+      if (!ALIAS && !FLY) issue_ctx(tn + a.coff1);
       if (emb && uw == 0) issue_esc(tn);
     }
 
+    if constexpr (FLY) combine_ctx(t);
     SSTAMP(2)
     f32x16 acc0, acc1;
 #pragma unroll
@@ -328,7 +356,9 @@
 }
 
 static inline bool conv_stream_ok(const OnirisConvArgs& a) {
-  if (!(a.S == 2 && a.ctx && a.taps == 9 && a.Cin == 32 && a.CinP == 64 && a.CoutP == 32 && a.W % 16 == 0 && a.H % 4 == 0))
+  const bool fly = !a.ctx && a.dy3_cb;
+  if (fly && !(a.coff0 == 2 && a.coff1 == 1 && a.ctx_fill == 0.f)) return false;
+  if (!(a.S == 2 && (a.ctx || fly) && a.taps == 9 && a.Cin == 32 && a.CinP == 64 && a.CoutP == 32 && a.W % 16 == 0 && a.H % 4 == 0))
     return false;
   if (!(a.ctx_fill == 0.f || a.ctx_fill == 1.f) || a.ctx_T != a.T) return false;
   if (!((a.coff0 == -2 && a.coff1 == -1) || (a.coff0 == 2 && a.coff1 == 1))) return false;
@@ -348,8 +378,9 @@
   d.nt = 2LL * a.B * a.T * a.H * a.W * a.Cout * 2 >= oniris_ew_nt_bytes();
   d.seglen = cdiv(a.T, nseg);
   d.nseg = cdiv(a.T, d.seglen);
-  const bool alias = a.ctx == a.x && a.ctx_bstride == 2 * a.T && d.dir == 1;
+  const bool alias = a.ctx && a.ctx == a.x && a.ctx_bstride == 2 * a.T && d.dir == 1;
   if (alias) oniris_launch_tagged(d.nt ? "nt-stores" : nullptr, conv_stream_kernel<true>, dim3(units * d.nseg), dim3(256), stream, d);
+  else if (!a.ctx) oniris_launch_tagged(d.nt ? "nt-stores" : nullptr, conv_stream_kernel<false, true>, dim3(units * d.nseg), dim3(256), stream, d);
   else oniris_launch_tagged(d.nt ? "nt-stores" : nullptr, conv_stream_kernel<false>, dim3(units * d.nseg), dim3(256), stream, d);
   ONIRIS_LAUNCH_CHECK();
   return ONIRIS_OK;
diff --git a/autoregressive_diffusion_amd/csrc/conv_wgrad.hip b/autoregressive_diffusion_amd/csrc/conv_wgrad.hip
--- a/autoregressive_diffusion_amd/csrc/conv_wgrad.hip
+++ b/autoregressive_diffusion_amd/csrc/conv_wgrad.hip
@@ -298,7 +298,7 @@
   const OnirisWgradArgs& a = args[0];
   for (int g = 0; g < ngroups; ++g) {
     const OnirisWgradArgs& b = args[g];
-    ONIRIS_CHECK_ARG(b.x && b.dy && b.dwp, "conv_wgrad: null pointer (group %d)", g);
+    ONIRIS_CHECK_ARG(b.x && (b.dy || (g > 0 && b.dy3_cb)) && b.dwp, "conv_wgrad: null pointer (group %d)", g);
     ONIRIS_CHECK_ARG(b.nsplit_cap >= 1 && b.taps_total >= b.taps + b.tap0 && b.tap0 >= 0,
                      "conv_wgrad: bad slab description (group %d)", g);
     ONIRIS_CHECK_ARG(b.B > 0 && b.T > 0, "conv_wgrad: empty group %d", g);
@@ -309,7 +309,10 @@
   ONIRIS_CHECK_ARG(a.Cin % 8 == 0 && a.Cout % 8 == 0, "conv_wgrad: Cin/Cout must be multiples of 8");
   ONIRIS_CHECK_ARG(a.CoutP % 32 == 0 && a.CinP % 64 == 0 && a.CoutP >= a.Cout && a.CinP >= a.Cin,
                    "conv_wgrad: bad padded sizes");
+  bool fly = false;
+  for (int g = 1; g < ngroups; ++g) fly |= !args[g].dy;
   if (a.taps == 1) {
+    if (fly) { oniris_set_error("conv_wgrad: dy == NULL (dy3_cb) needs the streaming kernel"); return ONIRIS_EUNSUPPORTED; }
     if (ngroups == 1 && a.pad_ >= 0 && wgrad1x1_glds_ok(a)) return launch_wgrad1x1_glds(a, stream);
     return wgrad_pick_tile<1, 16>(args, ngroups, stream);
   }
@@ -318,6 +321,7 @@
     const int rc = launch_wgrad_stream(args, stream);
     if (rc != 1) return rc;
   }
+  if (fly) { oniris_set_error("conv_wgrad: dy == NULL (dy3_cb) needs the streaming kernel"); return ONIRIS_EUNSUPPORTED; }
   if (W >= 16 && W % 16 == 0 && H % 8 == 0) return wgrad_pick_tile<9, 16>(args, ngroups, stream);
   if (W == 8 && H % 8 == 0) return wgrad_pick_tile<9, 8>(args, ngroups, stream);
   if (W == 4 && H % 4 == 0) return wgrad_pick_tile<9, 4>(args, ngroups, stream);
diff --git a/autoregressive_diffusion_amd/csrc/conv_wgrad_stream.h b/autoregressive_diffusion_amd/csrc/conv_wgrad_stream.h
--- a/autoregressive_diffusion_amd/csrc/conv_wgrad_stream.h
+++ b/autoregressive_diffusion_amd/csrc/conv_wgrad_stream.h
@@ -6,6 +6,8 @@
   const void* dout;
   const void* dy3;
   const float* scale;
+  const float* cb;
+  float tb;
   void* dwp2;
   void* dwp3;
   int32_t* nsplit2;
@@ -15,15 +17,16 @@
   float fill;
 };
 
-template <int PH>
+template <int PH, bool FLY>
 __global__ __launch_bounds__(64 * PH, 2) void conv_wgrad_stream_kernel(const WgradStreamDev d) {
 #if defined(__HIP_DEVICE_COMPILE__)
   static_assert(PH == 8 || PH == 4, "tile heights");
   constexpr int NTHR = 64 * PH, NPOS = PH * 16;
   constexpr int TAPS = 9, HW_ = 18, HALO = (PH + 2) * HW_, XB = HALO * 64, DB = NPOS * 64;
+  constexpr int ND = FLY ? 2 : 3;
   constexpr int XS0 = 0, XS1 = 4 * XB, DY0 = 6 * XB;
-  constexpr int LDS_BYTES = 6 * XB + 6 * DB;
-  static_assert(LDS_BYTES <= 160 * 1024 && 5 * 3 * 16 * 64 * 4 <= LDS_BYTES, "LDS budget");
+  constexpr int LDS_BYTES = 6 * XB + 2 * ND * DB;
+  static_assert(LDS_BYTES <= 160 * 1024 && (PH == 8 ? 5 : 1) * 3 * 16 * 64 * 4 <= LDS_BYTES, "LDS budget");
   __shared__ __attribute__((aligned(16))) unsigned char smem[LDS_BYTES];
 
   const int tid = threadIdx.x, lane = tid & 63, wave = tid >> 6;
@@ -62,7 +65,7 @@
     xvoff[i] = xok[i] ? (((y0 + hy - 1) * W + (x0 + hx - 1)) * Cin + ci) * 2 : OOB;
   }
   const i32x4 rs_do = make_rsrc(d.dout, d.B * 2 * T * HWp * Cout * 2);
-  const i32x4 rs_d3 = make_rsrc(d.dy3, d.B * T * HWp * Cout * 2);
+  const i32x4 rs_d3 = make_rsrc(FLY ? d.dout : d.dy3, FLY ? 0 : d.B * T * HWp * Cout * 2);
   const i32x4 rs_x = make_rsrc(d.x, d.B * 2 * T * HWp * Cin * 2);
   const i32x4 rs_f = make_rsrc(oniris_fill_rows, 128);
   const int fillsel = (d.fill != 0.f) ? 64 : 0;
@@ -83,10 +86,10 @@
   auto issue_frame = [&](int f) __attribute__((always_inline)) {
     issue_halo(0, f, XS0 + (f & 3) * XB);
     issue_halo(1, f, XS1 + (f & 1) * XB);
-    const unsigned dyb = DY0 + (f & 1) * 3 * DB;
+    const unsigned dyb = DY0 + (f & 1) * ND * DB;
     dma16(rs_do, dvoff, (((b * 2 + 0) * T + f) * HWp * Cout) * 2 + dy_origin, dyb + wdst);
     dma16(rs_do, dvoff, (((b * 2 + 1) * T + f) * HWp * Cout) * 2 + dy_origin, dyb + DB + wdst);
-    dma16(rs_d3, dvoff, ((b * T + f) * HWp * Cout) * 2 + dy_origin, dyb + 2 * DB + wdst);
+    if constexpr (!FLY) dma16(rs_d3, dvoff, ((b * T + f) * HWp * Cout) * 2 + dy_origin, dyb + 2 * DB + wdst);
   };
 
   const int hh = lane >> 5, q = (lane & 15) >> 2;
@@ -108,10 +111,12 @@
   };
 
   const bool scaled = role == 0 && d.scale != nullptr;
-  float sc_next = 1.f;
+  const bool fly = FLY && role != 0;
+  float sc_next = 1.f, sc1_next = 1.f;
   if (t0 < t1) {
     if (scaled) sc_next = d.scale[(b * 2 + slot) * T + t0];
-    asm volatile("" : "+v"(sc_next));
+    if (fly) { sc_next = d.cb[(b * 2 + 0) * T + t0]; sc1_next = d.cb[(b * 2 + 1) * T + t0]; }
+    asm volatile("" : "+v"(sc_next), "+v"(sc1_next));
     issue_halo(0, t0 - 2, XS0 + ((t0 - 2) & 3) * XB);
     issue_halo(0, t0 - 1, XS0 + ((t0 - 1) & 3) * XB);
     issue_frame(t0);
@@ -120,20 +125,22 @@
   for (int t = t0; t < t1; ++t) {
     dma_wait();
     __syncthreads();
-    float sc = sc_next;
-    asm volatile("" : "+v"(sc));
+    float sc = sc_next, sc1 = sc1_next;
+    asm volatile("" : "+v"(sc), "+v"(sc1));
     if (t + 1 < t1) {
       if (scaled) sc_next = d.scale[(b * 2 + slot) * T + t + 1];
-      asm volatile("" : "+v"(sc_next));
+      if (fly) { sc_next = d.cb[(b * 2 + 0) * T + t + 1]; sc1_next = d.cb[(b * 2 + 1) * T + t + 1]; }
+      asm volatile("" : "+v"(sc_next), "+v"(sc1_next));
       issue_frame(t + 1);
     }
-    const unsigned char* abuf = smem + DY0 + (t & 1) * 3 * DB + ((role == 0) ? slot * DB : 2 * DB);
+    const unsigned char* abuf = smem + DY0 + (t & 1) * ND * DB + ((role == 0) ? slot * DB : (FLY ? 0 : 2 * DB));
     const unsigned char* bbuf = smem + ((role == 0) ? (slot ? XS1 + (t & 1) * XB : XS0 + (t & 3) * XB)
                                                     : XS0 + ((t - 3 + role) & 3) * XB);
     constexpr int NK = 4, NSTEP = NK * TAPS, LA = 3;
     bf16x8 af[2], bfm[4];
     auto ld_a = [&](int kb, int j) __attribute__((always_inline)) {
       bf16x8 v = trf(abuf + dya + j * 16 * 64);
+      if (fly) v = dy3_combine8(v, trf(abuf + DB + dya + j * 16 * 64), sc, sc1, d.tb);
       if (scaled) {
 #pragma unroll
         for (int k = 0; k < 8; ++k) v[k] = f2bf(bf2f(v[k]) * sc);
@@ -249,6 +256,7 @@
   if (o.Cin > 32 && o.Cout > 32) return false;
   if (o.B != 1 || o.coff != 0 || o.tap0 != 0 || o.taps_total != 9 || o.xb_stride != o.T || o.x_T != o.T) return false;
   if (c0.x != o.x || c1.x != o.x || c0.dy != c1.dy || c0.dwp != c1.dwp || c0.scale || c1.scale) return false;
+  if (!c0.dy && (!c0.dy3_cb || c0.dy3_cb != c1.dy3_cb || c0.dy3_tb != c1.dy3_tb)) return false;
   if (c0.B != c1.B || c0.T != c1.T || o.T != 2 * c0.B * c0.T) return false;
   if (c0.xb_stride != 2 * c0.T || c1.xb_stride != 2 * c0.T || c0.x_T != c0.T || c1.x_T != c0.T) return false;
   if (c0.coff != -2 || c1.coff != -1 || c0.tap0 != 0 || c1.tap0 != 9 || c0.taps_total != 18 || c1.taps_total != 18) return false;
@@ -261,7 +269,8 @@
   const OnirisWgradArgs &o = a[0], &c0 = a[1];
   WgradStreamDev d;
   memset(&d, 0, sizeof(d));
-  d.x = o.x; d.dout = o.dy; d.dy3 = c0.dy; d.scale = o.scale;
+  const bool fly = c0.dy == nullptr;
+  d.x = o.x; d.dout = o.dy; d.dy3 = c0.dy; d.scale = o.scale; d.cb = c0.dy3_cb; d.tb = c0.dy3_tb;
   d.dwp2 = o.dwp; d.dwp3 = c0.dwp; d.nsplit2 = o.nsplit_out; d.nsplit3 = c0.nsplit_out;
   d.B = c0.B; d.T = c0.T; d.H = o.H; d.W = o.W; d.Cin = o.Cin; d.CinP = o.CinP; d.Cout = o.Cout; d.CoutP = o.CoutP;
 #ifndef WGRAD_STREAM_PH
@@ -281,8 +290,13 @@
   if (nseg < 1) nseg = 1;
   d.seglen = cdiv(d.T, nseg);
   d.nseg = cdiv(d.T, d.seglen);
-  if (ph == 4) oniris_launch(conv_wgrad_stream_kernel<4>, dim3(units * d.nseg, gy), dim3(256), stream, d);
-  else oniris_launch(conv_wgrad_stream_kernel<8>, dim3(units * d.nseg, gy), dim3(512), stream, d);
+  if (ph == 4) {
+    if (fly) oniris_launch(conv_wgrad_stream_kernel<4, true>, dim3(units * d.nseg, gy), dim3(256), stream, d);
+    else oniris_launch(conv_wgrad_stream_kernel<4, false>, dim3(units * d.nseg, gy), dim3(256), stream, d);
+  } else {
+    if (fly) oniris_launch(conv_wgrad_stream_kernel<8, true>, dim3(units * d.nseg, gy), dim3(512), stream, d);
+    else oniris_launch(conv_wgrad_stream_kernel<8, false>, dim3(units * d.nseg, gy), dim3(512), stream, d);
+  }
   ONIRIS_LAUNCH_CHECK();
   return ONIRIS_OK;
 }
diff --git a/autoregressive_diffusion_amd/csrc/weights.hip b/autoregressive_diffusion_amd/csrc/weights.hip
--- a/autoregressive_diffusion_amd/csrc/weights.hip
+++ b/autoregressive_diffusion_amd/csrc/weights.hip
@@ -391,13 +391,15 @@
 #pragma unroll
       for (int i = 0; i < 8; ++i) {
         const float dd = bf2f(dv[i]);
-        s1[s] += dd * bf2f(ov[i]); s2[s] += dd * bf2f(yv[i]); acc[i] += c[s] * dd;
-      }
-    }
-    bf16x8 o;
-#pragma unroll
-    for (int i = 0; i < 8; ++i) o[i] = f2bf(acc[i]);
-    *(bf16x8*)(dy3f + e) = o;
+        s1[s] += dd * bf2f(ov[i]); s2[s] += dd * bf2f(yv[i]); acc[i] = dy3_accum(acc[i], c[s], dd);
+      }
+    }
+    if (dy3) {
+      bf16x8 o;
+#pragma unroll
+      for (int i = 0; i < 8; ++i) o[i] = f2bf(acc[i]);
+      *(bf16x8*)(dy3f + e) = o;
+    }
   }
   for (int s = 0; s < S; ++s) {
     const float a = block_sum(s1[s], red), bsum = block_sum(s2[s], red);
@@ -477,20 +479,22 @@
             float gg = bf2f(gv[i]);
             if (masked && !(fabsf(bf2f(xv[i])) < clip)) gg = 0.f;
             drv[i] = f2bf(gg * ta);
-            d = gg * tb;
+            d = dy3_term(gg, tb);
             if (alias) dv[i] = f2bf(gg);
           }
           float dr = d;
           if (!alias) { dv[i] = f2bf(d); dr = bf2f(dv[i]); }
-          s1[s] += dr * r_; s2[s] += dr * bf2f(yv3[i]); acc3[i] += cbv[s] * dr;
+          s1[s] += dr * r_; s2[s] += dr * bf2f(yv3[i]); acc3[i] = dy3_accum(acc3[i], cbv[s], dr);
         }
         if (!alias || masked) stv<NT>((bf16x8*)(dout + o), dv);
         if (MODE == 2 && dres) stv<NT>((bf16x8*)(dres + o), drv);
       }
-      bf16x8 o3;
-#pragma unroll
-      for (int i = 0; i < 8; ++i) o3[i] = f2bf(acc3[i]);
-      stv<NT>((bf16x8*)(dy3 + (size_t)bt * PC + off), o3);
+      if (dy3) {
+        bf16x8 o3;
+#pragma unroll
+        for (int i = 0; i < 8; ++i) o3[i] = f2bf(acc3[i]);
+        stv<NT>((bf16x8*)(dy3 + (size_t)bt * PC + off), o3);
+      }
     }
   }
   if (MODE == 1 && (G8 & (G8 - 1)) == 0) {
@@ -539,7 +543,7 @@
                                       int P, int C, float ta, float tb, float clip, int cscale_pitch,
                                       const int32_t* clip_flag, float* coef_own_scaled, oniris_stream_t stream_) {
   hipStream_t stream = (hipStream_t)stream_;
-  ONIRIS_CHECK_ARG((mode == 1 || mode == 2) && g && raw && y3 && coef_own && coef_ctx && dout && dy3 && d_coef_own &&
+  ONIRIS_CHECK_ARG((mode == 1 || mode == 2) && g && raw && y3 && coef_own && coef_ctx && dout && d_coef_own &&
                    d_coef_ctx && B > 0 && T > 0 && P > 0 && C % 8 == 0 && C <= 512, "gconv_bwd_fused: bad arguments");
   ONIRIS_CHECK_ARG(mode != 1 || (cscale && d_cscale), "gconv_bwd_fused: mode 1 needs cscale / d_cscale");
   ONIRIS_CHECK_ARG(mode != 2 || ((dres || coef_own_scaled) && (clip <= 0.f || xo)),
@@ -576,7 +580,7 @@
                                      int64_t frame_elems,
                                      oniris_stream_t stream_) {
   hipStream_t stream = (hipStream_t)stream_;
-  ONIRIS_CHECK_ARG(dout && out && y3 && coef_own && coef_ctx && S1 && S2 && dy3 && B > 0 && T > 0 && (S == 1 || S == 2) &&
+  ONIRIS_CHECK_ARG(dout && out && y3 && coef_own && coef_ctx && S1 && S2 && B > 0 && T > 0 && (S == 1 || S == 2) &&
                    frame_elems > 0 && frame_elems % 8 == 0, "gconv_bwd_prep: bad arguments");
   int slices = 1;
   while (slices < 2 && (long long)B * T * slices < 1024 && frame_elems / (slices * 2) >= 256 * 8 * 2) slices *= 2;
diff --git a/autoregressive_diffusion_amd/ops.py b/autoregressive_diffusion_amd/ops.py
--- a/autoregressive_diffusion_amd/ops.py
+++ b/autoregressive_diffusion_amd/ops.py
@@ -555,35 +555,36 @@
 def _conv_launch(x, ctx, w_own, w_ctx, out, coef_own, coef_ctx, B, S, T, H, W, Cin, CinP, Cout, CoutP, taps,
                  ctx_bstride=0, ctx_T=0, coff=(0, 0), ctx_fill=0.0, epi=0, res=None, escale=None, emb_gain=None,
                  out2=None, ta=0.0, tb=0.0, clip=0.0, ctx_out=None, clip_flag=None, ctx_prod=None, ctx_prod_mode=0,
-                 x2=None, act_out=None, x_split=0, cat_w=(1.0, 1.0), ctx_rows=0, act_bwd=None):
+                 x2=None, act_out=None, x_split=0, cat_w=(1.0, 1.0), ctx_rows=0, act_bwd=None, dy3_cb=None, dy3_tb=1.0):
     if KernelProfile.enabled:
+        gctx = x if (ctx is None and dy3_cb is not None) else ctx
         flops = 2.0 * B * S * T * H * W * Cout * Cin * taps
-        if ctx is not None:
+        if gctx is not None:
             flops += 2.0 * B * T * H * W * Cout * Cin * 2 * taps
         nt = 2 if CoutP % 64 == 0 else 1
-        if (BIG_TILE >= 4 and S == 2 and ctx is not None and taps == 9 and Cin == 32 and CinP == 64 and CoutP == 32 and W % 16 == 0
+        if (BIG_TILE >= 4 and S == 2 and gctx is not None and taps == 9 and Cin == 32 and CinP == 64 and CoutP == 32 and W % 16 == 0
                 and H % 4 == 0 and ctx_fill in (0.0, 1.0) and ctx_T == T and tuple(coff) in ((-2, -1), (2, 1))):
-            key = f"conv_stream_kernel<ALIAS={int(ctx.data_ptr() == x.data_ptr() and ctx_bstride == 2 * T and coff[0] < 0)}>"
-        elif (BIG_TILE >= 3 and S == 2 and ctx is not None and taps == 9 and Cin % 32 == 0 and H % 16 == 0 and W % 16 == 0
+            key = f"conv_stream_kernel<ALIAS={int(gctx.data_ptr() == x.data_ptr() and ctx_bstride == 2 * T and coff[0] < 0)}>"
+        elif (BIG_TILE >= 3 and S == 2 and gctx is not None and taps == 9 and Cin % 32 == 0 and H % 16 == 0 and W % 16 == 0
                 and ctx_fill in (0.0, 1.0)):
             key = f"conv_glds_kernel<NT={nt},PW=16,NW=8,MT=1,WC=1,CTX=1>"
-        elif (BIG_TILE >= 3 and S == 2 and ctx is not None and taps == 9 and Cin % 32 == 0 and H == 8 and W == 8
+        elif (BIG_TILE >= 3 and S == 2 and gctx is not None and taps == 9 and Cin % 32 == 0 and H == 8 and W == 8
               and CoutP % 64 == 0 and ctx_fill in (0.0, 1.0)):
             key = "conv_glds_kernel<NT=1,PW=8,NW=8,MT=1,WC=2,CTX=1>"
-        elif (BIG_TILE >= 4 and not (BIG_TILE & 128) and S == 1 and ctx is None and taps == 9 and Cin == 32 and CinP == 64 and CoutP == 32
+        elif (BIG_TILE >= 4 and not (BIG_TILE & 128) and S == 1 and gctx is None and taps == 9 and Cin == 32 and CinP == 64 and CoutP == 32
               and W % 16 == 0 and H % 8 == 0 and x2 is None and B * T * (H // 8) * (W // 16) >= 512):
             key = "conv_plain_stream_kernel"
-        elif (BIG_TILE >= 3 and S == 1 and ctx is None and taps == 9 and Cin % 32 == 0 and T % 2 == 0
+        elif (BIG_TILE >= 3 and S == 1 and gctx is None and taps == 9 and Cin % 32 == 0 and T % 2 == 0
               and ((H % 16 == 0 and W % 16 == 0) or (H == 8 and W == 8 and CoutP % 64 == 0))):
             key = (f"conv_glds_kernel<NT={nt},PW=16,NW=8,MT=1,WC=1,CTX=0>" if H % 16 == 0 else
                    "conv_glds_kernel<NT=1,PW=8,NW=8,MT=1,WC=2,CTX=0>")
-        elif (BIG_TILE >= 3 and taps == 1 and ctx is None and Cin % 64 == 0 and CinP == Cin
+        elif (BIG_TILE >= 3 and taps == 1 and gctx is None and Cin % 64 == 0 and CinP == Cin
               and epi in (0, _lib.EPI_MPSUM, _lib.EPI_ACT_BWD) and B * S * T * H * W >= 8192):
             key = "conv1x1_glds_kernel<ACTB>" if epi == _lib.EPI_ACT_BWD else "conv1x1_glds_kernel"
         elif epi == _lib.EPI_ACT_BWD:
             key = f"conv_fwd_kernel<S=1,TAPS=1,CK=64,NT={2 if CoutP % 64 == 0 else 3},CTX=0,PW={_patch_w(W)},ACTB>"
         else:
-            key = f"conv_fwd_kernel<S={S},TAPS={taps},CK={32 if taps == 9 else 64},NT={nt},CTX={int(ctx is not None)},PW={_patch_w(W)}>"
+            key = f"conv_fwd_kernel<S={S},TAPS={taps},CK={32 if taps == 9 else 64},NT={nt},CTX={int(gctx is not None)},PW={_patch_w(W)}>"
         if PROFILE_SHAPES:
             key += f" [{H}x{W} {Cin}->{Cout} epi={epi}{' act_bwd' if act_bwd is not None else ''}{' dadd' if act_bwd is not None and act_bwd[3] is not None else ''}{' res' if res is not None else ''}{' out2' if out2 is not None else ''}{' y3' if ctx_out is not None else ''}{' dgrad' if coff[0] > 0 else ''}]"
         KernelProfile.enabled = False
@@ -591,14 +592,14 @@
             e0, e1 = _timed_launch(lambda: _conv_launch(x, ctx, w_own, w_ctx, out, coef_own, coef_ctx, B, S, T, H, W, Cin, CinP,
                                                         Cout, CoutP, taps, ctx_bstride, ctx_T, coff, ctx_fill, epi, res, escale,
                                                         emb_gain, out2, ta, tb, clip, ctx_out, clip_flag, ctx_prod, ctx_prod_mode,
-                                                        ctx_rows=ctx_rows, act_bwd=act_bwd))
+                                                        ctx_rows=ctx_rows, act_bwd=act_bwd, dy3_cb=dy3_cb, dy3_tb=dy3_tb))
         finally:
             KernelProfile.enabled = True
         px = B * T * H * W
         nbytes = 2.0 * (S * px * Cin + S * px * Cout * (1 + (out2 is not None) + (res is not None))
                         + (px * Cout if ctx_out is not None else 0)
-                        + taps * CoutP * CinP * (3 if ctx is not None else 1))
-        if ctx is not None and ctx.data_ptr() != x.data_ptr():
+                        + taps * CoutP * CinP * (3 if gctx is not None else 1))
+        if gctx is not None and gctx.data_ptr() != x.data_ptr():
             nbytes += 2.0 * B * ctx_T * H * W * Cin
         if act_bwd is not None:
             nbytes += 2.0 * px * (2 * Cout + (act_bwd[4] if act_bwd[3] is not None else 0))
@@ -620,6 +621,7 @@
         a.x2, a.act_out, a.x_split, a.cat_w1, a.cat_w2 = _p(x2), _p(act_out), x_split, cat_w[0], cat_w[1]
     a.big_tile = BIG_TILE
     a.ctx_rows = ctx_rows
+    a.dy3_cb, a.dy3_tb = _p(dy3_cb), dy3_tb
     if act_bwd is not None:
         da, xo, dskip, dadd, a.ab_c1, a.ab_w1, a.ab_w2, a.ab_dxo_scale = act_bwd
         a.ab_da, a.ab_xo, a.ab_dskip, a.ab_dadd = _p(da), _p(xo), _p(dskip), _p(dadd)
@@ -640,7 +642,8 @@
     return _splitk_cache[key]
 
 
-def _wgrad_args(x, dy, pw, scale, B, T, H, W, Cin, CinP, Cout, CoutP, taps, xb_stride, x_T, coff, fill, tap0=0):
+def _wgrad_args(x, dy, pw, scale, B, T, H, W, Cin, CinP, Cout, CoutP, taps, xb_stride, x_T, coff, fill, tap0=0, dy3_cb=None,
+                dy3_tb=1.0):
     a = _lib.WgradArgs()
     pw.touched = pw.hit = True
     if pw.members is not None:
@@ -651,7 +654,19 @@
     a.B, a.T, a.H, a.W, a.Cin, a.CinP, a.Cout, a.CoutP, a.taps = B, T, H, W, Cin, CinP, Cout, CoutP, taps
     a.xb_stride, a.x_T, a.coff, a.fill = xb_stride, x_T, coff, fill
     a.pad_ = WGRAD_VARIANT
+    a.dy3_cb, a.dy3_tb = _p(dy3_cb), dy3_tb
     return a
+
+
+DY3_FLY = int(_os.environ.get("ONIRIS_DY3_FLY", "1"))
+
+
+def _wgrad_stream_family(B, T, H, W, Cin, Cout, pw2, pw3):
+    if WGRAD_VARIANT < 0 or (WGRAD_VARIANT & 2) or W % 16 != 0 or H % 8 != 0 or (Cin > 32 and Cout > 32):
+        return False
+    if 2 * B * T * H * W * max(Cin, Cout) * 2 >= 1 << 31:
+        return False
+    return B * (W // 16) * (H // 8) <= min(pw2.nsplit_cap, pw3.nsplit_cap)
 
 
 def _wgrad_launch_group(arglist):
@@ -673,7 +688,7 @@
         seen, nbytes = set(), 0.0
         for a in arglist:
             for ptr, n in ((a.x, a.B * a.xb_stride * a.H * a.W * a.Cin), (a.dy, a.B * a.T * a.H * a.W * a.Cout)):
-                if ptr not in seen:
+                if ptr and ptr not in seen:
                     seen.add(ptr)
                     nbytes += 2.0 * n
         KernelProfile.enabled = False
@@ -801,7 +816,8 @@
                 ca_own = torch.empty_like(ca)
             else:
                 dout = torch.empty_like(g)
-            dy3 = torch.empty_like(y3)
+            wg_fly, dg_fly, dy3 = _dy3_plan(ctx, cfg, x, y3, Co)
+            fly_tb = cfg.tb if alias else 1.0
             acc = pw2.bank.zero_arena.take(N * (2 + (Co if cfg.epi == "emb_silu" else 0)), dev)
             dca, dcb = acc[:N], acc[N:2 * N]
             res_alias = alias and cfg.res_alias
@@ -844,21 +860,23 @@
             if not fused:
                 acc = pw2.bank.zero_arena.take(2 * N, dev)
                 dca, dcb = acc[:N], acc[N:2 * N]
-                dy3 = torch.empty_like(y3)
+                wg_fly, dg_fly, dy3 = _dy3_plan(ctx, cfg, x, y3, Co)
+                fly_tb = 1.0
                 check(lib.oniris_gconv_bwd_prep(_p(dout), _p(raw), _p(y3), _p(ca), _p(cb), _p(dca), _p(dcb), _p(dy3), B, 2,
                                                 T, H * W * Co, _stream()), "gconv_bwd_prep")
             if ctx.needs_input_grad[0]:
                 dx = torch.empty_like(x)
                 sel = _clean_selector(B, T, dev)
-                _conv_launch(dout, dy3, pw2.wb, pw3.wb, dx, ca_own, sel, B, 2, T, H, W, Co, pw2.CinPb, Cin, pw2.CoutPb, 9,
-                             ctx_bstride=T, ctx_T=T, coff=(2, 1), ctx_fill=0.0)
+                _conv_launch(dout, None if dg_fly else dy3, pw2.wb, pw3.wb, dx, ca_own, sel, B, 2, T, H, W, Co, pw2.CinPb, Cin,
+                             pw2.CoutPb, 9, ctx_bstride=T, ctx_T=T, coff=(2, 1), ctx_fill=0.0,
+                             dy3_cb=cb if dg_fly else None, dy3_tb=fly_tb)
             grp = []
             if _wants_wgrad(pw2):
                 grp.append(_wgrad_args(x, dout, pw2, ca_own, 1, N, H, W, Cin, pw2.CinP, Co, pw2.CoutP, 9, N, N, 0, 0.0))
             if _wants_wgrad(pw3):
                 for j, coff in enumerate((-2, -1)):
-                    grp.append(_wgrad_args(x, dy3, pw3, None, B, T, H, W, Cin, pw3.CinP, Co, pw3.CoutP, 9, 2 * T, T, coff,
-                                           1.0, tap0=9 * j))
+                    grp.append(_wgrad_args(x, None if wg_fly else dy3, pw3, None, B, T, H, W, Cin, pw3.CinP, Co, pw3.CoutP, 9, 2 * T,
+                                           T, coff, 1.0, tap0=9 * j, dy3_cb=cb if wg_fly else None, dy3_tb=fly_tb))
             if grp:
                 _wgrad_launch_group(grp)
         else:
@@ -881,6 +899,17 @@
             cfg.res_slot.put(dres)
             dres = None
         return dx, None, None, dca, dcb, dcs, dres, None
+
+
+def _dy3_plan(ctx, cfg, x, y3, Co):
+    N, H, W, Cin = x.shape
+    pw2, pw3 = cfg.pw2, cfg.pw3
+    wg_want, dg_want = _wants_wgrad(pw3), ctx.needs_input_grad[0]
+    wg_fly = bool(DY3_FLY and wg_want and _wants_wgrad(pw2) and _wgrad_stream_family(cfg.B, cfg.T, H, W, Cin, Co, pw2, pw3))
+    dg_fly = bool(DY3_FLY and dg_want and 2 * cfg.T * H * W * 32 * 2 < 1 << 31 and
+                  _s2ctx_family(cfg.T, H, W, Co, pw2.CinPb, pw2.CoutPb, cfg.T, (2, 1), 0.0) == "stream")
+    need = (wg_want and not wg_fly) or (dg_want and not dg_fly)
+    return wg_fly, dg_fly, (torch.empty_like(y3) if need else None)
 
 
 _const_cache = {}
diff --git a/include/oniris.h b/include/oniris.h
--- a/include/oniris.h
+++ b/include/oniris.h
@@ -135,6 +135,8 @@
   void* ab_dskip;
   const void* ab_dadd;
   float ab_w1, ab_w2, ab_dxo_scale;
+  const float* dy3_cb;
+  float dy3_tb;
 } OnirisConvArgs;
 
 int oniris_conv_fwd(const OnirisConvArgs* args , oniris_stream_t stream);
@@ -150,6 +152,8 @@
   int32_t nsplit_cap, taps_total, tap0;
   int32_t pad_;
   int32_t* nsplit_out;
+  const float* dy3_cb;
+  float dy3_tb;
 } OnirisWgradArgs;
 
 int oniris_conv_wgrad(const OnirisWgradArgs* args , oniris_stream_t stream);
```

Result: no change. 8892 latent-frames/s, median of 6 (+0.9%).
